# nyasyamorina/font-renderer

Measured on AMD Instinct MI355X. Metric: Mpixel/s AA glyph coverage, higher is better.
Workload: dtype f32

## Files before the change

### bindings/fr_raster.zig

```
const std = @import("std");

const Font = @import("../font/Font.zig");
const Glyph = @import("../font/Glyph.zig");
const Image = @import("Image.zig");
const Point = @import("geometry.zig").Point;

pub const fr_ctx = opaque {};
pub const fr_glyphset = opaque {};
pub const fr_plan = opaque {};
pub const fr_font = opaque {};

pub const Status = enum(c_int) { ok = 0, invalid = -1, hip = -2, nomem = -3, unsupported = -4 };
pub const Mode = enum(i32) { winding_i16 = 0, gray_debug = 1, mask_nonzero = 2, coverage_u8 = 3, sdf_u8 = 4 };
pub const SamplePhase = enum(i32) { corner = 0, center = 1 };
pub const FR_FONT_ALLOW_HINTED: u32 = 1;
pub const FR_FILL_CONSISTENT: u32 = 1;
pub const FR_TEXT_BGRA: u32 = 4;
pub const FR_TEXT_SRGB: u32 = 8;
pub const FR_TEXT_LOAD: u32 = 32;
pub const FR_TEXT_CACHE: u32 = 128;
pub const FR_TEXT_OVER: u32 = 256;

pub const RasterParams = extern struct {
    mode: i32,
    samples_per_axis: i32,
    sample_phase: i32,
    reserved: i32 = 0,
};

pub const Job = extern struct {
    glyph: u32,
    min_x: i32,
    max_y: i32,
    w: u32,
    h: u32,
    out_x: u32,
    out_y: u32,
    scale: f32,
};

pub const GlyphPlace = extern struct {
    glyph: u32,
    pen_x64: i32,
    pen_y: i32,
};

pub const GlyphPlaceEx = extern struct {
    glyph: u32,
    pen_x64: i32,
    pen_y64: i32,
    scale: f32,
    slant: f32,
};

pub const GlyphPlaceAffine = extern struct {
    glyph: u32,
    pen_x64: i32,
    pen_y64: i32,
    m: [4]f32,
};

pub const TextRun = extern struct {
    first: u32,
    count: u32,
    w: u32,
    h: u32,
    out_x: u32,
    out_y: u32,
    scale: f32,
};

pub extern "c" fn fr_abi_version() c_int;
pub extern "c" fn fr_last_error() [*:0]const u8;
pub extern "c" fn fr_build_id() [*:0]const u8;
pub extern "c" fn fr_ctx_create(device: c_int, hip_stream: ?*anyopaque, out: *?*fr_ctx) c_int;
pub extern "c" fn fr_ctx_destroy(ctx: ?*fr_ctx) void;
pub extern "c" fn fr_ctx_sync(ctx: *fr_ctx) c_int;
pub extern "c" fn fr_ctx_set_option(ctx: *fr_ctx, key: [*:0]const u8, value: i64) c_int;
pub extern "c" fn fr_glyphset_create(ctx: *fr_ctx, points_xy: [*]const i16, contour_start: [*]const u32, n_contours: u32, glyph_start: [*]const u32, n_glyphs: u32, out: *?*fr_glyphset) c_int;
pub extern "c" fn fr_glyphset_destroy(gs: ?*fr_glyphset) void;
pub extern "c" fn fr_glyphset_prepare(gs: *fr_glyphset) c_int;
pub extern "c" fn fr_glyphset_stats(gs: *const fr_glyphset, n_segments: ?*u64, n_records: ?*u64) c_int;
pub extern "c" fn fr_glyphset_set_boxes(gs: *fr_glyphset, boxes: [*]const i16) c_int;
pub extern "c" fn fr_plan_create(ctx: *fr_ctx, gs: *const fr_glyphset, jobs: [*]const Job, n_jobs: u32, params: *const RasterParams, out: *?*fr_plan) c_int;
pub extern "c" fn fr_plan_create_ex(ctx: *fr_ctx, gs: *const fr_glyphset, jobs: [*]const Job, n_jobs: u32, params: *const RasterParams, flags: u32, out: *?*fr_plan) c_int;
pub extern "c" fn fr_plan_destroy(plan: ?*fr_plan) void;
pub extern "c" fn fr_plan_render(plan: *fr_plan, out_dev: *anyopaque, out_stride: usize, out_rows: usize) c_int;
pub extern "c" fn fr_plan_render_timed(plan: *fr_plan, out_dev: *anyopaque, out_stride: usize, out_rows: usize, ms: *f32) c_int;
pub extern "c" fn fr_plan_pixels(plan: *const fr_plan) u64;
pub extern "c" fn fr_plan_stats(plan: *const fr_plan, n_jobs_cov4: ?*u32, n_jobs_general: ?*u32) c_int;
pub extern "c" fn fr_plan_describe(plan: *const fr_plan, buf: [*]u8, cap: usize) c_int;
pub extern "c" fn fr_text_plan_create(ctx: *fr_ctx, gs: *const fr_glyphset, places: [*]const GlyphPlace, n_places: u32, runs: [*]const TextRun, n_runs: u32, params: *const RasterParams, flags: u32, out: *?*fr_plan) c_int;
pub extern "c" fn fr_text_plan_create_rgba(ctx: *fr_ctx, gs: *const fr_glyphset, places: [*]const GlyphPlace, place_rgba: [*]const u8, n_places: u32, runs: [*]const TextRun, run_clear_rgba: [*]const u8, n_runs: u32, params: *const RasterParams, flags: u32, out: *?*fr_plan) c_int;
pub extern "c" fn fr_text_plan_create_ex(ctx: *fr_ctx, gs: *const fr_glyphset, places: [*]const GlyphPlaceEx, n_places: u32, runs: [*]const TextRun, n_runs: u32, params: *const RasterParams, flags: u32, out: *?*fr_plan) c_int;
pub extern "c" fn fr_text_plan_create_rgba_ex(ctx: *fr_ctx, gs: *const fr_glyphset, places: [*]const GlyphPlaceEx, place_rgba: [*]const u8, n_places: u32, runs: [*]const TextRun, run_clear_rgba: [*]const u8, n_runs: u32, params: *const RasterParams, flags: u32, out: *?*fr_plan) c_int;
pub extern "c" fn fr_text_plan_create_affine(ctx: *fr_ctx, gs: *const fr_glyphset, places: [*]const GlyphPlaceAffine, n_places: u32, runs: [*]const TextRun, n_runs: u32, params: *const RasterParams, flags: u32, out: *?*fr_plan) c_int;
pub extern "c" fn fr_text_plan_create_rgba_affine(ctx: *fr_ctx, gs: *const fr_glyphset, places: [*]const GlyphPlaceAffine, place_rgba: [*]const u8, n_places: u32, runs: [*]const TextRun, run_clear_rgba: [*]const u8, n_runs: u32, params: *const RasterParams, flags: u32, out: *?*fr_plan) c_int;
pub extern "c" fn fr_allgather_bands(ctx: *fr_ctx, nccl_comm: *anyopaque, atlas_dev: *anyopaque, band_bytes: usize) c_int;
pub extern "c" fn fr_gather_bands(ctx: *fr_ctx, nccl_comm: *anyopaque, atlas_dev: *anyopaque, band_bytes: usize, root: c_int) c_int;
pub extern "c" fn fr_render_batch(ctx: *fr_ctx, gs: *const fr_glyphset, jobs: [*]const Job, n_jobs: u32, params: *const RasterParams, out_host: *anyopaque, out_stride: usize, out_rows: usize) c_int;
pub extern "c" fn fr_render_batch_ex(ctx: *fr_ctx, gs: *const fr_glyphset, jobs: [*]const Job, n_jobs: u32, params: *const RasterParams, flags: u32, out_host: *anyopaque, out_stride: usize, out_rows: usize) c_int;
pub extern "c" fn fr_render_glyph_dims(box: *const [4]i16, units_per_em: u16, font_size: u16, min_corner: *[2]i16, max_corner: *[2]i16, width: *u16, height: *u16, scale: ?*f32) c_int;
pub extern "c" fn fr_render_glyph(ctx: *fr_ctx, points_xy: [*]const i16, contour_start: [*]const u32, n_contours: u32, box: *const [4]i16, units_per_em: u16, font_size: u16, mode: i32, out_host: *anyopaque) c_int;
pub extern "c" fn fr_render_glyph_ex(ctx: *fr_ctx, points_xy: [*]const i16, contour_start: [*]const u32, n_contours: u32, box: *const [4]i16, units_per_em: u16, font_size: u16, mode: i32, flags: u32, out_host: *anyopaque) c_int;
pub extern "c" fn fr_glyph_info_init(ctx: *fr_ctx, points_xy: [*]const i16, contour_start: [*]const u32, n_contours: u32, curve_type: [*]u8, include_p0: [*]u8) c_int;
pub extern "c" fn fr_winding_in_glyph(ctx: *fr_ctx, points_xy: [*]const i16, contour_start: [*]const u32, n_contours: u32, query_xy: [*]const i16, n_query: u32, out_winding: [*]i16) c_int;
pub extern "c" fn fr_winding_lattice(ctx: *fr_ctx, points_xy: [*]const i16, contour_start: [*]const u32, n_contours: u32, box: *const [4]i16, out_host: [*]i16) c_int;
pub extern "c" fn fr_glyph_debug_render(ctx: *fr_ctx, points_xy: [*]const i16, contour_start: [*]const u32, n_contours: u32, box: *const [4]i16, winding_scale: u8, rgb_host: [*]u8) c_int;
pub extern "c" fn fr_exact_lattice(ctx: *fr_ctx, points_xy: [*]const i16, contour_start: [*]const u32, n_contours: u32, k: u32, x0: i32, y0: i32, w: u32, h: u32, out_host: [*]i16) c_int;
pub extern "c" fn fr_exact_coverage(ctx: *fr_ctx, points_xy: [*]const i16, contour_start: [*]const u32, n_contours: u32, k: u32, x0: i32, y0: i32, w_px: u32, h_px: u32, n: u32, out_host: [*]u8) c_int;
pub extern "c" fn fr_atlas_layout(boxes: [*]const i16, n_glyphs: u32, first_glyph: u32, units_per_em: [*]const u16, n_upm: u32, font_size: u16, cell: u32, cols: u32, rows_per_page: u32, jobs_out: [*]Job, page_of_job: ?[*]u32, n_pages: ?*u32) c_int;
pub extern "c" fn fr_atlas_layout_glyph_dims(boxes: [*]const i16, n_glyphs: u32, first_glyph: u32, units_per_em: [*]const u16, n_upm: u32, font_size: u16, atlas_w: u32, @"align": u32, jobs_out: [*]Job, atlas_h: ?*u32) c_int;
pub extern "c" fn fr_font_open(ttf_bytes: *const anyopaque, len: usize, flags: u32, out: *?*fr_font) c_int;
pub extern "c" fn fr_font_close(font: ?*fr_font) void;
pub extern "c" fn fr_font_info(font: *const fr_font, units_per_em: ?*u16, num_glyphs: ?*u16, y0_baseline: ?*c_int) c_int;
pub extern "c" fn fr_font_char_to_glyph(font: *const fr_font, codepoint: u32, glyph_index: *u16) c_int;
pub extern "c" fn fr_font_glyph_advance(font: *const fr_font, glyph_index: u16, advance_width: *i16) c_int;
pub extern "c" fn fr_text_layout(font: *const fr_font, codepoints: [*]const u32, n: u32, font_size: u16, glyph_index_out: [*]u16, pen_x64_out: [*]i32, end_pen_x64: ?*i32) c_int;
pub extern "c" fn fr_font_glyph_measure(font: *fr_font, glyph_index: u16, n_contours: *u32, n_points: *u32, box: *[4]i16) c_int;
pub extern "c" fn fr_font_glyph_fill(font: *fr_font, glyph_index: u16, points_xy: [*]i16, contour_start: [*]u32) c_int;
pub extern "c" fn fr_qoi_bound(width: u32, height: u32) usize;
pub extern "c" fn fr_qoi_encode_rgb(rgb: [*]const u8, width: u32, height: u32, out: [*]u8, cap: usize, n_out: *usize) c_int;
pub extern "c" fn fr_qoi_encode_gray(gray: [*]const u8, width: u32, height: u32, stride: usize, out: [*]u8, cap: usize, n_out: *usize) c_int;
pub extern "c" fn fr_qoi_encode_rgba(rgba: [*]const u8, width: u32, height: u32, stride_px: usize, out: [*]u8, cap: usize, n_out: *usize) c_int;
pub extern "c" fn fr_srgb_decode(in: [*]const u8, n: usize, out: [*]u16) c_int;
pub extern "c" fn fr_srgb_encode(in: [*]const u16, n: usize, out: [*]u8) c_int;
pub extern "c" fn fr_rgba_unpremultiply(rgba: [*]u8, n_pixels: usize, srgb: c_int) c_int;
pub extern "c" fn fr_selftest_division(d_lo: u32, d_hi: u32, mismatches: *u64, bad_divisor: ?*u32, bad_x_bits: ?*u32) c_int;
pub extern "c" fn fr_selftest_sqrt(mismatches: *u64, bad_x_bits: ?*u32) c_int;

pub const Error = error{ RasterFailed, OutOfMemory };

var g_ctx: ?*fr_ctx = null;

fn context() Error!*fr_ctx {
    if (g_ctx == null) {
        if (fr_ctx_create(0, null, &g_ctx) != 0) return error.RasterFailed;
    }
    return g_ctx.?;
}

pub fn deinit() void {
    if (g_ctx) |c| fr_ctx_destroy(c);
    g_ctx = null;
}

fn flatten(glyph: Glyph, starts: []u32) [*]const i16 {
    starts[0] = 0;
    for (glyph.contours, 0..) |contour, i| starts[i + 1] = starts[i] + @as(u32, @intCast(contour.points.len));
    if (glyph.contours.len == 0) return @ptrCast(&[_]i16{ 0, 0 });
    return @ptrCast(glyph.contours[0].points.ptr);
}

fn boxOf(glyph: Glyph) [4]i16 {
    return .{ glyph.box.x_min, glyph.box.y_min, glyph.box.x_max, glyph.box.y_max };
}

pub fn renderGlyph(glyph: Glyph, font_info: Font.Information, font_size: u16) !Image.Gray {
    const helpers = @import("../helpers.zig");
    const ctx = try context();
    const box = boxOf(glyph);
    var mn: [2]i16 = undefined;
    var mx: [2]i16 = undefined;
    var w: u16 = 0;
    var h: u16 = 0;
    if (fr_render_glyph_dims(&box, font_info.units_per_em, font_size, &mn, &mx, &w, &h, null) != 0) return error.RasterFailed;

    var im: Image.Gray = .init(w, h);
    errdefer im.deinit();

    const starts = helpers.alloc(u32, glyph.contours.len + 1);
    defer helpers.allocator.free(starts);
    const pts = flatten(glyph, starts);
    const rc = fr_render_glyph(ctx, pts, starts.ptr, @intCast(glyph.contours.len), &box, font_info.units_per_em, font_size, @intFromEnum(Mode.gray_debug), im.data.ptr);
    if (rc != 0) return error.RasterFailed;
    return im;
}

pub fn renderGlyphWinding(glyph: Glyph, font_info: Font.Information, font_size: u16, scaler: u8, overflow_color: u8) !Image.Winding {
    const helpers = @import("../helpers.zig");
    const ctx = try context();
    const box = boxOf(glyph);
    var mn: [2]i16 = undefined;
    var mx: [2]i16 = undefined;
    var w: u16 = 0;
    var h: u16 = 0;
    if (fr_render_glyph_dims(&box, font_info.units_per_em, font_size, &mn, &mx, &w, &h, null) != 0) return error.RasterFailed;

    var im: Image.Winding = .init(w, h, scaler, overflow_color);
    errdefer im.deinit();

    const starts = helpers.alloc(u32, glyph.contours.len + 1);
    defer helpers.allocator.free(starts);
    const pts = flatten(glyph, starts);
    const rc = fr_render_glyph(ctx, pts, starts.ptr, @intCast(glyph.contours.len), &box, font_info.units_per_em, font_size, @intFromEnum(Mode.winding_i16), im.data.ptr);
    if (rc != 0) return error.RasterFailed;
    return im;
}

pub fn windingLattice(glyph: Glyph, out: []i16) !void {
    const helpers = @import("../helpers.zig");
    const ctx = try context();
    const box = boxOf(glyph);
    const starts = helpers.alloc(u32, glyph.contours.len + 1);
    defer helpers.allocator.free(starts);
    const pts = flatten(glyph, starts);
    if (fr_winding_lattice(ctx, pts, starts.ptr, @intCast(glyph.contours.len), &box, out.ptr) != 0) return error.RasterFailed;
}

pub fn glyphDebugRender(glyph: Glyph, winding_scale: u8) !Image.GlyphDebug {
    const helpers = @import("../helpers.zig");
    const ctx = try context();
    const box = boxOf(glyph);
    var im: Image.GlyphDebug = .init(glyph.box, winding_scale, 150, .{ 255, 255, 0 }, .{ 0, 255, 255 });
    errdefer im.rgb.deinit();
    const starts = helpers.alloc(u32, glyph.contours.len + 1);
    defer helpers.allocator.free(starts);
    const pts = flatten(glyph, starts);
    if (fr_glyph_debug_render(ctx, pts, starts.ptr, @intCast(glyph.contours.len), &box, winding_scale, @ptrCast(im.rgb.data.ptr)) != 0) return error.RasterFailed;
    return im;
}

pub fn renderAtlas(glyphs: []const Glyph, font_info: Font.Information, font_size: u16, cell: u32, cols: u32, samples_per_axis: i32) !Image.Gray {
    const helpers = @import("../helpers.zig");
    const ctx = try context();
    var n_points: usize = 0;
    var n_contours: usize = 0;
    for (glyphs) |g| {
        n_contours += g.contours.len;
        for (g.contours) |c| n_points += c.points.len;
    }
    const pts = helpers.alloc(i16, 2 * @max(n_points, 1));
    defer helpers.allocator.free(pts);
    const cstart = helpers.alloc(u32, n_contours + 1);
    defer helpers.allocator.free(cstart);
    const gstart = helpers.alloc(u32, glyphs.len + 1);
    defer helpers.allocator.free(gstart);
    const boxes = helpers.alloc(i16, 4 * @max(glyphs.len, 1));
    defer helpers.allocator.free(boxes);
    var p: usize = 0;
    var c_i: usize = 0;
    cstart[0] = 0;
    gstart[0] = 0;
    for (glyphs, 0..) |g, gi| {
        for (g.contours) |c| {
            for (c.points) |pt| {
                pts[2 * p] = pt.x;
                pts[2 * p + 1] = pt.y;
                p += 1;
            }
            c_i += 1;
            cstart[c_i] = @intCast(p);
        }
        gstart[gi + 1] = @intCast(c_i);
        const b = boxOf(g);
        @memcpy(boxes[4 * gi .. 4 * gi + 4], &b);
    }
    const jobs = helpers.alloc(Job, @max(glyphs.len, 1));
    defer helpers.allocator.free(jobs);
    const upm = [1]u16{font_info.units_per_em};
    if (fr_atlas_layout(boxes.ptr, @intCast(glyphs.len), 0, &upm, 1, font_size, cell, cols, 0, jobs.ptr, null, null) != 0) return error.RasterFailed;

    var gs: ?*fr_glyphset = null;
    if (fr_glyphset_create(ctx, pts.ptr, cstart.ptr, @intCast(n_contours), gstart.ptr, @intCast(glyphs.len), &gs) != 0) return error.RasterFailed;
    defer fr_glyphset_destroy(gs);

    const rows: u32 = @intCast((glyphs.len + cols - 1) / cols);
    var im: Image.Gray = .init(@intCast(cols * cell), @intCast(rows * cell));
    errdefer im.deinit();
    @memset(im.data, 0);
    const prm = RasterParams{ .mode = @intFromEnum(Mode.coverage_u8), .samples_per_axis = samples_per_axis, .sample_phase = @intFromEnum(SamplePhase.center) };
    if (fr_render_batch(ctx, gs.?, jobs.ptr, @intCast(glyphs.len), &prm, im.data.ptr, cols * cell, rows * cell) != 0) return error.RasterFailed;
    return im;
}
```

### font-renderer_amd/_lib.py

```python
from __future__ import annotations

import ctypes as C
import os

FR_WINDING_I16, FR_GRAY_DEBUG, FR_MASK_NONZERO, FR_COVERAGE_U8, FR_SDF_U8 = 0, 1, 2, 3, 4
FR_SAMPLE_CORNER, FR_SAMPLE_CENTER = 0, 1
FR_FILL_CONSISTENT = 1
FR_TEXT_SRGB, FR_TEXT_BGRA = 8, 4
FR_TEXT_LOAD = 32
FR_TEXT_CACHE = 128
FR_TEXT_OVER = 256

_HERE = os.path.dirname(os.path.abspath(__file__))


def lib_path() -> str:
    return os.environ.get("FR_RASTER_LIB") or os.path.join(_HERE, "libfr_raster.so")


class FrError(RuntimeError):
    def __init__(self, code: int, msg: str):
        super().__init__(f"fr_raster error {code}: {msg}")
        self.code = code


class Job(C.Structure):
    _fields_ = [("glyph", C.c_uint32), ("min_x", C.c_int32), ("max_y", C.c_int32),
                ("w", C.c_uint32), ("h", C.c_uint32), ("out_x", C.c_uint32), ("out_y", C.c_uint32),
                ("scale", C.c_float)]


class RasterParams(C.Structure):
    _fields_ = [("mode", C.c_int32), ("samples_per_axis", C.c_int32), ("sample_phase", C.c_int32),
                ("reserved", C.c_int32)]


class GlyphPlace(C.Structure):
    _fields_ = [("glyph", C.c_uint32), ("pen_x64", C.c_int32), ("pen_y", C.c_int32)]


class GlyphPlaceEx(C.Structure):
    _fields_ = [("glyph", C.c_uint32), ("pen_x64", C.c_int32), ("pen_y64", C.c_int32), ("scale", C.c_float),
                ("slant", C.c_float)]


class GlyphPlaceAffine(C.Structure):
    _fields_ = [("glyph", C.c_uint32), ("pen_x64", C.c_int32), ("pen_y64", C.c_int32), ("m", C.c_float * 4)]


class TextRun(C.Structure):
    _fields_ = [("first", C.c_uint32), ("count", C.c_uint32), ("w", C.c_uint32), ("h", C.c_uint32),
                ("out_x", C.c_uint32), ("out_y", C.c_uint32), ("scale", C.c_float)]


_P = C.c_void_p
_I16P, _U32P, _U8P = C.POINTER(C.c_int16), C.POINTER(C.c_uint32), C.POINTER(C.c_uint8)
SYMBOLS = [
    ("fr_abi_version", C.c_int, []),
    ("fr_last_error", C.c_char_p, []),
    ("fr_build_id", C.c_char_p, []),
    ("fr_ctx_create", C.c_int, [C.c_int, _P, C.POINTER(_P)]),
    ("fr_ctx_destroy", None, [_P]),
    ("fr_ctx_sync", C.c_int, [_P]),
    ("fr_ctx_set_option", C.c_int, [_P, C.c_char_p, C.c_int64]),
    ("fr_glyphset_create", C.c_int, [_P, _P, _P, C.c_uint32, _P, C.c_uint32, C.POINTER(_P)]),
    ("fr_glyphset_destroy", None, [_P]),
    ("fr_glyphset_prepare", C.c_int, [_P]),
    ("fr_glyphset_stats", C.c_int, [_P, C.POINTER(C.c_uint64), C.POINTER(C.c_uint64)]),
    ("fr_glyphset_set_boxes", C.c_int, [_P, _P]),
    ("fr_plan_create", C.c_int, [_P, _P, _P, C.c_uint32, C.POINTER(RasterParams), C.POINTER(_P)]),
    ("fr_plan_create_ex", C.c_int, [_P, _P, _P, C.c_uint32, C.POINTER(RasterParams), C.c_uint32, C.POINTER(_P)]),
    ("fr_plan_destroy", None, [_P]),
    ("fr_plan_render", C.c_int, [_P, _P, C.c_size_t, C.c_size_t]),
    ("fr_plan_render_timed", C.c_int, [_P, _P, C.c_size_t, C.c_size_t, C.POINTER(C.c_float)]),
    ("fr_plan_pixels", C.c_uint64, [_P]),
    ("fr_plan_stats", C.c_int, [_P, C.POINTER(C.c_uint32), C.POINTER(C.c_uint32)]),
    ("fr_plan_describe", C.c_int, [_P, C.c_char_p, C.c_size_t]),
    ("fr_text_plan_create", C.c_int, [_P, _P, _P, C.c_uint32, _P, C.c_uint32, C.POINTER(RasterParams), C.c_uint32,
                                      C.POINTER(_P)]),
    ("fr_text_plan_create_rgba", C.c_int, [_P, _P, _P, _P, C.c_uint32, _P, _P, C.c_uint32, C.POINTER(RasterParams),
                                           C.c_uint32, C.POINTER(_P)]),
    ("fr_text_plan_create_ex", C.c_int, [_P, _P, _P, C.c_uint32, _P, C.c_uint32, C.POINTER(RasterParams), C.c_uint32,
                                         C.POINTER(_P)]),
    ("fr_text_plan_create_rgba_ex", C.c_int, [_P, _P, _P, _P, C.c_uint32, _P, _P, C.c_uint32, C.POINTER(RasterParams),
                                              C.c_uint32, C.POINTER(_P)]),
    ("fr_text_plan_create_affine", C.c_int, [_P, _P, _P, C.c_uint32, _P, C.c_uint32, C.POINTER(RasterParams), C.c_uint32,
                                             C.POINTER(_P)]),
    ("fr_text_plan_create_rgba_affine", C.c_int, [_P, _P, _P, _P, C.c_uint32, _P, _P, C.c_uint32, C.POINTER(RasterParams),
                                                  C.c_uint32, C.POINTER(_P)]),
    ("fr_allgather_bands", C.c_int, [_P, _P, _P, C.c_size_t]),
    ("fr_gather_bands", C.c_int, [_P, _P, _P, C.c_size_t, C.c_int]),
    ("fr_render_batch", C.c_int, [_P, _P, _P, C.c_uint32, C.POINTER(RasterParams), _P, C.c_size_t, C.c_size_t]),
    ("fr_render_batch_ex", C.c_int, [_P, _P, _P, C.c_uint32, C.POINTER(RasterParams), C.c_uint32, _P, C.c_size_t, C.c_size_t]),
    ("fr_render_glyph_dims", C.c_int, [_P, C.c_uint16, C.c_uint16, _P, _P, C.POINTER(C.c_uint16),
                                       C.POINTER(C.c_uint16), C.POINTER(C.c_float)]),
    ("fr_render_glyph", C.c_int, [_P, _P, _P, C.c_uint32, _P, C.c_uint16, C.c_uint16, C.c_int32, _P]),
    ("fr_render_glyph_ex", C.c_int, [_P, _P, _P, C.c_uint32, _P, C.c_uint16, C.c_uint16, C.c_int32, C.c_uint32, _P]),
    ("fr_glyph_info_init", C.c_int, [_P, _P, _P, C.c_uint32, _P, _P]),
    ("fr_winding_in_glyph", C.c_int, [_P, _P, _P, C.c_uint32, _P, C.c_uint32, _P]),
    ("fr_winding_lattice", C.c_int, [_P, _P, _P, C.c_uint32, _P, _P]),
    ("fr_glyph_debug_render", C.c_int, [_P, _P, _P, C.c_uint32, _P, C.c_uint8, _P]),
    ("fr_atlas_layout", C.c_int, [_P, C.c_uint32, C.c_uint32, _P, C.c_uint32, C.c_uint16, C.c_uint32, C.c_uint32, C.c_uint32,
                                  _P, _P, C.POINTER(C.c_uint32)]),
    ("fr_atlas_layout_glyph_dims", C.c_int, [_P, C.c_uint32, C.c_uint32, _P, C.c_uint32, C.c_uint16, C.c_uint32, C.c_uint32, _P,
                                             C.POINTER(C.c_uint32)]),
    ("fr_exact_lattice", C.c_int, [_P, _P, _P, C.c_uint32, C.c_uint32, C.c_int32, C.c_int32, C.c_uint32, C.c_uint32, _P]),
    ("fr_exact_coverage", C.c_int, [_P, _P, _P, C.c_uint32, C.c_uint32, C.c_int32, C.c_int32, C.c_uint32, C.c_uint32, C.c_uint32, _P]),
    ("fr_font_open", C.c_int, [_P, C.c_size_t, C.c_uint32, C.POINTER(_P)]),
    ("fr_font_close", None, [_P]),
    ("fr_font_info", C.c_int, [_P, C.POINTER(C.c_uint16), C.POINTER(C.c_uint16), C.POINTER(C.c_int)]),
    ("fr_font_char_to_glyph", C.c_int, [_P, C.c_uint32, C.POINTER(C.c_uint16)]),
    ("fr_font_glyph_advance", C.c_int, [_P, C.c_uint16, C.POINTER(C.c_int16)]),
    ("fr_text_layout", C.c_int, [_P, _P, C.c_uint32, C.c_uint16, _P, _P, C.POINTER(C.c_int32)]),
    ("fr_font_glyph_measure", C.c_int, [_P, C.c_uint16, C.POINTER(C.c_uint32), C.POINTER(C.c_uint32), _P]),
    ("fr_font_glyph_fill", C.c_int, [_P, C.c_uint16, _P, _P]),
    ("fr_qoi_bound", C.c_size_t, [C.c_uint32, C.c_uint32]),
    ("fr_qoi_encode_rgb", C.c_int, [_P, C.c_uint32, C.c_uint32, _P, C.c_size_t, C.POINTER(C.c_size_t)]),
    ("fr_qoi_encode_gray", C.c_int, [_P, C.c_uint32, C.c_uint32, C.c_size_t, _P, C.c_size_t, C.POINTER(C.c_size_t)]),
    ("fr_qoi_encode_rgba", C.c_int, [_P, C.c_uint32, C.c_uint32, C.c_size_t, _P, C.c_size_t, C.POINTER(C.c_size_t)]),
    ("fr_srgb_decode", C.c_int, [_P, C.c_size_t, _P]),
    ("fr_srgb_encode", C.c_int, [_P, C.c_size_t, _P]),
    ("fr_rgba_unpremultiply", C.c_int, [_P, C.c_size_t, C.c_int]),
    ("fr_selftest_sqrt", C.c_int, [C.POINTER(C.c_uint64), C.POINTER(C.c_uint32)]),
    ("fr_selftest_division", C.c_int, [C.c_uint32, C.c_uint32, C.POINTER(C.c_uint64), C.POINTER(C.c_uint32), C.POINTER(C.c_uint32)]),
]

_lib = None


def _preload_hip_runtime() -> None:
    if os.environ.get("FR_HIP_RUNTIME", "") == "system":
        return
    import importlib.util
    import sys
    if "torch" in sys.modules:
        return
    try:
        spec = importlib.util.find_spec("torch")
    except (ImportError, ValueError):
        spec = None
    if spec and spec.submodule_search_locations:
        cand = os.path.join(list(spec.submodule_search_locations)[0], "lib", "libamdhip64.so")
        if os.path.exists(cand):
            C.CDLL(cand, mode=C.RTLD_GLOBAL)


def load_library() -> C.CDLL:
    global _lib
    if _lib is not None:
        return _lib
    path = lib_path()
    if not os.path.exists(path):
        raise FileNotFoundError(
            f"{path} not found: build the HIP library first (python -c 'import __graft_entry__ as g; g.build()'). "
            "There is no CPU fallback.")
    _preload_hip_runtime()
    lib = C.CDLL(path)
    for name, res, args in SYMBOLS:
        fn = getattr(lib, name)
        fn.restype = res
        fn.argtypes = args
    _lib = lib
    return lib


def check(rc: int) -> None:
    if rc != 0:
        raise FrError(rc, load_library().fr_last_error().decode("utf-8", "replace"))


def ptr(a):
    return a.ctypes.data_as(C.c_void_p)
```

### font-renderer_amd/csrc/fr_api.hip

```cpp
#include "../../include/fr_raster.h"
#include "fr_device.hpp"
#include "fr_srgb.hpp"
#include "fr_text.hpp"
#include "fr_raster_plan.hpp"
#include "fr_text_plan.hpp"

#include <cmath>
#include <cstdarg>
#include <cstdio>
#include <cstring>
#include <new>
#include <algorithm>
#include <dlfcn.h>
#include <type_traits>
#include <vector>

namespace fr {
void launch_prepare(const int16_t *, const uint32_t *, const uint32_t *, const uint32_t *, uint32_t, Rec *,
                    uint32_t *, hipStream_t, int fill = 0);
hipError_t launch_render(const RenderArgs &, const RasterLaunch &, hipStream_t);
uint32_t render_wg_waves();
hipError_t launch_cov4(const RenderArgs &, const RasterLaunch &, hipStream_t);
hipError_t launch_win1(const RenderArgs &, const RasterLaunch &, hipStream_t);
uint32_t cov4_wg_waves();
uint32_t cov4_max_segments();
hipError_t launch_sdf(const RenderArgs &, uint32_t, uint32_t, uint32_t max_seg, int cull, hipStream_t);
void launch_glyph_info(const int16_t *, const uint32_t *, const uint32_t *, uint32_t, int, uint8_t *,
                       uint8_t *, hipStream_t);
void launch_exact_winding(const int16_t *, const uint32_t *, const uint8_t *, const uint8_t *,
                          uint32_t, const int16_t *, uint64_t, uint32_t, int, int, int, int16_t *,
                          hipStream_t);
void launch_exact_cover(const int16_t *, uint32_t, uint32_t, uint32_t, uint8_t *, hipStream_t);
void launch_glyph_debug_color(const int16_t *, uint64_t, uint32_t, uint32_t, uint8_t *, hipStream_t);
}

static_assert(sizeof(fr_job) == sizeof(fr::Job), "fr_job layout");
static_assert(sizeof(fr_job) == 32, "fr_job is 32 bytes");

static thread_local char g_err[512] = "";

static int fail(int code, const char *fmt, ...)
{
    va_list ap;
    va_start(ap, fmt);
    vsnprintf(g_err, sizeof g_err, fmt, ap);
    va_end(ap);
    return code;
}
namespace fr {
int set_error(int code, const char *fmt, ...)
{
    va_list ap;
    va_start(ap, fmt);
    vsnprintf(g_err, sizeof g_err, fmt, ap);
    va_end(ap);
    return code;
}
}
#define HIP_TRY(expr)                                                                        \
    do {                                                                                     \
        hipError_t e_ = (expr);                                                              \
        if (e_ != hipSuccess)                                                                \
            return fail(e_ == hipErrorOutOfMemory ? FR_E_NOMEM : FR_E_HIP, "%s: %s", #expr,  \
                        hipGetErrorString(e_));                                              \
    } while (0)

struct fr_ctx {
    int device = 0;
    hipStream_t stream = nullptr;
    bool owns_stream = false;
    uint32_t kmax = 32;
    uint32_t strip_px = 256;
    uint32_t fuse_prepare = 1;
    uint32_t lds_pad = 0;
    uint32_t min_wgs = 2048;
    uint32_t cov4 = 1;
    uint32_t zero_copy = 0;
    uint32_t sdf_cull = 1;
    uint32_t overlap = 1;
    uint32_t graph = 0;
    uint32_t opt_epoch = 0;
    hipStream_t aux = nullptr;
    hipEvent_t ev_fork = nullptr, ev_join = nullptr;
    unsigned char *arena = nullptr;
    size_t arena_cap = 0;
    unsigned char *stage = nullptr;
    size_t stage_cap = 0;
};

struct fr_glyphset {
    fr_ctx *ctx = nullptr;
    uint32_t n_glyphs = 0, n_contours = 0, n_seg = 0, max_seg_per_glyph = 0;
    uint64_t n_points = 0;
    int16_t *d_pts = nullptr, *d_seg_pts = nullptr;
    uint32_t *d_seg_p0 = nullptr, *d_seg_prev = nullptr, *d_glyph_seg_start = nullptr, *d_rec_count = nullptr;
    fr::Rec *d_recs = nullptr;
    std::vector<uint32_t> h_glyph_seg_start;
    std::vector<uint32_t> h_root_bound;
    std::vector<uint32_t> h_ray_bound;
    std::vector<int16_t> h_box;
};

enum TextForm { TEXT_PLAIN, TEXT_EX, TEXT_AFFINE };
static constexpr TextForm text_form_of(const fr_glyph_place *) { return TEXT_PLAIN; }
static constexpr TextForm text_form_of(const fr_glyph_place_ex *) { return TEXT_EX; }
static constexpr TextForm text_form_of(const fr_glyph_place_affine *) { return TEXT_AFFINE; }

struct fr_plan {
    fr_ctx *ctx = nullptr;
    const fr_glyphset *gs = nullptr;
    fr::Job *d_jobs = nullptr;
    uint32_t *d_job_seg = nullptr;
    uint32_t *d_bits = nullptr;
    uint32_t *d_job_bits = nullptr;
    uint32_t *d_large = nullptr;
    fr::RasterPlan rp;
    fr_raster_params params{};
    uint32_t flags = 0;
    hipEvent_t ev0 = nullptr, ev1 = nullptr;
    hipGraphExec_t gexec = nullptr;
    void *g_out = nullptr;
    size_t g_stride = 0, g_rows = 0;
    uint32_t g_epoch = 0;
    bool text = false;
    bool rgba = false;
    bool srgb = false;
    bool load = false;
    int blend = 0;
    fr::TextTile *d_tiles = nullptr;
    fr::TextRun *d_runs = nullptr;
    TextForm text_form = TEXT_PLAIN;
    void *d_insts = nullptr;
    uint32_t *d_tlist = nullptr, *d_tglyphs = nullptr, *d_trec_count = nullptr;
    fr::Rec *d_trecs = nullptr;
    uint32_t n_tiles = 0, n_insts = 0, n_tglyphs = 0;
    bool cached = false;
    fr::TextMaskCell *d_mcells = nullptr;
    fr::TextMaskTile *d_mtiles = nullptr;
    uint16_t *d_masks = nullptr;
    uint32_t n_mcells = 0, n_mtiles = 0;
};

template <class T> static void dfree(T *&p) { if (p) { (void)hipFree(p); p = nullptr; } }

static fr::RasterOpts raster_opts(const fr_ctx *ctx)
{
    return fr::RasterOpts{ctx->strip_px, ctx->cov4, ctx->fuse_prepare, ctx->min_wgs, ctx->overlap, fr::render_wg_waves(), fr::cov4_wg_waves(), ctx->kmax};
}

static fr::RenderArgs render_args(const fr_plan *plan, void *out_dev, size_t out_stride)
{
    fr::RenderArgs a{};
    a.glyph_seg_start = plan->gs->d_glyph_seg_start;
    a.glyph_rec_count = plan->gs->d_rec_count;
    a.recs = plan->gs->d_recs;
    a.pts = plan->gs->d_pts;
    a.seg_p0 = plan->gs->d_seg_p0;
    a.seg_pts = plan->gs->d_seg_pts;
    a.fused = plan->ctx->fuse_prepare ? 1u : 0u;
    a.out = out_dev;
    a.out_stride = out_stride;
    a.kmax = plan->ctx->kmax;
    a.phase_center = plan->params.sample_phase == FR_SAMPLE_CENTER ? 1 : 0;
    a.lds_pad = plan->ctx->lds_pad;
    return a;
}

static hipError_t launch_entry(const fr_plan *plan, fr::RenderArgs a, const fr::RasterLaunch &e, hipStream_t st)
{
    const fr_glyphset *gs = plan->gs;
    a.jobs = plan->d_jobs + e.first;
    a.job_seg = plan->d_job_seg + 2u * (size_t)e.first;
    a.n_jobs = e.cnt; a.bands = e.bands; a.strips = e.strips; a.strip_w = e.strip_w; a.uniform = e.uniform ? 1u : 0u;
    a.bands_per_wg = e.bands_per_wg; a.band_groups = e.band_groups;
    switch (e.family) {
    case fr::RL_PREPARE:
        fr::launch_prepare(gs->d_pts, gs->d_seg_p0, gs->d_glyph_seg_start, e.cnt ? plan->d_large : nullptr,
                           e.cnt ? e.cnt : gs->n_glyphs, gs->d_recs, gs->d_rec_count, st, e.mode);
        return hipSuccess;
    case fr::RL_RENDER: return fr::launch_render(a, e, st);
    case fr::RL_COV4: return fr::launch_cov4(a, e, st);
    case fr::RL_WIN1:
        if (e.mode == 3) { a.out = plan->d_bits; a.job_bits = plan->d_job_bits + e.first; }
        return fr::launch_win1(a, e, st);
    default:
        a.bits = plan->d_bits; a.job_bits = plan->d_job_bits;
        return fr::launch_sdf(a, plan->rp.max_w, plan->rp.max_h, gs->max_seg_per_glyph, (int)plan->ctx->sdf_cull, st);
    }
}

template <class ARGS>
static hipError_t text_args_launch(const fr_plan *plan, void *out_dev, size_t out_stride, uint32_t n_tiles, char *name = nullptr,
                                   size_t name_cap = 0)
{
    ARGS a;
    a.tiles = plan->d_tiles; a.runs = plan->d_runs; a.list = plan->d_tlist;
    a.insts = static_cast<decltype(a.insts)>(plan->d_insts);
    a.recs = plan->d_trecs; a.rec_count = plan->d_trec_count;
    a.out = static_cast<uint8_t *>(out_dev);
    a.out_stride = out_stride;
    a.phase_center = plan->params.sample_phase == FR_SAMPLE_CENTER ? 1 : 0;
    return fr::launch_text(a, plan->params.samples_per_axis, (plan->flags & FR_FILL_CONSISTENT) ? 1 : 0, plan->rgba, plan->blend,
                           plan->srgb, plan->load, n_tiles, plan->ctx->stream, name, name_cap);
}

static hipError_t text_plan_launch(const fr_plan *plan, void *out_dev, size_t out_stride, uint32_t n_tiles, char *name = nullptr,
                                   size_t name_cap = 0)
{
    if (plan->cached) {
        fr::TextCachedArgs a;
        a.tiles = plan->d_tiles; a.runs = plan->d_runs; a.list = plan->d_tlist;
        a.insts = static_cast<const fr::TextCachedInst *>(plan->d_insts);
        a.recs = nullptr; a.rec_count = nullptr;
        a.out = static_cast<uint8_t *>(out_dev);
        a.out_stride = out_stride;
        a.phase_center = plan->params.sample_phase == FR_SAMPLE_CENTER ? 1 : 0;
        a.masks = plan->d_masks;
        return fr::launch_text_cached(a, plan->params.samples_per_axis, plan->rgba, plan->blend, plan->srgb, plan->load, n_tiles,
                                      plan->ctx->stream, name, name_cap);
    }
    switch (plan->text_form) {
    case TEXT_AFFINE: return text_args_launch<fr::TextAffineArgs>(plan, out_dev, out_stride, n_tiles, name, name_cap);
    case TEXT_EX: return text_args_launch<fr::TextPlaceArgs>(plan, out_dev, out_stride, n_tiles, name, name_cap);
    default: return text_args_launch<fr::TextArgs>(plan, out_dev, out_stride, n_tiles, name, name_cap);
    }
}

static hipError_t text_mask_launch(const fr_plan *plan, uint32_t n_tiles, char *name = nullptr, size_t name_cap = 0)
{
    fr::TextMaskArgs a;
    a.tiles = plan->d_mtiles; a.cells = plan->d_mcells;
    a.recs = plan->d_trecs; a.rec_count = plan->d_trec_count;
    a.masks = plan->d_masks;
    a.phase_center = plan->params.sample_phase == FR_SAMPLE_CENTER ? 1 : 0;
    return fr::launch_glyph_mask(a, plan->params.samples_per_axis, (plan->flags & FR_FILL_CONSISTENT) ? 1 : 0, n_tiles, plan->ctx->stream,
                                 name, name_cap);
}

extern "C" {

int fr_abi_version(void) { return FR_ABI_VERSION; }
const char *fr_last_error(void) { return g_err; }
#ifndef FR_BUILD_ID
#error "FR_BUILD_ID comes from the Makefile (a hash of the sources)"
#endif
const char *fr_build_id(void) { return FR_BUILD_ID; }

int fr_ctx_create(int device, void *hip_stream, fr_ctx **out)
{
    if (!out) return fail(FR_E_INVALID, "fr_ctx_create: out is NULL");
    *out = nullptr;
    int n = 0;
    hipError_t e = hipGetDeviceCount(&n);
    if (e != hipSuccess || n <= 0)
        return fail(FR_E_HIP, "fr_ctx_create: no HIP device (%s); this library has no CPU path",
                    e != hipSuccess ? hipGetErrorString(e) : "count = 0");
    if (device < 0 || device >= n) return fail(FR_E_INVALID, "fr_ctx_create: device %d of %d", device, n);
    if (fr::cov4_max_segments() != fr::COV4_MAX_SEGMENTS)
        return fail(FR_E_UNSUPPORTED, "fr_ctx_create: fast_class takes %u segments, cov4_kernel %u", fr::COV4_MAX_SEGMENTS, fr::cov4_max_segments());
    HIP_TRY(hipSetDevice(device));
    fr_ctx *c = new (std::nothrow) fr_ctx;
    if (!c) return fail(FR_E_NOMEM, "fr_ctx_create: host allocation");
    c->device = device;
    if (hip_stream) {
        c->stream = static_cast<hipStream_t>(hip_stream);
    } else {
        e = hipStreamCreateWithFlags(&c->stream, hipStreamNonBlocking);
        if (e != hipSuccess) { delete c; return fail(FR_E_HIP, "hipStreamCreate: %s", hipGetErrorString(e)); }
        c->owns_stream = true;
    }
    *out = c;
    return FR_OK;
}

void fr_ctx_destroy(fr_ctx *ctx)
{
    if (!ctx) return;
    (void)hipSetDevice(ctx->device);
    (void)hipStreamSynchronize(ctx->stream);
    if (ctx->arena) (void)hipFree(ctx->arena);
    if (ctx->stage) (void)hipHostFree(ctx->stage);
    if (ctx->aux) { (void)hipStreamSynchronize(ctx->aux); (void)hipStreamDestroy(ctx->aux); }
    if (ctx->ev_fork) (void)hipEventDestroy(ctx->ev_fork);
    if (ctx->ev_join) (void)hipEventDestroy(ctx->ev_join);
    if (ctx->owns_stream) (void)hipStreamDestroy(ctx->stream);
    delete ctx;
}

int fr_ctx_sync(fr_ctx *ctx)
{
    if (!ctx) return fail(FR_E_INVALID, "fr_ctx_sync: ctx is NULL");
    HIP_TRY(hipStreamSynchronize(ctx->stream));
    return FR_OK;
}

int fr_ctx_set_option(fr_ctx *ctx, const char *key, int64_t value)
{
    if (!ctx || !key) return fail(FR_E_INVALID, "fr_ctx_set_option: NULL argument");
    ++ctx->opt_epoch;
    if (!strcmp(key, "graph")) { ctx->graph = value ? 1u : 0u; return FR_OK; }
    if (!strcmp(key, "kmax")) {
        if (value < 1 || value > 128) return fail(FR_E_INVALID, "kmax must be in [1,128]");
        ctx->kmax = (uint32_t)value;
        return FR_OK;
    }
    if (!strcmp(key, "strip_px")) {
        if (value < 16 || value > 256 || (value % 16)) return fail(FR_E_INVALID, "strip_px must be a multiple of 16 in [16,256]");
        ctx->strip_px = (uint32_t)value;
        return FR_OK;
    }
    if (!strcmp(key, "fuse_prepare")) { ctx->fuse_prepare = value ? 1u : 0u; return FR_OK; }
    if (!strcmp(key, "lds_pad")) { ctx->lds_pad = (uint32_t)value; return FR_OK; }
    if (!strcmp(key, "cov4")) { ctx->cov4 = value ? 1u : 0u; return FR_OK; }
    if (!strcmp(key, "sdf_cull")) { ctx->sdf_cull = value ? 1u : 0u; return FR_OK; }
    if (!strcmp(key, "overlap")) {
        if (value < 0 || value > 2) return fail(FR_E_INVALID, "overlap must be 0 (never), 1 (plans of >= 32 Mpixel) or 2 (always)");
        ctx->overlap = (uint32_t)value;
        return FR_OK;
    }
    if (!strcmp(key, "zero_copy")) { ctx->zero_copy = value ? 1u : 0u; return FR_OK; }
    if (!strcmp(key, "min_wgs")) {
        if (value < 1 || value > (1 << 24)) return fail(FR_E_INVALID, "min_wgs out of range");
        ctx->min_wgs = (uint32_t)value;
        return FR_OK;
    }
    return fail(FR_E_INVALID, "fr_ctx_set_option: unknown key '%s'", key);
}

void fr_glyphset_destroy(fr_glyphset *gs)
{
    if (!gs) return;
    (void)hipSetDevice(gs->ctx->device);
    (void)hipStreamSynchronize(gs->ctx->stream);
    dfree(gs->d_pts); dfree(gs->d_seg_pts); dfree(gs->d_seg_p0); dfree(gs->d_seg_prev); dfree(gs->d_glyph_seg_start);
    dfree(gs->d_rec_count); dfree(gs->d_recs);
    delete gs;
}

int fr_glyphset_prepare(fr_glyphset *gs)
{
    if (!gs) return fail(FR_E_INVALID, "fr_glyphset_prepare: NULL");
    HIP_TRY(hipSetDevice(gs->ctx->device));
    fr::launch_prepare(gs->d_pts, gs->d_seg_p0, gs->d_glyph_seg_start, nullptr, gs->n_glyphs, gs->d_recs,
                       gs->d_rec_count, gs->ctx->stream);
    HIP_TRY(hipGetLastError());
    return FR_OK;
}

int fr_glyphset_create(fr_ctx *ctx, const int16_t *points_xy, const uint32_t *contour_start,
                       uint32_t n_contours, const uint32_t *glyph_start, uint32_t n_glyphs,
                       fr_glyphset **out)
{
    if (!ctx || !out) return fail(FR_E_INVALID, "fr_glyphset_create: NULL argument");
    *out = nullptr;
    if (n_glyphs && !glyph_start) return fail(FR_E_INVALID, "glyph_start is NULL");
    if (n_glyphs && (glyph_start[0] != 0 || glyph_start[n_glyphs] != n_contours))
        return fail(FR_E_INVALID, "glyph_start must run from 0 to n_contours");
    std::vector<uint32_t> seg_p0, seg_prev, cseg;
    uint64_t np = 0;
    int rc = fr::flatten_segments(contour_start, n_contours, &np, seg_p0, seg_prev, &cseg);
    if (rc) return rc;
    if (np && !points_xy) return fail(FR_E_INVALID, "points_xy is NULL");
    if (seg_p0.size() > 0x7fffffffull) return fail(FR_E_UNSUPPORTED, "too many segments");
    std::vector<uint32_t> gseg(n_glyphs + 1, 0u);
    for (uint32_t g = 0; g < n_glyphs; ++g) {
        if (glyph_start[g + 1] < glyph_start[g] || glyph_start[g + 1] > n_contours)
            return fail(FR_E_INVALID, "glyph_start not monotone at %u", g);
        gseg[g + 1] = cseg[glyph_start[g + 1]];
    }
    uint32_t max_seg = 0;
    for (uint32_t g = 0; g < n_glyphs; ++g) max_seg = std::max(max_seg, gseg[g + 1] - gseg[g]);
    std::vector<uint32_t> root_bound(n_glyphs, 0u), ray_bound(n_glyphs, 0u);
    {
        std::vector<std::pair<int32_t, int32_t>> ev;
        for (uint32_t g = 0; g < n_glyphs; ++g) {
            root_bound[g] = fr::glyph_root_bound(points_xy, seg_p0.data(), gseg[g], gseg[g + 1]);
            ray_bound[g] = fr::glyph_ray_bound(points_xy, seg_p0.data(), gseg[g], gseg[g + 1], ev);
        }
    }
    HIP_TRY(hipSetDevice(ctx->device));
    fr_glyphset *gs = new (std::nothrow) fr_glyphset;
    if (!gs) return fail(FR_E_NOMEM, "fr_glyphset_create: host allocation");
    gs->ctx = ctx; gs->n_glyphs = n_glyphs; gs->n_contours = n_contours;
    gs->n_seg = (uint32_t)seg_p0.size(); gs->n_points = np; gs->max_seg_per_glyph = max_seg;
    const size_t nseg1 = gs->n_seg ? gs->n_seg : 1, np1 = np ? np : 1;
#define GS_TRY(expr)                                                                          \
    do {                                                                                      \
        hipError_t e_ = (expr);                                                               \
        if (e_ != hipSuccess) {                                                               \
            fr_glyphset_destroy(gs);                                                          \
            return fail(e_ == hipErrorOutOfMemory ? FR_E_NOMEM : FR_E_HIP, "%s: %s", #expr,   \
                        hipGetErrorString(e_));                                               \
        }                                                                                     \
    } while (0)
    GS_TRY(hipMalloc(&gs->d_pts, np1 * 2 * sizeof(int16_t) + 16));
    GS_TRY(hipMalloc(&gs->d_seg_pts, nseg1 * 12 + 16));
    GS_TRY(hipMalloc(&gs->d_seg_p0, nseg1 * 4));
    GS_TRY(hipMalloc(&gs->d_seg_prev, nseg1 * 4));
    GS_TRY(hipMalloc(&gs->d_glyph_seg_start, ((size_t)n_glyphs + 1) * 4));
    GS_TRY(hipMalloc(&gs->d_rec_count, ((size_t)n_glyphs + 1) * 4));
    GS_TRY(hipMalloc(&gs->d_recs, 2 * nseg1 * sizeof(fr::Rec)));
    hipStream_t st = ctx->stream;
    if (np) GS_TRY(hipMemcpyAsync(gs->d_pts, points_xy, np * 2 * sizeof(int16_t), hipMemcpyHostToDevice, st));
    std::vector<int16_t> seg_pts((size_t)gs->n_seg * 6);
    for (size_t sgi = 0; sgi < gs->n_seg; ++sgi) memcpy(&seg_pts[6 * sgi], points_xy + 2u * (size_t)seg_p0[sgi], 12);
    if (gs->n_seg) {
        GS_TRY(hipMemcpyAsync(gs->d_seg_pts, seg_pts.data(), (size_t)gs->n_seg * 12, hipMemcpyHostToDevice, st));
        GS_TRY(hipMemcpyAsync(gs->d_seg_p0, seg_p0.data(), (size_t)gs->n_seg * 4, hipMemcpyHostToDevice, st));
        GS_TRY(hipMemcpyAsync(gs->d_seg_prev, seg_prev.data(), (size_t)gs->n_seg * 4, hipMemcpyHostToDevice, st));
    }
    GS_TRY(hipMemcpyAsync(gs->d_glyph_seg_start, gseg.data(), ((size_t)n_glyphs + 1) * 4, hipMemcpyHostToDevice, st));
    gs->h_glyph_seg_start = gseg;
    gs->h_root_bound = root_bound;
    gs->h_ray_bound = ray_bound;
    GS_TRY(hipMemsetAsync(gs->d_rec_count, 0, ((size_t)n_glyphs + 1) * 4, st));
    fr::launch_prepare(gs->d_pts, gs->d_seg_p0, gs->d_glyph_seg_start, nullptr, n_glyphs, gs->d_recs,
                       gs->d_rec_count, st);
    GS_TRY(hipGetLastError());
    GS_TRY(hipStreamSynchronize(st));
#undef GS_TRY
    *out = gs;
    return FR_OK;
}

int fr_glyphset_stats(const fr_glyphset *gs, uint64_t *n_segments, uint64_t *n_records)
{
    if (!gs) return fail(FR_E_INVALID, "fr_glyphset_stats: NULL");
    HIP_TRY(hipSetDevice(gs->ctx->device));
    if (n_segments) *n_segments = gs->n_seg;
    if (n_records) {
        std::vector<uint32_t> cnt(gs->n_glyphs + 1);
        HIP_TRY(hipStreamSynchronize(gs->ctx->stream));
        HIP_TRY(hipMemcpy(cnt.data(), gs->d_rec_count, ((size_t)gs->n_glyphs) * 4, hipMemcpyDeviceToHost));
        uint64_t t = 0;
        for (uint32_t g = 0; g < gs->n_glyphs; ++g) t += cnt[g];
        *n_records = t;
    }
    return FR_OK;
}

static int check_params(const fr_raster_params *p)
{
    if (!p) return fail(FR_E_INVALID, "params is NULL");
    if (p->mode < FR_WINDING_I16 || p->mode > FR_SDF_U8) return fail(FR_E_INVALID, "unknown mode %d", p->mode);
    const int n = p->samples_per_axis;
    if (p->mode == FR_COVERAGE_U8) {
        if (n != 1 && n != 2 && n != 4) return fail(FR_E_UNSUPPORTED, "samples_per_axis %d not in {1,2,4}", n);
    } else if (n != 1) {
        return fail(FR_E_INVALID, "samples_per_axis must be 1 for mode %d", p->mode);
    }
    if (p->sample_phase != FR_SAMPLE_CORNER && p->sample_phase != FR_SAMPLE_CENTER)
        return fail(FR_E_INVALID, "unknown sample_phase %d", p->sample_phase);
    return FR_OK;
}

void fr_plan_destroy(fr_plan *plan)
{
    if (!plan) return;
    (void)hipSetDevice(plan->ctx->device);
    (void)hipStreamSynchronize(plan->ctx->stream);
    dfree(plan->d_jobs); dfree(plan->d_job_seg); dfree(plan->d_large); dfree(plan->d_bits); dfree(plan->d_job_bits);
    dfree(plan->d_tiles); dfree(plan->d_runs); dfree(plan->d_insts); dfree(plan->d_tlist); dfree(plan->d_tglyphs);
    dfree(plan->d_trec_count); dfree(plan->d_trecs);
    dfree(plan->d_mcells); dfree(plan->d_mtiles); dfree(plan->d_masks);
    if (plan->ev0) (void)hipEventDestroy(plan->ev0);
    if (plan->ev1) (void)hipEventDestroy(plan->ev1);
    if (plan->gexec) (void)hipGraphExecDestroy(plan->gexec);
    delete plan;
}

static int check_flags(uint32_t flags, uint32_t also = 0u)
{
    const uint32_t known = (uint32_t)FR_FILL_CONSISTENT | also;
    if (flags & ~known) return fail(FR_E_INVALID, "unknown flag bits 0x%x", flags & ~known);
    return FR_OK;
}

}

static int raster_plan_upload(fr_plan *p, const fr::RasterPlanIn &in, fr::RasterTables t)
{
    fr::RasterPlan &rp = p->rp;
    hipStream_t st = p->ctx->stream;
    hipError_t e = hipSetDevice(p->ctx->device);
    auto upload = [&](auto *&dst, const void *src, size_t bytes) {
        if (e != hipSuccess || !bytes) return;
        e = hipMalloc(&dst, bytes);
        if (e == hipSuccess) e = hipMemcpyAsync(dst, src, bytes, hipMemcpyHostToDevice, st);
    };
    upload(p->d_jobs, t.sorted_jobs, (size_t)rp.n_jobs * sizeof(fr::Job));
    std::vector<uint32_t> jseg((size_t)rp.n_jobs * 2), large(rp.n_jobs - rp.n_fast), jbits(in.params.mode == FR_SDF_U8 ? rp.n_jobs : 0u);
    t.jseg = jseg.data(); t.large = large.data(); t.jbits = jbits.data();
    fr::raster_plan_tables(in, t, rp);
    upload(p->d_large, t.large, (size_t)rp.n_large * 4);
    upload(p->d_job_seg, t.jseg, (size_t)rp.n_jobs * 8);
    if (rp.bit_plane) {
        if (rp.bit_words >= 0xffffffffull) e = hipErrorInvalidValue;
        if (e == hipSuccess) e = hipMalloc(&p->d_bits, (size_t)(rp.bit_words ? rp.bit_words : 1) * 4);
        upload(p->d_job_bits, t.jbits, (size_t)rp.n_jobs * 4);
    }
    if (e == hipSuccess) e = hipStreamSynchronize(st);
    if (e == hipSuccess) e = hipEventCreate(&p->ev0);
    if (e == hipSuccess) e = hipEventCreate(&p->ev1);
    if (e != hipSuccess) return fail(e == hipErrorOutOfMemory ? FR_E_NOMEM : FR_E_HIP, "fr_plan_create: %s", hipGetErrorString(e));
    return FR_OK;
}

extern "C" {

int fr_plan_create(fr_ctx *ctx, const fr_glyphset *gs, const fr_job *jobs, uint32_t n_jobs,
                   const fr_raster_params *params, fr_plan **out)
{
    return fr_plan_create_ex(ctx, gs, jobs, n_jobs, params, 0u, out);
}

int fr_plan_create_ex(fr_ctx *ctx, const fr_glyphset *gs, const fr_job *jobs, uint32_t n_jobs,
                      const fr_raster_params *params, uint32_t flags, fr_plan **out)
{
    if (!ctx || !gs || !out) return fail(FR_E_INVALID, "fr_plan_create: NULL argument");
    *out = nullptr;
    if (const int frc = check_flags(flags)) return frc;
    if (gs->ctx != ctx) return fail(FR_E_INVALID, "glyph set belongs to another context");
    int rc = check_params(params);
    if (rc) return rc;
    if (n_jobs && !jobs) return fail(FR_E_INVALID, "jobs is NULL");
    for (uint32_t j = 0; j < n_jobs; ++j) {
        const fr_job &jb = jobs[j];
        if (jb.glyph >= gs->n_glyphs) return fail(FR_E_INVALID, "job %u: glyph %u of %u", j, jb.glyph, gs->n_glyphs);
        if (!(jb.scale > 0.0f) || !std::isfinite(jb.scale)) return fail(FR_E_INVALID, "job %u: scale must be finite and > 0", j);
        if (jb.scale < 9.5367431640625e-07f || jb.scale > 1048576.0f)
            return fail(FR_E_UNSUPPORTED, "job %u: scale outside [2^-20, 2^20]", j);
        if (jb.w > 65535u || jb.h > 65535u) return fail(FR_E_UNSUPPORTED, "job %u: cell larger than 65535", j);
        if (jb.min_x < -(1 << 22) || (int64_t)jb.min_x + jb.w > (1 << 22) || jb.max_y > (1 << 22) ||
            (int64_t)jb.max_y - jb.h < -(1 << 22))
            return fail(FR_E_UNSUPPORTED, "job %u: pixel coordinates beyond +-2^22", j);
    }
    fr_plan *p = new (std::nothrow) fr_plan;
    if (!p) return fail(FR_E_NOMEM, "fr_plan_create: host allocation");
    p->ctx = ctx; p->gs = gs; p->params = *params; p->flags = flags;
    std::vector<uint8_t> cls(n_jobs);
    std::vector<uint32_t> order(n_jobs);
    std::vector<fr_job> sorted_jobs(n_jobs);
    const fr::RasterTables t = {cls.data(), order.data(), sorted_jobs.data(), nullptr, nullptr, nullptr};
    fr::RasterPlanIn in{};
    in.jobs = jobs; in.n_jobs = n_jobs; in.params = *params;
    in.glyph_seg_start = gs->h_glyph_seg_start.data(); in.root_bound = gs->h_root_bound.data(); in.ray_bound = gs->h_ray_bound.data();
    in.sdf_fast = true; in.merge = true; in.uniform = true;
    fr::raster_plan_build(in, raster_opts(ctx), t, p->rp);
    if (p->rp.too_many) {
        delete p;
        return fail(FR_E_UNSUPPORTED, "batch needs more than 2^31 workgroups; split it");
    }
    if (const int urc = raster_plan_upload(p, in, t)) {
        fr_plan_destroy(p);
        return urc;
    }
    *out = p;
    return FR_OK;
}

int fr_glyphset_set_boxes(fr_glyphset *gs, const int16_t *boxes)
{
    if (!gs || (gs->n_glyphs && !boxes)) return fail(FR_E_INVALID, "fr_glyphset_set_boxes: NULL argument");
    for (uint32_t g = 0; g < gs->n_glyphs; ++g)
        if (boxes[4 * (size_t)g] > boxes[4 * (size_t)g + 2] || boxes[4 * (size_t)g + 1] > boxes[4 * (size_t)g + 3])
            return fail(FR_E_INVALID, "glyph %u: box min above max", g);
    gs->h_box.assign(boxes, boxes + 4 * (size_t)gs->n_glyphs);
    return FR_OK;
}

}

template <class PLACE>
static int text_plan_upload(const char *fn, fr_plan *p, const fr::TextPlanTables<PLACE> &t, const fr::TextCacheTables *cache)
{
    fr_ctx *ctx = p->ctx;
    const fr_glyphset *gs = p->gs;
    p->text_form = text_form_of((const PLACE *)nullptr);
    p->blend = t.blend;
    p->rp.pixels = t.pixels; p->rp.need_cols = t.need_cols; p->rp.need_rows = t.need_rows;
    p->n_tiles = (uint32_t)t.tiles.size(); p->n_insts = (uint32_t)t.insts.size(); p->n_tglyphs = (uint32_t)t.glyphs.size();
    hipStream_t st = ctx->stream;
    hipError_t e = hipSetDevice(ctx->device);
    auto upload = [&](auto *&dst, const auto &v) {
        using T = typename std::remove_reference<decltype(v)>::type::value_type;
        if (e != hipSuccess || v.empty()) return;
        e = hipMalloc(&dst, v.size() * sizeof(T));
        if (e == hipSuccess) e = hipMemcpyAsync(dst, v.data(), v.size() * sizeof(T), hipMemcpyHostToDevice, st);
    };
    upload(p->d_tiles, t.tiles);
    upload(p->d_runs, t.runs);
    if (cache) {
        p->cached = true;
        p->n_mcells = (uint32_t)cache->cells.size(); p->n_mtiles = (uint32_t)cache->tiles.size();
        upload(p->d_insts, cache->insts);
        upload(p->d_mcells, cache->cells);
        upload(p->d_mtiles, cache->tiles);
        if (e == hipSuccess) e = hipMalloc(&p->d_masks, (size_t)cache->elems * sizeof(uint16_t));
    } else {
        upload(p->d_insts, t.insts);
    }
    upload(p->d_tlist, t.list);
    upload(p->d_tglyphs, t.glyphs);
    if (e == hipSuccess && p->n_tglyphs) e = hipMalloc(&p->d_trecs, 2 * (size_t)gs->n_seg * sizeof(fr::Rec));
    if (e == hipSuccess && p->n_tglyphs) e = hipMalloc(&p->d_trec_count, ((size_t)gs->n_glyphs + 1) * 4);
    if (e == hipSuccess && p->n_tglyphs) e = hipMemsetAsync(p->d_trec_count, 0, ((size_t)gs->n_glyphs + 1) * 4, st);
    if (e == hipSuccess) e = hipStreamSynchronize(st);
    if (e == hipSuccess) e = hipEventCreate(&p->ev0);
    if (e == hipSuccess) e = hipEventCreate(&p->ev1);
    if (e != hipSuccess) return fail(e == hipErrorOutOfMemory ? FR_E_NOMEM : FR_E_HIP, "%s: %s", fn, hipGetErrorString(e));
    return FR_OK;
}

template <class PLACE>
static int text_plan_create(const char *fn, fr_ctx *ctx, const fr_glyphset *gs, const PLACE *places, const uint8_t *place_rgba,
                            uint32_t n_places, const fr_text_run *runs, const uint8_t *run_clear_rgba, uint32_t n_runs,
                            const fr_raster_params *params, uint32_t flags, bool rgba, fr_plan **out)
{
    if (!ctx || !gs || !out) return fail(FR_E_INVALID, "%s: NULL argument", fn);
    *out = nullptr;
    constexpr bool can_cache = !std::is_same<PLACE, fr_glyph_place_affine>::value;
    if (const int frc = check_flags(flags, (rgba ? FR_TEXT_SRGB | FR_TEXT_BGRA | FR_TEXT_LOAD | FR_TEXT_OVER : 0u) | (can_cache ? FR_TEXT_CACHE : 0u))) return frc;
    if (gs->ctx != ctx) return fail(FR_E_INVALID, "glyph set belongs to another context");
    if (!params) return fail(FR_E_INVALID, "params is NULL");
    if (params->mode < FR_WINDING_I16 || params->mode > FR_SDF_U8) return fail(FR_E_INVALID, "unknown mode %d", params->mode);
    if (params->sample_phase != FR_SAMPLE_CORNER && params->sample_phase != FR_SAMPLE_CENTER)
        return fail(FR_E_INVALID, "unknown sample_phase %d", params->sample_phase);
    const int n = params->samples_per_axis;
    if (rgba) {
        if (params->mode != FR_COVERAGE_U8)
            return fail(FR_E_UNSUPPORTED, "RGBA text runs: mode %d (only FR_COVERAGE_U8)", params->mode);
        if (n != 1 && n != 2 && n != 4) return fail(FR_E_UNSUPPORTED, "RGBA text runs: samples_per_axis %d", n);
    } else {
        if (params->mode != FR_COVERAGE_U8 && params->mode != FR_MASK_NONZERO)
            return fail(FR_E_UNSUPPORTED, "text runs: mode %d has no meaning for overlapping instances", params->mode);
        if (params->mode == FR_COVERAGE_U8 ? (n != 1 && n != 2 && n != 4) : n != 1)
            return fail(FR_E_UNSUPPORTED, "text runs: samples_per_axis %d with mode %d", n, params->mode);
    }
    fr::TextPlanIn in{};
    in.runs = runs; in.n_runs = n_runs; in.n_places = n_places;
    in.place_rgba = place_rgba; in.run_clear_rgba = run_clear_rgba;
    in.rgba = rgba; in.flags = flags;
    in.boxes = gs->h_box.empty() ? nullptr : gs->h_box.data();
    in.glyph_seg_start = gs->h_glyph_seg_start.data(); in.n_glyphs = gs->n_glyphs;
    fr::TextPlanTables<PLACE> t;
    if (const int rc = fr::text_plan_tables(in, places, t)) return rc;
    fr::TextCacheTables cache;
    if constexpr (can_cache) {
        if (flags & FR_TEXT_CACHE)
            if (const int rc = fr::text_cache_tables(in, places, t, cache)) return rc;
    }

    fr_plan *p = new (std::nothrow) fr_plan;
    if (!p) return fail(FR_E_NOMEM, "%s: host allocation", fn);
    p->ctx = ctx; p->gs = gs; p->params = *params; p->flags = flags; p->text = true;
    p->rgba = rgba;
    p->srgb = (flags & FR_TEXT_SRGB) != 0;
    p->load = (flags & FR_TEXT_LOAD) != 0;
    if (const int rc = text_plan_upload(fn, p, t, cache.cells.empty() ? nullptr : &cache)) {
        fr_plan_destroy(p);
        return rc;
    }
    *out = p;
    return FR_OK;
}

extern "C" {

int fr_text_plan_create(fr_ctx *ctx, const fr_glyphset *gs, const fr_glyph_place *places, uint32_t n_places,
                        const fr_text_run *runs, uint32_t n_runs, const fr_raster_params *params, uint32_t flags,
                        fr_plan **out)
{
    return text_plan_create("fr_text_plan_create", ctx, gs, places, nullptr, n_places, runs, nullptr, n_runs, params, flags, false, out);
}
int fr_text_plan_create_rgba(fr_ctx *ctx, const fr_glyphset *gs, const fr_glyph_place *places, const uint8_t *place_rgba,
                             uint32_t n_places, const fr_text_run *runs, const uint8_t *run_clear_rgba, uint32_t n_runs,
                             const fr_raster_params *params, uint32_t flags, fr_plan **out)
{
    return text_plan_create("fr_text_plan_create_rgba", ctx, gs, places, place_rgba, n_places, runs, run_clear_rgba, n_runs, params, flags, true, out);
}
int fr_text_plan_create_ex(fr_ctx *ctx, const fr_glyphset *gs, const fr_glyph_place_ex *places, uint32_t n_places,
                           const fr_text_run *runs, uint32_t n_runs, const fr_raster_params *params, uint32_t flags,
                           fr_plan **out)
{
    return text_plan_create("fr_text_plan_create_ex", ctx, gs, places, nullptr, n_places, runs, nullptr, n_runs, params, flags, false, out);
}
int fr_text_plan_create_rgba_ex(fr_ctx *ctx, const fr_glyphset *gs, const fr_glyph_place_ex *places, const uint8_t *place_rgba,
                                uint32_t n_places, const fr_text_run *runs, const uint8_t *run_clear_rgba, uint32_t n_runs,
                                const fr_raster_params *params, uint32_t flags, fr_plan **out)
{
    return text_plan_create("fr_text_plan_create_rgba_ex", ctx, gs, places, place_rgba, n_places, runs, run_clear_rgba, n_runs, params, flags, true, out);
}
int fr_text_plan_create_affine(fr_ctx *ctx, const fr_glyphset *gs, const fr_glyph_place_affine *places, uint32_t n_places,
                               const fr_text_run *runs, uint32_t n_runs, const fr_raster_params *params, uint32_t flags,
                               fr_plan **out)
{
    return text_plan_create("fr_text_plan_create_affine", ctx, gs, places, nullptr, n_places, runs, nullptr, n_runs, params, flags, false, out);
}
int fr_text_plan_create_rgba_affine(fr_ctx *ctx, const fr_glyphset *gs, const fr_glyph_place_affine *places,
                                    const uint8_t *place_rgba, uint32_t n_places, const fr_text_run *runs,
                                    const uint8_t *run_clear_rgba, uint32_t n_runs, const fr_raster_params *params,
                                    uint32_t flags, fr_plan **out)
{
    return text_plan_create("fr_text_plan_create_rgba_affine", ctx, gs, places, place_rgba, n_places, runs, run_clear_rgba, n_runs, params, flags, true, out);
}

int fr_srgb_decode(const uint8_t *in, size_t n, uint16_t *out)
{
    if (n && (!in || !out)) return fail(FR_E_INVALID, "fr_srgb_decode: NULL argument");
    for (size_t i = 0; i < n; ++i) out[i] = fr::SRGB_D[in[i]];
    return FR_OK;
}

int fr_srgb_encode(const uint16_t *in, size_t n, uint8_t *out)
{
    if (n && (!in || !out)) return fail(FR_E_INVALID, "fr_srgb_encode: NULL argument");
    for (size_t i = 0; i < n; ++i) {
        const uint32_t L = in[i], k = fr::SRGB_K[L >> 4];
        out[i] = (uint8_t)((k & 0xffu) + ((L & 15u) >= (k >> 8) ? 1u : 0u));
    }
    return FR_OK;
}

int fr_rgba_unpremultiply(uint8_t *rgba, size_t n_pixels, int srgb)
{
    if (n_pixels && !rgba) return fail(FR_E_INVALID, "fr_rgba_unpremultiply: NULL argument");
    for (size_t i = 0; i < n_pixels; ++i) {
        uint8_t *p = rgba + 4 * i;
        const uint32_t a = p[3];
        if (a == 0u) { p[0] = p[1] = p[2] = 0; continue; }
        for (int c = 0; c < 3; ++c) {
            if (srgb) {
                const uint32_t L = std::min<uint32_t>(65535u, (255u * fr::SRGB_D[p[c]] + a / 2u) / a), k = fr::SRGB_K[L >> 4];
                p[c] = (uint8_t)((k & 0xffu) + ((L & 15u) >= (k >> 8) ? 1u : 0u));
            } else {
                p[c] = (uint8_t)std::min<uint32_t>(255u, (255u * p[c] + a / 2u) / a);
            }
        }
    }
    return FR_OK;
}

uint64_t fr_plan_pixels(const fr_plan *plan) { return plan ? plan->rp.pixels : 0; }

int fr_plan_stats(const fr_plan *plan, uint32_t *n_jobs_cov4, uint32_t *n_jobs_general)
{
    if (!plan) return fail(FR_E_INVALID, "fr_plan_stats: NULL");
    if (plan->text) {
        if (n_jobs_cov4) *n_jobs_cov4 = 0;
        if (n_jobs_general) *n_jobs_general = plan->n_insts;
        return FR_OK;
    }
    if (n_jobs_cov4) *n_jobs_cov4 = plan->rp.n_fast;
    if (n_jobs_general) *n_jobs_general = plan->rp.n_jobs - plan->rp.n_fast;
    return FR_OK;
}

int fr_plan_describe(const fr_plan *plan, char *buf, size_t cap)
{
    if (!plan || !buf || cap == 0) return fail(FR_E_INVALID, "fr_plan_describe: NULL argument");
    buf[0] = 0;
    size_t at = 0;
    auto add = [&](const char *name, uint32_t cnt) {
        const int k = snprintf(buf + at, cap - at, "%s%s x%u", at ? "; " : "", name, cnt);
        if (k > 0) at = std::min(cap - 1, at + (size_t)k);
    };
    char name[96];
    const int fill = (plan->flags & FR_FILL_CONSISTENT) ? 1 : 0;
    if (plan->text) {
        if (plan->n_tglyphs) add(fill ? "fr::prepare_fill_kernel" : "fr::prepare_kernel", plan->n_tglyphs);
        name[0] = 0;
        if (plan->cached) {
            (void)text_mask_launch(plan, 0u, name, sizeof name);
            add(name, plan->n_mcells);
        }
        (void)text_plan_launch(plan, nullptr, 0, 0u, name, sizeof name);
        if (plan->n_tiles) add(name, plan->n_insts);
        return FR_OK;
    }
    fr::RasterLaunchList L;
    fr::raster_launches(plan->rp, plan->params, plan->flags, raster_opts(plan->ctx), plan->gs->max_seg_per_glyph, L);
    for (const bool fast : {true, false})
        for (uint32_t i = 0; i < L.n; ++i) {
            const fr::RasterLaunch &e = L.l[i];
            if (e.family == fr::RL_PREPARE || (e.family == fr::RL_COV4 || e.family == fr::RL_WIN1) != fast) continue;
            fr::raster_launch_name(e, name, sizeof name);
            add(name, e.cnt);
        }
    return FR_OK;
}

static int ensure_aux(fr_ctx *ctx)
{
    if (!ctx->aux) {
        HIP_TRY(hipStreamCreateWithFlags(&ctx->aux, hipStreamNonBlocking));
        HIP_TRY(hipEventCreateWithFlags(&ctx->ev_fork, hipEventDisableTiming));
        HIP_TRY(hipEventCreateWithFlags(&ctx->ev_join, hipEventDisableTiming));
    }
    return FR_OK;
}

static int plan_check(fr_plan *plan, void *out_dev, size_t out_stride, size_t out_rows)
{
    if (!plan) return fail(FR_E_INVALID, "plan is NULL");
    if (plan->rp.n_jobs == 0 && plan->n_tiles == 0 && !(plan->load && plan->rp.pixels)) return FR_OK;
    if (!out_dev) return fail(FR_E_INVALID, "out is NULL");
    if (plan->rp.need_cols > out_stride || plan->rp.need_rows > out_rows)
        return fail(FR_E_INVALID, "jobs need %llu x %llu elements, output is %zu x %zu",
                    (unsigned long long)plan->rp.need_cols, (unsigned long long)plan->rp.need_rows, out_stride, out_rows);
    if (out_stride > ((size_t)1 << 26))
        return fail(FR_E_INVALID, "row pitch of %zu elements: at most 2^26", out_stride);
    if (plan->rgba && ((uintptr_t)out_dev & 3u)) return fail(FR_E_INVALID, "RGBA output %p is not 4-byte aligned", out_dev);
    return FR_OK;
}

static int text_launch(fr_plan *plan, void *out_dev, size_t out_stride)
{
    if (plan->n_tiles == 0) return FR_OK;
    HIP_TRY(hipSetDevice(plan->ctx->device));
    const int fill = (plan->flags & FR_FILL_CONSISTENT) ? 1 : 0;
    hipStream_t st = plan->ctx->stream;
    if (plan->n_tglyphs) {
        fr::launch_prepare(plan->gs->d_pts, plan->gs->d_seg_p0, plan->gs->d_glyph_seg_start, plan->d_tglyphs, plan->n_tglyphs,
                           plan->d_trecs, plan->d_trec_count, st, fill);
        HIP_TRY(hipGetLastError());
    }
    if (plan->cached) HIP_TRY(text_mask_launch(plan, plan->n_mtiles));
    HIP_TRY(text_plan_launch(plan, out_dev, out_stride, plan->n_tiles));
    return FR_OK;
}

static int plan_launch_direct(fr_plan *plan, void *out_dev, size_t out_stride, size_t out_rows)
{
    if (const int rc = plan_check(plan, out_dev, out_stride, out_rows)) return rc;
    if (plan->text) return text_launch(plan, out_dev, out_stride);
    if (plan->rp.n_jobs == 0) return FR_OK;
    HIP_TRY(hipSetDevice(plan->ctx->device));
    fr_ctx *const ctx = plan->ctx;
    fr::RasterLaunchList L;
    fr::raster_launches(plan->rp, plan->params, plan->flags, raster_opts(ctx), plan->gs->max_seg_per_glyph, L);
    const fr::RenderArgs a = render_args(plan, out_dev, out_stride);
    if (L.forked) {
        if (const int rc = ensure_aux(ctx)) return rc;
        HIP_TRY(hipEventRecord(ctx->ev_fork, ctx->stream));
        HIP_TRY(hipStreamWaitEvent(ctx->aux, ctx->ev_fork, 0));
    }
    auto run = [&](uint32_t i0, uint32_t i1, bool forked) -> int {
        for (uint32_t i = i0; i < i1; ++i)
            HIP_TRY(launch_entry(plan, a, L.l[i], (forked && !L.l[i].largest) ? ctx->aux : ctx->stream));
        return FR_OK;
    };
    const int rc_parts = run(0, L.join_at, L.forked);
    if (L.forked) {
        HIP_TRY(hipEventRecord(ctx->ev_join, ctx->aux));
        HIP_TRY(hipStreamWaitEvent(ctx->stream, ctx->ev_join, 0));
    }
    if (rc_parts) return rc_parts;
    return run(L.join_at, L.n, false);
}

static int plan_launch(fr_plan *plan, void *out_dev, size_t out_stride, size_t out_rows)
{
    if (const int rc = plan_check(plan, out_dev, out_stride, out_rows)) return rc;
    if (plan->rp.n_jobs == 0 && plan->n_tiles == 0) return FR_OK;
    fr_ctx *const ctx = plan->ctx;
    if (!ctx->graph) return plan_launch_direct(plan, out_dev, out_stride, out_rows);
    HIP_TRY(hipSetDevice(ctx->device));
    if (plan->gexec && (plan->g_out != out_dev || plan->g_stride != out_stride || plan->g_rows != out_rows || plan->g_epoch != ctx->opt_epoch)) {
        (void)hipGraphExecDestroy(plan->gexec);
        plan->gexec = nullptr;
    }
    if (!plan->gexec) {
        if (const int rc = ensure_aux(ctx)) return rc;
        HIP_TRY(hipStreamBeginCapture(ctx->stream, hipStreamCaptureModeRelaxed));
        const int rc = plan_launch_direct(plan, out_dev, out_stride, out_rows);
        hipGraph_t g = nullptr;
        const hipError_t ce = hipStreamEndCapture(ctx->stream, &g);
        if (rc) { if (g) (void)hipGraphDestroy(g); return rc; }
        HIP_TRY(ce);
        const hipError_t ie = hipGraphInstantiate(&plan->gexec, g, nullptr, nullptr, 0);
        (void)hipGraphDestroy(g);
        if (ie != hipSuccess) plan->gexec = nullptr;
        HIP_TRY(ie);
        plan->g_out = out_dev; plan->g_stride = out_stride; plan->g_rows = out_rows; plan->g_epoch = ctx->opt_epoch;
    }
    HIP_TRY(hipGraphLaunch(plan->gexec, ctx->stream));
    return FR_OK;
}

namespace {
using nccl_allgather_fn = int (*)(const void *, void *, size_t, int , void * , hipStream_t);
using nccl_rank_fn = int (*)(void *, int *);
void *rccl_symbol(const char *name)
{
    if (void *p = dlsym(RTLD_DEFAULT, name)) return p;
    for (const char *lib : {"librccl.so", "librccl.so.1"})
        if (void *h = dlopen(lib, RTLD_NOW | RTLD_NOLOAD))
            if (void *p = dlsym(h, name)) return p;
    return nullptr;
}
}

int fr_allgather_bands(fr_ctx *ctx, void *nccl_comm, void *atlas_dev, size_t band_bytes)
{
    if (!ctx || !nccl_comm || !atlas_dev) return fail(FR_E_INVALID, "fr_allgather_bands: NULL argument");
    if (band_bytes == 0) return FR_OK;
    static const auto all_gather = reinterpret_cast<nccl_allgather_fn>(rccl_symbol("ncclAllGather"));
    static const auto user_rank = reinterpret_cast<nccl_rank_fn>(rccl_symbol("ncclCommUserRank"));
    if (!all_gather || !user_rank)
        return fail(FR_E_UNSUPPORTED, "fr_allgather_bands: no RCCL in this process (the host creates the communicator with it)");
    HIP_TRY(hipSetDevice(ctx->device));
    int rank = -1;
    if (user_rank(nccl_comm, &rank) != 0 || rank < 0) return fail(FR_E_INVALID, "fr_allgather_bands: ncclCommUserRank failed");
    const unsigned char *mine = static_cast<const unsigned char *>(atlas_dev) + (size_t)rank * band_bytes;
    const int rc = all_gather(mine, atlas_dev, band_bytes, 0 , nccl_comm, ctx->stream);
    if (rc != 0) return fail(FR_E_HIP, "fr_allgather_bands: ncclAllGather returned %d", rc);
    return FR_OK;
}

int fr_gather_bands(fr_ctx *ctx, void *nccl_comm, void *atlas_dev, size_t band_bytes, int root)
{
    if (root < 0) return fr_allgather_bands(ctx, nccl_comm, atlas_dev, band_bytes);
    if (!ctx || !nccl_comm || !atlas_dev) return fail(FR_E_INVALID, "fr_gather_bands: NULL argument");
    if (band_bytes == 0) return FR_OK;
    using p2p_fn = int (*)(void *, size_t, int, int, void *, hipStream_t);
    using group_fn = int (*)();
    using count_fn = int (*)(void *, int *);
    static const auto nsend = reinterpret_cast<p2p_fn>(rccl_symbol("ncclSend"));
    static const auto nrecv = reinterpret_cast<p2p_fn>(rccl_symbol("ncclRecv"));
    static const auto gstart = reinterpret_cast<group_fn>(rccl_symbol("ncclGroupStart"));
    static const auto gend = reinterpret_cast<group_fn>(rccl_symbol("ncclGroupEnd"));
    static const auto user_rank = reinterpret_cast<nccl_rank_fn>(rccl_symbol("ncclCommUserRank"));
    static const auto comm_count = reinterpret_cast<count_fn>(rccl_symbol("ncclCommCount"));
    if (!nsend || !nrecv || !gstart || !gend || !user_rank || !comm_count)
        return fail(FR_E_UNSUPPORTED, "fr_gather_bands: no RCCL in this process (the host creates the communicator with it)");
    HIP_TRY(hipSetDevice(ctx->device));
    int rank = -1, world = 0;
    if (user_rank(nccl_comm, &rank) != 0 || comm_count(nccl_comm, &world) != 0 || rank < 0 || world <= 0)
        return fail(FR_E_INVALID, "fr_gather_bands: ncclCommUserRank / ncclCommCount failed");
    if (root >= world) return fail(FR_E_INVALID, "fr_gather_bands: root %d of %d ranks", root, world);
    unsigned char *base = static_cast<unsigned char *>(atlas_dev);
    int rc = gstart();
    if (rc == 0) {
        if (rank == root) {
            for (int r = 0; r < world && rc == 0; ++r)
                if (r != root) rc = nrecv(base + (size_t)r * band_bytes, band_bytes, 0 , r, nccl_comm, ctx->stream);
        } else {
            rc = nsend(base + (size_t)rank * band_bytes, band_bytes, 0, root, nccl_comm, ctx->stream);
        }
        const int rc2 = gend();
        if (rc == 0) rc = rc2;
    }
    if (rc != 0) return fail(FR_E_HIP, "fr_gather_bands: RCCL returned %d", rc);
    return FR_OK;
}

int fr_plan_render(fr_plan *plan, void *out_dev, size_t out_stride, size_t out_rows)
{
    return plan_launch(plan, out_dev, out_stride, out_rows);
}

int fr_plan_render_timed(fr_plan *plan, void *out_dev, size_t out_stride, size_t out_rows, float *ms)
{
    if (!plan || !ms) return fail(FR_E_INVALID, "fr_plan_render_timed: NULL argument");
    HIP_TRY(hipSetDevice(plan->ctx->device));
    HIP_TRY(hipEventRecord(plan->ev0, plan->ctx->stream));
    int rc = plan_launch(plan, out_dev, out_stride, out_rows);
    if (rc) return rc;
    HIP_TRY(hipEventRecord(plan->ev1, plan->ctx->stream));
    HIP_TRY(hipEventSynchronize(plan->ev1));
    HIP_TRY(hipEventElapsedTime(ms, plan->ev0, plan->ev1));
    return FR_OK;
}

int fr_render_batch(fr_ctx *ctx, const fr_glyphset *gs, const fr_job *jobs, uint32_t n_jobs,
                    const fr_raster_params *params, void *out_host, size_t out_stride, size_t out_rows)
{
    return fr_render_batch_ex(ctx, gs, jobs, n_jobs, params, 0u, out_host, out_stride, out_rows);
}

int fr_render_batch_ex(fr_ctx *ctx, const fr_glyphset *gs, const fr_job *jobs, uint32_t n_jobs,
                       const fr_raster_params *params, uint32_t flags, void *out_host, size_t out_stride, size_t out_rows)
{
    fr_plan *plan = nullptr;
    int rc = fr_plan_create_ex(ctx, gs, jobs, n_jobs, params, flags, &plan);
    if (rc) return rc;
    if (n_jobs == 0) { fr_plan_destroy(plan); return FR_OK; }
    if (!out_host) { fr_plan_destroy(plan); return fail(FR_E_INVALID, "out_host is NULL"); }
    const size_t esz = params->mode == FR_WINDING_I16 ? 2 : 1;
    const size_t bytes = out_stride * out_rows * esz;
    void *d_out = nullptr;
    hipError_t e = hipMalloc(&d_out, bytes ? bytes : 16);
    if (e == hipSuccess) e = hipMemcpyAsync(d_out, out_host, bytes, hipMemcpyHostToDevice, ctx->stream);
    if (e == hipSuccess) {
        rc = plan_launch(plan, d_out, out_stride, out_rows);
        if (rc == FR_OK) {
            e = hipMemcpyAsync(out_host, d_out, bytes, hipMemcpyDeviceToHost, ctx->stream);
            if (e == hipSuccess) e = hipStreamSynchronize(ctx->stream);
        }
    }
    if (d_out) { (void)hipStreamSynchronize(ctx->stream); (void)hipFree(d_out); }
    fr_plan_destroy(plan);
    if (rc) return rc;
    if (e != hipSuccess) return fail(e == hipErrorOutOfMemory ? FR_E_NOMEM : FR_E_HIP, "fr_render_batch: %s", hipGetErrorString(e));
    return FR_OK;
}

int fr_render_glyph_dims(const int16_t box[4], uint16_t units_per_em, uint16_t font_size,
                         int16_t min_corner[2], int16_t max_corner[2], uint16_t *width,
                         uint16_t *height, float *scale_out)
{
    if (!box || !min_corner || !max_corner || !width || !height) return fail(FR_E_INVALID, "fr_render_glyph_dims: NULL argument");
    if (units_per_em == 0 || font_size == 0) return fail(FR_E_INVALID, "units_per_em and font_size must be > 0");
    const float scale = (float)font_size / (float)units_per_em;
    const float b[4] = {(float)box[0] * scale, (float)box[1] * scale, (float)box[2] * scale, (float)box[3] * scale};
    const float lo0 = std::floor(b[0]), lo1 = std::floor(b[1]), hi0 = std::ceil(b[2]), hi1 = std::ceil(b[3]);
    if (lo0 < -32768.f || lo1 < -32768.f || hi0 > 32767.f || hi1 > 32767.f)
        return fail(FR_E_UNSUPPORTED, "scaled box leaves i16 (the reference's @intFromFloat would trap)");
    min_corner[0] = (int16_t)lo0; min_corner[1] = (int16_t)lo1;
    max_corner[0] = (int16_t)hi0; max_corner[1] = (int16_t)hi1;
    const int w = (int)max_corner[0] - min_corner[0] + 1, h = (int)max_corner[1] - min_corner[1] + 1;
    if (w < 1 || h < 1 || w > 32767 || h > 32767) return fail(FR_E_UNSUPPORTED, "image size leaves i16");
    *width = (uint16_t)w; *height = (uint16_t)h;
    if (scale_out) *scale_out = scale;
    return FR_OK;
}

int fr_render_glyph(fr_ctx *ctx, const int16_t *points_xy, const uint32_t *contour_start,
                    uint32_t n_contours, const int16_t box[4], uint16_t units_per_em,
                    uint16_t font_size, int32_t mode, void *out_host)
{
    return fr_render_glyph_ex(ctx, points_xy, contour_start, n_contours, box, units_per_em, font_size, mode, 0u, out_host);
}

int fr_render_glyph_ex(fr_ctx *ctx, const int16_t *points_xy, const uint32_t *contour_start,
                       uint32_t n_contours, const int16_t box[4], uint16_t units_per_em,
                       uint16_t font_size, int32_t mode, uint32_t flags, void *out_host)
{
    if (!ctx) return fail(FR_E_INVALID, "ctx is NULL");
    if (const int frc = check_flags(flags)) return frc;
    int16_t mn[2], mx[2];
    uint16_t w, h;
    float scale;
    int rc = fr_render_glyph_dims(box, units_per_em, font_size, mn, mx, &w, &h, &scale);
    if (rc) return rc;
    fr_raster_params prm{};
    prm.mode = mode; prm.samples_per_axis = 1; prm.sample_phase = FR_SAMPLE_CORNER;
    rc = check_params(&prm);
    if (rc) return rc;
    if (!out_host) return fail(FR_E_INVALID, "out_host is NULL");
    const uint32_t zero_start[1] = {0};
    std::vector<uint32_t> seg_p0, seg_prev;
    uint64_t np = 0;
    rc = fr::flatten_segments(n_contours ? contour_start : zero_start, n_contours, &np, seg_p0, seg_prev, nullptr);
    if (rc) return rc;
    if (np && !points_xy) return fail(FR_E_INVALID, "points_xy is NULL");
    const uint32_t ns = (uint32_t)seg_p0.size();
    if (scale < 9.5367431640625e-07f || scale > 1048576.0f) return fail(FR_E_UNSUPPORTED, "scale outside [2^-20, 2^20]");
    fr_job jb{};
    jb.glyph = 0; jb.min_x = mn[0]; jb.max_y = mx[1]; jb.w = w; jb.h = h; jb.out_x = 0; jb.out_y = 0; jb.scale = scale;
    auto al = [](size_t v) { return (v + 15u) & ~(size_t)15; };
    const size_t esz = mode == FR_WINDING_I16 ? 2 : 1;
    const size_t o_pts = 0, o_p0 = al(o_pts + np * 4 + 16), o_spts = al(o_p0 + (size_t)ns * 4 + 4);
    const size_t o_gseg = al(o_spts + (size_t)ns * 12 + 16), o_job = al(o_gseg + 8), o_jseg = al(o_job + sizeof(fr_job));
    const size_t o_large = al(o_jseg + 8), up = al(o_large + 4);
    const size_t o_cnt = up, o_recs = al(o_cnt + 8), o_out = al(o_recs + (size_t)(ns ? ns : 1) * 2 * sizeof(fr::Rec));
    const size_t total = al(o_out + (size_t)w * h * esz);
    HIP_TRY(hipSetDevice(ctx->device));
    const size_t img_bytes = (size_t)w * h * esz;
    const bool zero_copy = ns <= 128u && mode != FR_SDF_U8 && total <= ((size_t)1 << 20) && ctx->zero_copy;
    if (!zero_copy && total > ctx->arena_cap) {
        HIP_TRY(hipStreamSynchronize(ctx->stream));
        if (ctx->arena) { (void)hipFree(ctx->arena); ctx->arena = nullptr; ctx->arena_cap = 0; }
        const size_t cap = std::max<size_t>(total + total / 2, 1u << 20);
        HIP_TRY(hipMalloc(&ctx->arena, cap));
        ctx->arena_cap = cap;
    }
    const size_t stage_need = zero_copy ? total : up + img_bytes;
    if (stage_need > ctx->stage_cap) {
        HIP_TRY(hipStreamSynchronize(ctx->stream));
        if (ctx->stage) { (void)hipHostFree(ctx->stage); ctx->stage = nullptr; ctx->stage_cap = 0; }
        const size_t cap = std::max<size_t>(stage_need * 2, 1u << 16);
        HIP_TRY(hipHostMalloc(reinterpret_cast<void **>(&ctx->stage), cap, hipHostMallocDefault));
        ctx->stage_cap = cap;
    }
    unsigned char *st = ctx->stage;
    memset(st, 0, up);
    if (np) memcpy(st + o_pts, points_xy, np * 4);
    if (ns) memcpy(st + o_p0, seg_p0.data(), (size_t)ns * 4);
    for (uint32_t sgi = 0; sgi < ns; ++sgi) memcpy(st + o_spts + 12u * (size_t)sgi, points_xy + 2u * (size_t)seg_p0[sgi], 12);
    const uint32_t gseg[2] = {0, ns}, jseg[2] = {0, ns}, large0[1] = {0};
    memcpy(st + o_gseg, gseg, 8); memcpy(st + o_job, &jb, sizeof jb); memcpy(st + o_jseg, jseg, 8); memcpy(st + o_large, large0, 4);
    unsigned char *A0 = zero_copy ? st : ctx->arena;
    if (!zero_copy) HIP_TRY(hipMemcpyAsync(A0, st, up, hipMemcpyHostToDevice, ctx->stream));
    fr_glyphset gs;
    gs.ctx = ctx; gs.n_glyphs = 1; gs.n_contours = n_contours; gs.n_seg = ns; gs.max_seg_per_glyph = ns; gs.n_points = np;
    gs.d_pts = reinterpret_cast<int16_t *>(A0 + o_pts); gs.d_seg_pts = reinterpret_cast<int16_t *>(A0 + o_spts);
    gs.d_seg_p0 = reinterpret_cast<uint32_t *>(A0 + o_p0); gs.d_glyph_seg_start = reinterpret_cast<uint32_t *>(A0 + o_gseg);
    gs.d_rec_count = reinterpret_cast<uint32_t *>(A0 + o_cnt); gs.d_recs = reinterpret_cast<fr::Rec *>(A0 + o_recs);
    fr_plan pl;
    pl.ctx = ctx; pl.gs = &gs; pl.params = prm; pl.flags = flags;
    pl.d_jobs = reinterpret_cast<fr::Job *>(A0 + o_job); pl.d_job_seg = reinterpret_cast<uint32_t *>(A0 + o_jseg);
    pl.d_large = reinterpret_cast<uint32_t *>(A0 + o_large);
    {
        std::vector<std::pair<int32_t, int32_t>> ev;
        const uint32_t root = fr::glyph_root_bound(points_xy, seg_p0.data(), 0, ns), ray = fr::glyph_ray_bound(points_xy, seg_p0.data(), 0, ns, ev);
        const fr::RasterPlanIn in = fr::single_glyph_in(&jb, gseg, &root, &ray, prm);
        uint8_t cls1;
        uint32_t order1, jseg1[2], large1, jbits1;
        fr_job sorted1;
        const fr::RasterTables t1 = {&cls1, &order1, &sorted1, jseg1, &large1, &jbits1};
        fr::raster_plan_build(in, raster_opts(ctx), t1, pl.rp);
        fr::raster_plan_tables(in, t1, pl.rp);
    }
    int lrc = FR_OK;
    if (mode == FR_SDF_U8 || pl.rp.n_large) {
        hipError_t e = hipMemsetAsync(gs.d_rec_count, 0, 8, ctx->stream);
        if (e != hipSuccess) lrc = fail(FR_E_HIP, "hipMemsetAsync: %s", hipGetErrorString(e));
    }
    if (lrc == FR_OK) lrc = plan_launch_direct(&pl, A0 + o_out, w, h);
    hipError_t e = hipSuccess;
    if (lrc == FR_OK && !zero_copy) e = hipMemcpyAsync(st + up, A0 + o_out, img_bytes, hipMemcpyDeviceToHost, ctx->stream);
    hipError_t e2 = hipStreamSynchronize(ctx->stream);
    if (lrc == FR_OK && e == hipSuccess && e2 == hipSuccess) memcpy(out_host, zero_copy ? st + o_out : st + up, img_bytes);
    gs.d_pts = gs.d_seg_pts = nullptr; gs.d_seg_p0 = gs.d_glyph_seg_start = gs.d_rec_count = nullptr; gs.d_recs = nullptr;
    pl.d_jobs = nullptr; pl.d_job_seg = nullptr; pl.d_large = nullptr;
    if (lrc) return lrc;
    if (e == hipSuccess) e = e2;
    if (e != hipSuccess) return fail(FR_E_HIP, "fr_render_glyph: %s", hipGetErrorString(e));
    return FR_OK;
}

struct ExactDev {
    int16_t *pts = nullptr;
    uint32_t *seg_p0 = nullptr, *seg_prev = nullptr;
    uint8_t *ctype = nullptr, *inc = nullptr;
    uint32_t n_seg = 0;
    int K = 1;
    ~ExactDev() { dfree(pts); dfree(seg_p0); dfree(seg_prev); dfree(ctype); dfree(inc); }
};

static int exact_setup(fr_ctx *ctx, const int16_t *points_xy, const uint32_t *contour_start,
                       uint32_t n_contours, ExactDev &d, int K = 1)
{
    if (!ctx) return fail(FR_E_INVALID, "ctx is NULL");
    std::vector<uint32_t> seg_p0, seg_prev;
    uint64_t np = 0;
    int rc = fr::flatten_segments(contour_start, n_contours, &np, seg_p0, seg_prev, nullptr);
    if (rc) return rc;
    if (np && !points_xy) return fail(FR_E_INVALID, "points_xy is NULL");
    d.n_seg = (uint32_t)seg_p0.size();
    const size_t ns1 = d.n_seg ? d.n_seg : 1, np1 = np ? np : 1;
    HIP_TRY(hipSetDevice(ctx->device));
    HIP_TRY(hipMalloc(&d.pts, np1 * 4 + 16));
    HIP_TRY(hipMalloc(&d.seg_p0, ns1 * 4));
    HIP_TRY(hipMalloc(&d.seg_prev, ns1 * 4));
    HIP_TRY(hipMalloc(&d.ctype, ns1));
    HIP_TRY(hipMalloc(&d.inc, ns1));
    if (np) HIP_TRY(hipMemcpyAsync(d.pts, points_xy, np * 4, hipMemcpyHostToDevice, ctx->stream));
    if (d.n_seg) {
        HIP_TRY(hipMemcpyAsync(d.seg_p0, seg_p0.data(), (size_t)d.n_seg * 4, hipMemcpyHostToDevice, ctx->stream));
        HIP_TRY(hipMemcpyAsync(d.seg_prev, seg_prev.data(), (size_t)d.n_seg * 4, hipMemcpyHostToDevice, ctx->stream));
    }
    d.K = K;
    fr::launch_glyph_info(d.pts, d.seg_p0, d.seg_prev, d.n_seg, K, d.ctype, d.inc, ctx->stream);
    HIP_TRY(hipGetLastError());
    HIP_TRY(hipStreamSynchronize(ctx->stream));
    return FR_OK;
}

int fr_glyph_info_init(fr_ctx *ctx, const int16_t *points_xy, const uint32_t *contour_start,
                       uint32_t n_contours, uint8_t *curve_type, uint8_t *include_p0)
{
    ExactDev d;
    int rc = exact_setup(ctx, points_xy, contour_start, n_contours, d);
    if (rc) return rc;
    if (d.n_seg) {
        if (!curve_type || !include_p0) return fail(FR_E_INVALID, "output is NULL");
        HIP_TRY(hipMemcpy(curve_type, d.ctype, d.n_seg, hipMemcpyDeviceToHost));
        HIP_TRY(hipMemcpy(include_p0, d.inc, d.n_seg, hipMemcpyDeviceToHost));
    }
    return FR_OK;
}

static int exact_run(fr_ctx *ctx, ExactDev &d, const int16_t *query_xy, uint64_t n_query,
                     uint32_t lat_w, int lat_x0, int lat_y0, void *out_host,
                     uint32_t cover_w = 0, uint32_t cover_h = 0, uint32_t cover_n = 0)
{
    if (n_query == 0) return FR_OK;
    if (!out_host) return fail(FR_E_INVALID, "output is NULL");
    if (n_query > 0xffffffffull * 256ull) return fail(FR_E_UNSUPPORTED, "too many query points");
    int16_t *d_q = nullptr, *d_out = nullptr;
    hipError_t e = hipMalloc(&d_out, n_query * 2);
    if (e == hipSuccess && query_xy) e = hipMalloc(&d_q, n_query * 4);
    if (e == hipSuccess && query_xy) e = hipMemcpyAsync(d_q, query_xy, n_query * 4, hipMemcpyHostToDevice, ctx->stream);
    if (e == hipSuccess) {
        fr::launch_exact_winding(d.pts, d.seg_p0, d.ctype, d.inc, d.n_seg, d_q, n_query, lat_w, lat_x0, lat_y0, d.K, d_out, ctx->stream);
        e = hipGetLastError();
    }
    uint8_t *d_cov = nullptr;
    if (cover_n) {
        const size_t npx = (size_t)cover_w * cover_h;
        if (e == hipSuccess) e = hipMalloc(&d_cov, npx ? npx : 1);
        if (e == hipSuccess) {
            fr::launch_exact_cover(d_out, cover_w, cover_h, cover_n, d_cov, ctx->stream);
            e = hipGetLastError();
        }
        if (e == hipSuccess) e = hipMemcpyAsync(out_host, d_cov, npx, hipMemcpyDeviceToHost, ctx->stream);
    } else if (e == hipSuccess) {
        e = hipMemcpyAsync(out_host, d_out, n_query * 2, hipMemcpyDeviceToHost, ctx->stream);
    }
    hipError_t e2 = hipStreamSynchronize(ctx->stream);
    if (e == hipSuccess) e = e2;
    dfree(d_q); dfree(d_out); dfree(d_cov);
    if (e != hipSuccess) return fail(e == hipErrorOutOfMemory ? FR_E_NOMEM : FR_E_HIP, "exact winding: %s", hipGetErrorString(e));
    return FR_OK;
}

int fr_winding_in_glyph(fr_ctx *ctx, const int16_t *points_xy, const uint32_t *contour_start,
                        uint32_t n_contours, const int16_t *query_xy, uint32_t n_query,
                        int16_t *out_winding)
{
    if (n_query && !query_xy) return fail(FR_E_INVALID, "query_xy is NULL");
    ExactDev d;
    int rc = exact_setup(ctx, points_xy, contour_start, n_contours, d);
    if (rc) return rc;
    return exact_run(ctx, d, query_xy, n_query, 1, 0, 0, out_winding);
}

int fr_winding_lattice(fr_ctx *ctx, const int16_t *points_xy, const uint32_t *contour_start,
                       uint32_t n_contours, const int16_t box[4], int16_t *out_host)
{
    if (!box) return fail(FR_E_INVALID, "box is NULL");
    const int W = (int)box[2] - box[0] + 3, H = (int)box[3] - box[1] + 3;
    if (W < 1 || H < 1) return fail(FR_E_INVALID, "empty box");
    ExactDev d;
    int rc = exact_setup(ctx, points_xy, contour_start, n_contours, d);
    if (rc) return rc;
    return exact_run(ctx, d, nullptr, (uint64_t)W * H, (uint32_t)W, box[0] - 1, box[3] + 1, out_host);
}

static int check_k(uint32_t K, int32_t x0, int32_t y0, uint64_t w, uint64_t h)
{
    if (K < 1 || K > 8) return fail(FR_E_UNSUPPORTED, "K must be in [1, 8] (128-bit predicate range)");
    if (w > (1u << 20) || h > (1u << 20)) return fail(FR_E_UNSUPPORTED, "lattice larger than 2^20 per axis");
    const int64_t lim = (int64_t)1 << 20;
    if (x0 < -lim || x0 + (int64_t)w > lim || y0 > lim || y0 - (int64_t)h < -lim)
        return fail(FR_E_UNSUPPORTED, "lattice beyond +-2^20 scaled units");
    return FR_OK;
}

int fr_exact_lattice(fr_ctx *ctx, const int16_t *points_xy, const uint32_t *contour_start,
                     uint32_t n_contours, uint32_t K, int32_t x0, int32_t y0, uint32_t w, uint32_t h,
                     int16_t *out_host)
{
    int rc = check_k(K, x0, y0, w, h);
    if (rc) return rc;
    ExactDev d;
    rc = exact_setup(ctx, points_xy, contour_start, n_contours, d, (int)K);
    if (rc) return rc;
    return exact_run(ctx, d, nullptr, (uint64_t)w * h, w, x0, y0, out_host);
}

int fr_exact_coverage(fr_ctx *ctx, const int16_t *points_xy, const uint32_t *contour_start,
                      uint32_t n_contours, uint32_t K, int32_t x0, int32_t y0, uint32_t w_px, uint32_t h_px,
                      uint32_t n, uint8_t *out_host)
{
    if (n < 1 || n > 8) return fail(FR_E_INVALID, "samples per axis must be in [1, 8]");
    int rc = check_k(K, x0, y0, (uint64_t)w_px * n, (uint64_t)h_px * n);
    if (rc) return rc;
    ExactDev d;
    rc = exact_setup(ctx, points_xy, contour_start, n_contours, d, (int)K);
    if (rc) return rc;
    return exact_run(ctx, d, nullptr, (uint64_t)w_px * n * h_px * n, w_px * n, x0, y0, out_host, w_px, h_px, n);
}


int fr_glyph_debug_render(fr_ctx *ctx, const int16_t *points_xy, const uint32_t *contour_start,
                          uint32_t n_contours, const int16_t box[4], uint8_t winding_scale, uint8_t *rgb_host)
{
    if (!box) return fail(FR_E_INVALID, "box is NULL");
    if (!rgb_host) return fail(FR_E_INVALID, "rgb_host is NULL");
    const int W = (int)box[2] - box[0] + 3, H = (int)box[3] - box[1] + 3;
    if (W < 1 || H < 1) return fail(FR_E_INVALID, "empty box");
    ExactDev d;
    int rc = exact_setup(ctx, points_xy, contour_start, n_contours, d);
    if (rc) return rc;
    const uint64_t nq = (uint64_t)W * H;
    int16_t *d_lat = nullptr;
    uint8_t *d_rgb = nullptr;
    hipError_t e = hipMalloc(&d_lat, nq * 2);
    if (e == hipSuccess) e = hipMalloc(&d_rgb, nq * 3);
    if (e == hipSuccess) {
        fr::launch_exact_winding(d.pts, d.seg_p0, d.ctype, d.inc, d.n_seg, nullptr, nq, (uint32_t)W, box[0] - 1, box[3] + 1, 1, d_lat, ctx->stream);
        fr::launch_glyph_debug_color(d_lat, nq, winding_scale, 150u, d_rgb, ctx->stream);
        e = hipGetLastError();
    }
    if (e == hipSuccess) e = hipMemcpyAsync(rgb_host, d_rgb, nq * 3, hipMemcpyDeviceToHost, ctx->stream);
    hipError_t e2 = hipStreamSynchronize(ctx->stream);
    if (e == hipSuccess) e = e2;
    dfree(d_lat); dfree(d_rgb);
    if (e != hipSuccess) return fail(e == hipErrorOutOfMemory ? FR_E_NOMEM : FR_E_HIP, "fr_glyph_debug_render: %s", hipGetErrorString(e));
    for (uint32_t c = 0; c < n_contours; ++c) {
        const int16_t *cp = points_xy + 2u * (size_t)contour_start[c];
        const uint32_t curves = (contour_start[c + 1] - contour_start[c]) / 2u;
        for (uint32_t k = 0; k < curves; ++k) {
            for (int which = 0; which < 2; ++which) {
                const int16_t *pt = cp + 2u * (2u * k + (uint32_t)which);
                const int64_t wq = (int64_t)pt[0] - box[0] + 1, hq = (int64_t)box[3] - pt[1] + 1;
                if (wq < 0 || hq < 0 || wq >= W || hq >= H)
                    return fail(FR_E_INVALID, "glyph point outside its box (the reference would write out of bounds)");
                uint8_t *px = rgb_host + 3u * ((size_t)hq * W + (size_t)wq);
                if (which == 0) { px[0] = 255; px[1] = 255; px[2] = 0; }
                else { px[0] = 0; px[1] = 255; px[2] = 255; }
            }
        }
    }
    return FR_OK;
}

int fr_atlas_layout(const int16_t *boxes, uint32_t n_glyphs, uint32_t first_glyph,
                    const uint16_t *units_per_em, uint32_t n_upm, uint16_t font_size,
                    uint32_t cell, uint32_t cols, uint32_t rows_per_page,
                    fr_job *jobs_out, uint32_t *page_of_job, uint32_t *n_pages)
{
    if (n_glyphs && (!boxes || !jobs_out)) return fail(FR_E_INVALID, "fr_atlas_layout: NULL argument");
    if (!units_per_em || (n_upm != 1 && n_upm != n_glyphs)) return fail(FR_E_INVALID, "units_per_em: one value or one per glyph");
    if (cell == 0 || cols == 0 || font_size == 0) return fail(FR_E_INVALID, "cell, cols and font_size must be > 0");
    if ((uint64_t)cell * cols > 0xffffffffull) return fail(FR_E_UNSUPPORTED, "atlas wider than 2^32 pixels");
    const uint64_t per_page = rows_per_page ? (uint64_t)rows_per_page * cols : 0;
    for (uint32_t i = 0; i < n_glyphs; ++i) {
        const uint16_t upm = units_per_em[n_upm == 1 ? 0 : i];
        if (upm == 0) return fail(FR_E_INVALID, "units_per_em must be > 0");
        const float scale = (float)font_size / (float)upm;
        const float fx = std::floor((float)boxes[4 * (size_t)i + 0] * scale);
        const float fy = std::ceil((float)boxes[4 * (size_t)i + 3] * scale);
        const uint64_t slot = per_page ? i % per_page : i;
        const uint64_t row = slot / cols;
        if (row * cell > 0xffffffffull) return fail(FR_E_UNSUPPORTED, "atlas taller than 2^32 pixels: use pages");
        fr_job &jb = jobs_out[i];
        jb.glyph = first_glyph + i;
        jb.min_x = (int32_t)fx; jb.max_y = (int32_t)fy;
        jb.w = cell; jb.h = cell;
        jb.out_x = (uint32_t)(slot % cols) * cell;
        jb.out_y = (uint32_t)row * cell;
        jb.scale = scale;
        if (page_of_job) page_of_job[i] = per_page ? (uint32_t)(i / per_page) : 0u;
    }
    if (n_pages) *n_pages = per_page ? (uint32_t)((n_glyphs + per_page - 1) / per_page) : (n_glyphs ? 1u : 0u);
    return FR_OK;
}

int fr_atlas_layout_glyph_dims(const int16_t *boxes, uint32_t n_glyphs, uint32_t first_glyph,
                               const uint16_t *units_per_em, uint32_t n_upm, uint16_t font_size,
                               uint32_t atlas_w, uint32_t align, fr_job *jobs_out, uint32_t *atlas_h)
{
    if (n_glyphs && (!boxes || !jobs_out)) return fail(FR_E_INVALID, "fr_atlas_layout_glyph_dims: NULL argument");
    if (!units_per_em || (n_upm != 1 && n_upm != n_glyphs)) return fail(FR_E_INVALID, "units_per_em: one value or one per glyph");
    if (atlas_w == 0 || font_size == 0) return fail(FR_E_INVALID, "atlas_w and font_size must be > 0");
    if (align == 0) align = 1;
    uint64_t x = 0, y = 0, shelf_h = 0;
    for (uint32_t i = 0; i < n_glyphs; ++i) {
        int16_t mn[2], mx[2];
        uint16_t w, h;
        float scale;
        const int rc = fr_render_glyph_dims(boxes + 4 * (size_t)i, units_per_em[n_upm == 1 ? 0 : i], font_size, mn, mx, &w, &h, &scale);
        if (rc) return rc;
        if (w > atlas_w) return fail(FR_E_INVALID, "glyph %u is %u pixels wide, the atlas %u", i, (unsigned)w, atlas_w);
        x = (x + align - 1) / align * align;
        if (x + w > atlas_w) { x = 0; y += shelf_h; shelf_h = 0; }
        if (y + h > 0xffffffffull) return fail(FR_E_UNSUPPORTED, "atlas taller than 2^32 pixels");
        fr_job &jb = jobs_out[i];
        jb.glyph = first_glyph + i;
        jb.min_x = mn[0]; jb.max_y = mx[1];
        jb.w = w; jb.h = h;
        jb.out_x = (uint32_t)x; jb.out_y = (uint32_t)y;
        jb.scale = scale;
        x += w;
        shelf_h = std::max<uint64_t>(shelf_h, h);
    }
    if (atlas_h) *atlas_h = (uint32_t)std::min<uint64_t>(y + shelf_h, 0xffffffffull);
    return FR_OK;
}

}
```

### font-renderer_amd/csrc/fr_c4.hpp

```cpp
#pragma once
#include "fr_records.hpp"
#include "fr_wave.hpp"

namespace fr {

#ifndef FR_C4_WAVES
#define FR_C4_WAVES 4
#endif
#ifndef FR_C4_OCC
#define FR_C4_OCC 4
#endif
#ifndef FR_C4_PCAP
#define FR_C4_PCAP 448
#endif
#ifndef FR_C4_OCC_SMALL
#define FR_C4_OCC_SMALL 6
#endif
#ifndef FR_DYN_BANDS
#define FR_DYN_BANDS 1
#endif
#ifndef FR_W1_OCC_SMALL
#define FR_W1_OCC_SMALL 6
#endif
enum { C4_WAVES = FR_C4_WAVES, C4_PCAP = FR_C4_PCAP };
constexpr uint32_t c4_lstride(int cap) { return (uint32_t)cap + 4u; }
constexpr int c4_occ(int cap, int wlog, int rpl) { return rpl >= 16 ? 2 : (rpl >= 8 ? 3 : ((cap <= 16 && rpl == 2) ? FR_C4_OCC_SMALL : FR_C4_OCC)); }
constexpr int w1_occ(int rpl, int wlog) { return rpl >= 16 ? 2 : ((rpl == 2) ? FR_W1_OCC_SMALL : FR_C4_OCC); }
template <uint32_t LSTRIDE>
__device__ __forceinline__ uint4 c4_ld16(const uint16_t *p)
{
    if ((LSTRIDE * 2) % 16 == 0) return *reinterpret_cast<const uint4 *>(p);
    const uint2 a = reinterpret_cast<const uint2 *>(p)[0], b = reinterpret_cast<const uint2 *>(p)[1];
    return make_uint4(a.x, a.y, b.x, b.y);
}
template <uint32_t LSTRIDE>
__device__ __forceinline__ void c4_st16(uint16_t *p, uint4 v)
{
    if ((LSTRIDE * 2) % 16 == 0) { *reinterpret_cast<uint4 *>(p) = v; return; }
    reinterpret_cast<uint2 *>(p)[0] = make_uint2(v.x, v.y);
    reinterpret_cast<uint2 *>(p)[1] = make_uint2(v.z, v.w);
}

struct __attribute__((aligned(8))) Rec40 {
    float a;
    float b;
    float c1, c2;
    float ax, bx, p0x;
    float rden;
    float sgn;
    uint32_t fr;
};

__device__ __forceinline__ uint32_t c4_sel(unsigned long long m, uint32_t if_set, uint32_t if_clear)
{
    uint32_t r;
    asm("v_cndmask_b32_e64 %0, %1, %2, %3" : "=v"(r) : "v"(if_clear), "v"(if_set), "s"(m));
    return r;
}
__device__ __forceinline__ float c4_self(unsigned long long m, float if_set, float if_clear)
{
    return __builtin_bit_cast(float, c4_sel(m, __builtin_bit_cast(uint32_t, if_set), __builtin_bit_cast(uint32_t, if_clear)));
}
__device__ __forceinline__ void c4_store16(void *dst, uint4 v)
{
    typedef uint32_t u32x4 __attribute__((ext_vector_type(4)));
    typedef u32x4 u32x4_u __attribute__((aligned(4)));
    u32x4 w = {v.x, v.y, v.z, v.w};
    __builtin_nontemporal_store(w, reinterpret_cast<u32x4_u *>(dst));
}

template <int FILL = 0>
__device__ __forceinline__ Rec40 c4_make_rec40(const Rec &r, uint32_t ra, uint32_t re)
{
    Rec40 m;
    const bool lin = (int32_t)r.flags < 0;
    m.a = lin ? r.c1 : r.a;
    m.b = r.b; m.c1 = lin ? 0.0f : r.c1; m.c2 = r.c2;
    m.ax = r.ax; m.bx = r.bx; m.p0x = r.p0x; m.rden = r.rden;
    m.sgn = r.sqsign ? -1.0f : 1.0f;
    const uint32_t cb = (lin || FILL) ? (r.flags & 2u) : 2u, zb = (lin || FILL) ? cb : 0u;
    m.fr = ra | (re << 12) | (cb << 24) | (zb << 26) | (lin ? 0x80000000u : 0u);
    return m;
}

template <int N, uint32_t NCOL, uint32_t STEP>
__device__ __forceinline__ void c4_fill_cx(float *s_cxp, uint32_t tid, int32_t min_xs, int phase, const ScaleDiv &sdiv)
{
    auto num = [&](uint32_t j) { return (float)(min_xs + (int32_t)(j / (uint32_t)N)) + sub_off((int)(j % (uint32_t)N), N, phase); };
    if (sdiv.pow2) {
        for (uint32_t j = tid; j < NCOL; j += STEP) s_cxp[1u + j] = num(j) * sdiv.inv;
    } else {
        for (uint32_t j = tid; j < NCOL; j += STEP) s_cxp[1u + j] = num(j) / sdiv.scale;
    }
}

template <uint32_t RCAP, int N, uint32_t NCOL, int FILL>
__device__ __forceinline__ uint32_t c4_setup_small(const RenderArgs &A, const Job &job, uint32_t seg0, uint32_t nseg, uint32_t x0s,
                                                   int phase, float *s_cxp, Rec40 *s_rec, uint32_t *s_wcnt, uint32_t *s_tmp, const float *cyt = nullptr)
{
    const uint32_t tid = threadIdx.x, lane = tid & 63u, wave = tid >> 6;
    const uint32_t Hs = job.h * (uint32_t)N;
    const ScaleDiv sdiv = scale_div(job.scale);
    RowGeom geo;
    geo.max_y = job.max_y; geo.set_scale(sdiv); geo.rows = Hs; geo.n = N; geo.phase = phase; geo.cyt = cyt;
    const bool have = lane < 2u * nseg;
    Rec r;
    RowGuess g;
    Piece pc;
    g.empty = true; g.ra = 1u; g.re = 0u;
    uint32_t cls = 3u;
    if (have) {
        record_prep<FILL>(A.seg_pts + 6u * (size_t)(seg0 + (lane >> 1)), lane & 1u, geo, r, g, &pc);
        if (!g.empty) {
            const uint32_t row = (wave == 0u) ? g.ra - 1u : (wave == 1u) ? g.ra : (wave == 2u) ? g.re - 1u : g.re;
            if (row < Hs && (wave != 2u || g.re > g.ra)) cls = (uint32_t)row_class<FILL>(r, pc, geo.cy(row));
        }
    }
    s_tmp[tid] = cls;
    const int32_t min_xs = job.min_x + (int32_t)x0s;
    c4_fill_cx<N, NCOL, 256u>(s_cxp, tid, min_xs, phase, sdiv);
    if (tid == 2) s_cxp[0] = -__builtin_inff();
    if (tid == 3) s_cxp[1u + NCOL] = __builtin_inff();
    __syncthreads();
    if (wave == 0u) {
        Rec40 mine;
        mine.fr = 0u;
        bool live = false;
        if (have) {
            uint32_t ra = g.ra, re = g.re;
            if (!g.empty) {
                const uint32_t c0 = s_tmp[lane], c1 = s_tmp[64u + lane], c2 = s_tmp[128u + lane], c3 = s_tmp[192u + lane];
                const bool ok = (c0 >= 2u) && (c1 <= 1u || c1 == 3u) && re >= ra && (c2 >= 1u) && (c3 == 0u || c3 == 3u);
                if (!ok) record_settle<FILL>(r, geo, ra, re, &pc);
            }
            live = ra < re;
            mine = c4_make_rec40<FILL>(r, ra, re);
        }
        const bool linr = live && (int32_t)mine.fr < 0;
        const unsigned long long lm = __ballot(live && !linr), ll = __ballot(linr), below = (1ull << lane) - 1ull;
        const uint32_t n_quad = (uint32_t)__popcll(lm);
        uint32_t pos = RCAP;
        if ((lm >> lane) & 1ull) pos = (uint32_t)__popcll(lm & below);
        if ((ll >> lane) & 1ull) pos = n_quad + (uint32_t)__popcll(ll & below);
        if (pos < RCAP) s_rec[pos] = mine;
        if (lane == 0u) s_wcnt[0] = min(n_quad + (uint32_t)__popcll(ll), RCAP);
    }
    __syncthreads();
    return s_wcnt[0];
}

template <uint32_t RCAP, int N, uint32_t NCOL, int FILL>
__device__ __forceinline__ uint32_t c4_setup_mid(const RenderArgs &A, const Job &job, uint32_t seg0, uint32_t nseg, uint32_t x0s,
                                                 int phase, float *s_cxp, Rec40 *s_rec, uint32_t *s_wcnt, uint32_t *s_tmp, const float *cyt = nullptr)
{
    const uint32_t tid = threadIdx.x, lane = tid & 63u, wave = tid >> 6;
    const uint32_t c = tid & 127u, h = tid >> 7;
    const uint32_t Hs = job.h * (uint32_t)N;
    const ScaleDiv sdiv = scale_div(job.scale);
    RowGeom geo;
    geo.max_y = job.max_y; geo.set_scale(sdiv); geo.rows = Hs; geo.n = N; geo.phase = phase; geo.cyt = cyt;
    const bool have = c < 2u * nseg;
    Rec r;
    RowGuess g;
    Piece pc;
    g.empty = true; g.ra = 1u; g.re = 0u;
    uint32_t cls0 = 3u, cls1 = 3u;
    if (have) {
        record_prep<FILL>(A.seg_pts + 6u * (size_t)(seg0 + (c >> 1)), c & 1u, geo, r, g, &pc);
        if (!g.empty) {
            const uint32_t end = h ? g.re : g.ra;
            if (end - 1u < Hs && (h == 0u || g.re > g.ra)) cls0 = (uint32_t)row_class<FILL>(r, pc, geo.cy(end - 1u));
            if (end < Hs) cls1 = (uint32_t)row_class<FILL>(r, pc, geo.cy(end));
        }
    }
    s_tmp[tid] = cls0 | (cls1 << 8);
    const int32_t min_xs = job.min_x + (int32_t)x0s;
    c4_fill_cx<N, NCOL, 256u>(s_cxp, tid, min_xs, phase, sdiv);
    if (tid == 2) s_cxp[0] = -__builtin_inff();
    if (tid == 3) s_cxp[1u + NCOL] = __builtin_inff();
    __syncthreads();
    Rec40 mine;
    mine.fr = 0u;
    bool live = false;
    if (h == 0u && have) {
        uint32_t ra = g.ra, re = g.re;
        if (!g.empty) {
            const uint32_t up = s_tmp[c], dn = s_tmp[128u + c];
            const uint32_t c0 = up & 0xffu, c1 = up >> 8, c2 = dn & 0xffu, c3 = dn >> 8;
            const bool ok = (c0 >= 2u) && (c1 <= 1u || c1 == 3u) && re >= ra && (c2 >= 1u) && (c3 == 0u || c3 == 3u);
            if (!ok) record_settle<FILL>(r, geo, ra, re, &pc);
        }
        live = ra < re;
        mine = c4_make_rec40<FILL>(r, ra, re);
    }
    const bool linr = live && (int32_t)mine.fr < 0;
    const unsigned long long lm = __ballot(live && !linr), ll = __ballot(linr), below = (1ull << lane) - 1ull;
    if (lane == 0u && wave < 2u) { s_wcnt[wave] = (uint32_t)__popcll(lm); s_wcnt[2u + wave] = (uint32_t)__popcll(ll); }
    __syncthreads();
    const uint32_t q0 = s_wcnt[0], q1 = s_wcnt[1], l0 = s_wcnt[2], l1 = s_wcnt[3];
    const uint32_t n_quad = q0 + q1;
    uint32_t pos = RCAP;
    if ((lm >> lane) & 1ull) pos = (wave ? q0 : 0u) + (uint32_t)__popcll(lm & below);
    if ((ll >> lane) & 1ull) pos = n_quad + (wave ? l0 : 0u) + (uint32_t)__popcll(ll & below);
    if (wave < 2u && pos < RCAP) s_rec[pos] = mine;
    __syncthreads();
    return min(n_quad + l0 + l1, RCAP);
}

template <uint32_t NW, uint32_t RCAP, int N, uint32_t NCOL, int FILL = 0>
__device__ __forceinline__ uint32_t c4_setup(const RenderArgs &A, const Job &job, uint32_t seg0, uint32_t nseg, uint32_t x0s,
                                             int phase, float *s_cxp, Rec40 *s_rec, uint32_t *s_wcnt, uint32_t *s_tmp, const float *cyt = nullptr)
{
    if (NW == 4u && 2u * nseg <= 64u)
        return c4_setup_small<RCAP, N, NCOL, FILL>(A, job, seg0, nseg, x0s, phase, s_cxp, s_rec, s_wcnt, s_tmp, cyt);
    if (NW == 4u && 2u * nseg <= 128u)
        return c4_setup_mid<RCAP, N, NCOL, FILL>(A, job, seg0, nseg, x0s, phase, s_cxp, s_rec, s_wcnt, s_tmp, cyt);
    const uint32_t tid = threadIdx.x, lane = tid & 63u, wave = tid >> 6;
    const uint32_t Hs = job.h * (uint32_t)N;
    const ScaleDiv sdiv = scale_div(job.scale);
    constexpr uint32_t CPT = (RCAP >= 1024u ? 1536u : (RCAP >= 512u ? 768u : 512u)) / (64u * NW);
    s_wcnt = s_tmp;
    Rec40 mine[CPT];
    unsigned long long lm[CPT], ll[CPT];
#pragma unroll
    for (uint32_t it = 0; it < CPT; ++it) {
        const uint32_t c = tid + it * 64u * NW;
        bool live = false;
        lm[it] = 0ull; ll[it] = 0ull;
        mine[it].fr = 0u;
        if (it > 0 && it * 64u * NW >= 2u * nseg) continue;
        if (c < 2u * nseg) {
            Rec r;
            RowGeom geo;
            geo.max_y = job.max_y; geo.set_scale(sdiv); geo.rows = Hs; geo.n = N; geo.phase = phase; geo.cyt = cyt;
            build_record_rows<FILL>(A.seg_pts + 6u * (size_t)(seg0 + (c >> 1)), c & 1u, geo, r);
            const uint32_t ra = __builtin_bit_cast(uint32_t, r.lo), re = __builtin_bit_cast(uint32_t, r.hi);
            live = ra < re;
            mine[it] = c4_make_rec40<FILL>(r, ra, re);
        }
        const bool linr = live && (int32_t)mine[it].fr < 0;
        lm[it] = __ballot(live && !linr);
        ll[it] = __ballot(linr);
        if (lane == 0) { s_wcnt[it * NW + wave] = (uint32_t)__popcll(lm[it]); s_wcnt[CPT * NW + it * NW + wave] = (uint32_t)__popcll(ll[it]); }
    }
    const int32_t min_xs = job.min_x + (int32_t)x0s;
    c4_fill_cx<N, NCOL, 64u * NW>(s_cxp, tid, min_xs, phase, sdiv);
    if (tid == 2) s_cxp[0] = -__builtin_inff();
    if (tid == 3) s_cxp[1u + NCOL] = __builtin_inff();
    __syncthreads();
    uint32_t rec_cnt = 0;
    {
        uint32_t base_q[CPT], base_l[CPT], n_quad = 0;
#pragma unroll
        for (uint32_t it = 0; it < CPT; ++it) base_q[it] = base_l[it] = 0;
#pragma unroll
        for (uint32_t q = 0; q < CPT * NW; ++q) {
            if (q >= NW && q / NW * 64u * NW >= 2u * nseg) continue;
            const uint32_t cq = s_wcnt[q], cl = s_wcnt[CPT * NW + q];
#pragma unroll
            for (uint32_t it = 0; it < CPT; ++it) {
                base_q[it] += (q < it * NW + wave) ? cq : 0u;
                base_l[it] += (q < it * NW + wave) ? cl : 0u;
            }
            n_quad += cq;
            rec_cnt += cq + cl;
        }
#pragma unroll
        for (uint32_t it = 0; it < CPT; ++it) {
            const unsigned long long below = (1ull << lane) - 1ull;
            uint32_t pos = RCAP;
            if ((lm[it] >> lane) & 1ull) pos = base_q[it] + (uint32_t)__popcll(lm[it] & below);
            if ((ll[it] >> lane) & 1ull) pos = n_quad + base_l[it] + (uint32_t)__popcll(ll[it] & below);
            if (pos < RCAP) s_rec[pos] = mine[it];
        }
    }
    rec_cnt = min(rec_cnt, RCAP);
    __syncthreads();
    return rec_cnt;
}

}
```

### font-renderer_amd/csrc/fr_device.hpp

```cpp
#pragma once
#include <hip/hip_runtime.h>
#include <stdint.h>
#include <type_traits>

#pragma clang fp contract(off)

namespace fr {

struct __attribute__((aligned(16))) Rec {
    float lo, hi, a, b, c1, c2, ax, bx, p0x;
    uint32_t flags;
    float rden;
    uint32_t sqsign;
};

__device__ __forceinline__ float div_by_int(float x, float d, float rd)
{
    const float q = x * rd;
    const float r = __builtin_fmaf(-q, d, x);
    return __builtin_fmaf(r, rd, q);
}
__device__ __forceinline__ float sqrt_rn(float x)
{
    const float s = __builtin_amdgcn_sqrtf(x);
    const float sm = __builtin_bit_cast(float, __builtin_bit_cast(int, s) - 1);
    const float sp = __builtin_bit_cast(float, __builtin_bit_cast(int, s) + 1);
    const float rm = __builtin_fmaf(-sm, s, x);
    const float rp = __builtin_fmaf(-sp, s, x);
    float r = (rm <= 0.0f) ? sm : s;
    r = (rp > 0.0f) ? sp : r;
    return r;
}
template <int VARIANT>
__device__ __forceinline__ float sqrt_fast(float x)
{
    const float s = __builtin_amdgcn_sqrtf(x);
    const float g = VARIANT == 0 ? __builtin_amdgcn_rcpf(s) : __builtin_amdgcn_rsqf(x);
    const float h = __builtin_fminf(0.5f * g, 1.0e+30f);
    const float r = __builtin_fmaf(-s, s, x);
    return __builtin_fmaf(r, h, s);
}
struct ScaleDiv {
    float scale = 1.0f, inv = 1.0f;
    bool pow2 = false;
    __device__ __forceinline__ float operator()(float x) const
    {
        if (pow2) return x * inv;
        return x / scale;
    }
};
__device__ __forceinline__ ScaleDiv scale_div(float scale)
{
    ScaleDiv d;
    const uint32_t b = (uint32_t)__builtin_amdgcn_readfirstlane(__builtin_bit_cast(int, scale));
    const uint32_t e = (b >> 23) & 0xffu;
    d.scale = scale;
    d.pow2 = (b & 0x007fffffu) == 0u && e - 107u <= 40u;
    d.inv = __builtin_bit_cast(float, (b & 0x80000000u) | ((254u - e) << 23));
    return d;
}
enum : uint32_t {
    REC_LINEAR = 0x80000000u,
    REC_NEG_ROOT = 2u,
    REC_LIN_MINUS = 4u,
    REC_LIN_PLUS = 2u
};

struct Job {
    uint32_t glyph;
    int32_t min_x, max_y;
    uint32_t w, h;
    uint32_t out_x, out_y;
    float scale;
};

struct RenderArgs {
    const Job *jobs;
    const uint32_t *glyph_seg_start;
    const uint32_t *job_seg;
    const uint32_t *glyph_rec_count;
    const Rec *recs;
    const int16_t *pts;
    const uint32_t *seg_p0;
    const int16_t *seg_pts;
    const uint32_t *job_bits;
    const uint32_t *bits;
    uint32_t fused;
    uint32_t uniform;
    void *out;
    uint64_t out_stride;
    uint32_t n_jobs, bands, strips, strip_w, kmax;
    uint32_t bands_per_wg, band_groups;
    int32_t phase_center;
    uint32_t lds_pad;
    uint32_t nwin_log, lds_region, lds_rec_bytes, lds_wave_bytes, lds_tail;
};

template <typename K>
inline hipError_t launch_kernel(K *kern, dim3 grid, dim3 block, size_t lds, hipStream_t stream, const RenderArgs &a)
{
    if (lds > 48 * 1024) {
        const hipError_t e = hipFuncSetAttribute(reinterpret_cast<const void *>(kern), hipFuncAttributeMaxDynamicSharedMemorySize, (int)lds);
        if (e != hipSuccess) return e;
    }
    hipLaunchKernelGGL(kern, grid, block, lds, stream, a);
    return hipGetLastError();
}

template <int... V> struct Among {};
template <class F> inline hipError_t pick(const int *, F &&f) { return f(); }
template <class F, int... V, class... L>
inline hipError_t pick(const int *x, F &&f, Among<V...>, L... rest)
{
    hipError_t r = hipErrorInvalidValue;
    (void)((*x == V && (r = pick(x + 1, [&](auto... c) { return f(std::integral_constant<int, V>{}, c...); }, rest...), true)) || ...);
    return r;
}

__host__ __device__ inline uint32_t f2key(float f)
{
    uint32_t b;
    __builtin_memcpy(&b, &f, 4);
    return (b & 0x80000000u) ? ~b : (b | 0x80000000u);
}
__host__ __device__ inline float key2f(uint32_t k)
{
    uint32_t b = (k & 0x80000000u) ? (k & 0x7fffffffu) : ~k;
    float f;
    __builtin_memcpy(&f, &b, 4);
    return f;
}

__device__ __forceinline__ float rec_t_quad(const Rec &r, float cy)
{
    float delta = cy * r.a + r.c1 - r.c2;
    float sq = __builtin_sqrtf(delta);
    float num = (r.flags & REC_NEG_ROOT) ? (r.b - sq) : (r.b + sq);
    return num / r.a;
}
__device__ __forceinline__ float rec_t_lin(const Rec &r, float cy)
{
    return (cy - r.b) / r.c1;
}
template <int FILL = 0>
__device__ __forceinline__ bool rec_cross(const Rec &r, float cy, float &xx, int &sgn)
{
    float t;
    bool ok;
    if constexpr (FILL != 0) {
        if (r.flags & REC_LINEAR) {
            t = rec_t_lin(r, cy);
        } else {
            const float delta = __builtin_fmaxf(cy * r.a + r.c1 - r.c2, 0.0f);
            const float sq = __builtin_sqrtf(delta);
            t = ((r.flags & REC_NEG_ROOT) ? (r.b - sq) : (r.b + sq)) / r.a;
        }
        sgn = (r.flags & 2u) ? 1 : -1;
        xx = (r.ax * t + r.bx) * t + r.p0x;
        return true;
    }
    if (r.flags & REC_LINEAR) {
        t = rec_t_lin(r, cy);
        ok = !(t < 0.0f || t >= 1.0f);
        sgn = (r.flags & REC_LIN_MINUS) ? -1 : 1;
    } else {
        const float delta = cy * r.a + r.c1 - r.c2;
        t = rec_t_quad(r, cy);
        ok = !(delta < 0.0f) && !(t < 0.0f || t >= 1.0f);
        float dy = r.a * t + (-r.b);
        sgn = (dy > 0.0f) ? -1 : 1;
    }
    xx = (r.ax * t + r.bx) * t + r.p0x;
    return ok;
}

template <int FILL = 0>
__device__ inline int brute_winding(const Rec *__restrict__ recs, uint32_t n, float cx, float cy)
{
    int w = 0;
    for (uint32_t c = 0; c < n; ++c) {
        const Rec r = recs[c];
        if (cy >= r.lo && cy <= r.hi) {
            float xx; int sgn;
            if (rec_cross<FILL>(r, cy, xx, sgn) && !(xx < cx)) w += sgn;
        }
    }
    return w;
}

__device__ __forceinline__ float sub_off(int k, int n, int phase_center)
{
    return ((float)k + (phase_center ? 0.5f : 0.0f)) / (float)n;
}

}
```

### font-renderer_amd/csrc/fr_prepare.hip

```cpp
#include "fr_records.hpp"

namespace fr {

template <int FILL>
__device__ __forceinline__ void prepare_body(const int16_t *__restrict__ pts,
                                                     const uint32_t *__restrict__ seg_p0,
                                                     const uint32_t *__restrict__ glyph_seg_start,
                                                     const uint32_t *__restrict__ glyph_list,
                                                     uint32_t n_glyphs,
                                                     Rec *__restrict__ out_recs,
                                                     uint32_t *__restrict__ glyph_rec_count)
{
    if (blockIdx.x >= n_glyphs) return;
    const uint32_t g = glyph_list ? glyph_list[blockIdx.x] : blockIdx.x;
    const uint32_t s0 = glyph_seg_start[g], s1 = glyph_seg_start[g + 1];
    const uint32_t n_cand = 2u * (s1 - s0);
    const uint32_t lane = threadIdx.x;
    const size_t out_base = 2u * (size_t)s0;
    uint32_t n_out = 0;
    for (uint32_t base = 0; base < n_cand; base += 64u) {
        const uint32_t c = base + lane;
        bool valid = false;
        Rec r;
        if (c < n_cand) valid = FILL ? build_record_fill(pts + 2u * (size_t)seg_p0[s0 + (c >> 1)], c & 1u, r) : build_record(pts + 2u * (size_t)seg_p0[s0 + (c >> 1)], c & 1u, r);
        const unsigned long long m = __ballot(valid);
        if (valid) {
            const uint32_t pos = n_out + (uint32_t)__popcll(m & ((1ull << lane) - 1ull));
            out_recs[out_base + pos] = r;
        }
        n_out += (uint32_t)__popcll(m);
    }
    if (lane == 0) glyph_rec_count[g] = n_out;
}
__global__ __launch_bounds__(64) void prepare_kernel(const int16_t *__restrict__ pts,
                                                     const uint32_t *__restrict__ seg_p0,
                                                     const uint32_t *__restrict__ glyph_seg_start,
                                                     const uint32_t *__restrict__ glyph_list,
                                                     uint32_t n_glyphs,
                                                     Rec *__restrict__ out_recs,
                                                     uint32_t *__restrict__ glyph_rec_count)
{
    prepare_body<0>(pts, seg_p0, glyph_seg_start, glyph_list, n_glyphs, out_recs, glyph_rec_count);
}
__global__ __launch_bounds__(64) void prepare_fill_kernel(const int16_t *__restrict__ pts,
                                                     const uint32_t *__restrict__ seg_p0,
                                                     const uint32_t *__restrict__ glyph_seg_start,
                                                     const uint32_t *__restrict__ glyph_list,
                                                     uint32_t n_glyphs,
                                                     Rec *__restrict__ out_recs,
                                                     uint32_t *__restrict__ glyph_rec_count)
{
    prepare_body<1>(pts, seg_p0, glyph_seg_start, glyph_list, n_glyphs, out_recs, glyph_rec_count);
}

void launch_prepare(const int16_t *pts, const uint32_t *seg_p0, const uint32_t *glyph_seg_start,
                    const uint32_t *glyph_list, uint32_t n_glyphs, Rec *out_recs, uint32_t *glyph_rec_count,
                    hipStream_t stream, int fill)
{
    if (n_glyphs == 0) return;
    hipLaunchKernelGGL(fill ? prepare_fill_kernel : prepare_kernel, dim3(n_glyphs), dim3(64), 0, stream, pts, seg_p0,
                       glyph_seg_start, glyph_list, n_glyphs, out_recs, glyph_rec_count);
}

}
```

### font-renderer_amd/csrc/fr_records.hpp

```cpp
#pragma once
#include "fr_device.hpp"

namespace fr {

__device__ __forceinline__ int classify(const Rec &r, float cy)
{
    if (r.flags & REC_LINEAR) {
        float t = rec_t_lin(r, cy);
        bool up = r.c1 > 0.0f;
        if (t < 0.0f) return up ? 0 : 2;
        if (t >= 1.0f) return up ? 2 : 0;
        return 1;
    }
    float delta = cy * r.a + r.c1 - r.c2;
    if (delta < 0.0f) return (r.a > 0.0f) ? 0 : 2;
    float t = rec_t_quad(r, cy);
    bool neg = (r.flags & REC_NEG_ROOT) != 0;
    if (t < 0.0f) return neg ? 2 : 0;
    if (t >= 1.0f) return neg ? 0 : 2;
    return 1;
}

__device__ __noinline__ uint32_t first_at_least(float ra, float rb, float rc1, float rc2, uint32_t rflags, int T, uint32_t L, uint32_t H)
{
    Rec r;
    r.a = ra; r.b = rb; r.c1 = rc1; r.c2 = rc2; r.flags = rflags;
    uint32_t step = 1u;
    while (step < (1u << 30) && H - L > 2u * step) {
        const uint32_t pl = L + step - 1u;
        if (classify(r, key2f(pl)) >= T) { H = pl; break; }
        L = pl + 1u;
        const uint32_t ph = H - step;
        if (classify(r, key2f(ph)) < T) { L = ph + 1u; break; }
        H = ph;
        step <<= 1;
    }
    while (L < H) {
        const uint32_t mid = L + ((H - L) >> 1);
        if (classify(r, key2f(mid)) >= T) H = mid; else L = mid + 1u;
    }
    return L;
}

__device__ inline bool accept_bracket(const Rec &r, float p0y, float p2y, float &lo, float &hi)
{
    const uint32_t kmin = f2key(-3.402823466e+38f), kmax = f2key(3.402823466e+38f);
    uint32_t LB = kmin, HB = kmax + 1u;
    bool seen1 = false;
    auto probe = [&](float c) {
        if (!(c >= -3.402823466e+38f && c <= 3.402823466e+38f)) return;
        const uint32_t k = f2key(c);
        const int cl = classify(r, c);
        if (cl == 0) { if (k + 1u > LB) LB = k + 1u; }
        else if (cl == 2) { if (k < HB) HB = k; }
        else seen1 = true;
    };
    float w = 0.0f;
    float vert = 0.0f;
    const bool quad = !(r.flags & REC_LINEAR);
    if (quad) {
        vert = p0y - (r.b * r.b) / r.a;
        const float big = fmaxf(fmaxf(fabsf(r.c1), fabsf(r.c2)), 1.0f);
        w = (big * 1.1920929e-07f) / fabsf(r.a);
    }
    auto probe3 = [&](float c) {
        const float d = fmaxf(4.0f * w, fabsf(c) * 4.76837158e-07f);
        probe(c - d);
        probe(c);
        probe(c + d);
    };
    probe3(p0y);
    probe3(p2y);
    if (quad) probe3(vert);
    if (LB >= HB) return false;
    if (LB == kmin) LB = first_at_least(r.a, r.b, r.c1, r.c2, r.flags, 1, kmin, HB);
    if (HB == kmax + 1u) HB = first_at_least(r.a, r.b, r.c1, r.c2, r.flags, 2, LB, kmax + 1u);
    if (LB >= HB) return false;
    (void)seen1;
    lo = key2f(LB);
    hi = key2f(HB - 1u);
    return true;
}


__device__ inline bool build_record(const int16_t *p, uint32_t root, Rec &r)
{
    const float p0x = (float)p[0], p0y = (float)p[1];
    const float p1x = (float)p[2], p1y = (float)p[3];
    const float p2x = (float)p[4], p2y = (float)p[5];
    const float a = p0y - 2 * p1y + p2y;
    r.ax = p0x - 2 * p1x + p2x;
    r.bx = 2 * (p1x - p0x);
    r.p0x = p0x;
    r.sqsign = root ? 0x80000000u : 0u;
    if (a == 0.0f) {
        if (root != 0u || p2y == p0y) return false;
        r.a = 0.0f; r.b = p0y; r.c1 = p2y - p0y; r.c2 = 0.0f;
        r.rden = 1.0f / r.c1;
        r.flags = REC_LINEAR | ((p0y < p2y) ? REC_LIN_MINUS : REC_LIN_PLUS);
    } else {
        r.a = a; r.b = p0y - p1y; r.c1 = p1y * p1y; r.c2 = p0y * p2y;
        r.rden = 1.0f / a;
        r.flags = root ? REC_NEG_ROOT : 0u;
    }
    float lo, hi;
    if (!accept_bracket(r, p0y, p2y, lo, hi)) return false;
    r.lo = lo; r.hi = hi;
    return true;
}

struct RowGeom {
    int32_t max_y;
    float scale;
    uint32_t rows;
    int n, phase;
    const float *cyt = nullptr;
    float inv = 1.0f;
    bool pow2 = false;
    __device__ __forceinline__ void set_scale(const ScaleDiv &d) { scale = d.scale; inv = d.inv; pow2 = d.pow2; }
    __device__ __forceinline__ float cy(uint32_t r) const
    {
        if (cyt) return cyt[r];
        const float num = (float)(max_y - (int32_t)(r / (uint32_t)n)) - sub_off((int)(r % (uint32_t)n), n, phase);
        if (pow2) return num * inv;
        return num / scale;
    }
    __device__ __forceinline__ float row_of(float c) const
    {
        return ((float)max_y - c * scale) * (float)n - (phase ? 0.5f : 0.0f);
    }
};

__device__ __forceinline__ int classify_row(const Rec &r, float cy)
{
    const bool lin = (r.flags & REC_LINEAR) != 0;
    const float delta = cy * r.a + r.c1 - r.c2;
    const float sq = sqrt_rn(delta);
    const float num = lin ? (cy - r.b) : ((r.flags & REC_NEG_ROOT) ? (r.b - sq) : (r.b + sq));
    const float t = div_by_int(num, lin ? r.c1 : r.a, r.rden);
    const bool falls = lin ? !(r.c1 > 0.0f) : ((r.flags & REC_NEG_ROOT) != 0);
    int cl = 1;
    if (t >= 1.0f) cl = falls ? 0 : 2;
    if (t < 0.0f) cl = falls ? 2 : 0;
    if (!lin && delta < 0.0f) cl = (r.a > 0.0f) ? 0 : 2;
    return cl;
}

struct Piece {
    float ylo, yhi;
    float a;
    double cv;
    uint32_t vend;
};
__device__ __forceinline__ bool fill_at_or_above_vertex(const Piece &pc, float cy)
{
    const double d = __builtin_fma((double)pc.a, (double)cy, pc.cv);
    return pc.a > 0.0f ? d >= 0.0 : d <= 0.0;
}
__device__ __forceinline__ int classify_fill(const Piece &pc, float cy)
{
    const bool above = (pc.vend == 2u) ? fill_at_or_above_vertex(pc, cy) : (cy >= pc.yhi);
    const bool below = (pc.vend == 1u) ? !fill_at_or_above_vertex(pc, cy) : (cy < pc.ylo);
    return above ? 2 : (below ? 0 : 1);
}
template <int FILL>
__device__ __forceinline__ int row_class(const Rec &r, const Piece &pc, float cy)
{
    if constexpr (FILL != 0) return classify_fill(pc, cy);
    else return classify_row(r, cy);
}

struct RowGuess {
    uint32_t ra, re;
    bool empty;
};

template <int FILL = 0>
__device__ __forceinline__ void record_prep(const int16_t *p, uint32_t root, const RowGeom &G, Rec &r, RowGuess &g, Piece *pc = nullptr)
{
    const float p0x = (float)p[0], p0y = (float)p[1];
    const float p1x = (float)p[2], p1y = (float)p[3];
    const float p2x = (float)p[4], p2y = (float)p[5];
    const float a = p0y - 2 * p1y + p2y;
    r.ax = p0x - 2 * p1x + p2x;
    r.bx = 2 * (p1x - p0x);
    r.p0x = p0x;
    r.sqsign = root ? 0x80000000u : 0u;
    const bool lin = a == 0.0f;
    const float b = p0y - p1y;
    bool empty;
    float c_start = p0y, c_stop = p2y;
    bool stop_incl = false;
    if (lin) {
        empty = (root != 0u) || (p2y == p0y);
        r.a = 0.0f; r.b = p0y; r.c1 = p2y - p0y; r.c2 = 0.0f;
        r.rden = 1.0f / r.c1;
        r.flags = REC_LINEAR | ((p0y < p2y) ? REC_LIN_MINUS : REC_LIN_PLUS);
    } else {
        r.a = a; r.b = b; r.c1 = p1y * p1y; r.c2 = p0y * p2y;
        r.rden = 1.0f / a;
        r.flags = root ? REC_NEG_ROOT : 0u;
        const bool far_side = (root == 0u) == (a > 0.0f);
        const bool tv_le0 = (b * a) <= 0.0f, tv_lt0 = (b * a) < 0.0f;
        const bool tv_ge1 = (a > 0.0f) ? (b >= a) : (b <= a);
        const float yv = p0y - (b * b) * r.rden;
        if (far_side) {
            empty = tv_ge1;
            if (!tv_le0) c_start = yv;
        } else {
            empty = tv_lt0;
            if (!tv_ge1) { c_stop = yv; stop_incl = true; }
        }
        if constexpr (FILL != 0) {
            const bool has_v = far_side ? !tv_le0 : !tv_ge1;
            if (!far_side && b == 0.0f) empty = true;
            const float other = far_side ? p2y : p0y;
            pc->a = a;
            pc->cv = (double)b * (double)b - (double)a * (double)p0y;
            pc->vend = has_v ? (a > 0.0f ? 1u : 2u) : 0u;
            pc->ylo = has_v ? (a > 0.0f ? yv : other) : fminf(p0y, p2y);
            pc->yhi = has_v ? (a > 0.0f ? other : yv) : fmaxf(p0y, p2y);
            if (!has_v && p0y == p2y) empty = true;
            c_start = pc->yhi; c_stop = pc->ylo;
            stop_incl = true;
        }
    }
    if constexpr (FILL != 0) {
        if (lin) {
            pc->a = 1.0f; pc->cv = 0.0; pc->vend = 0u;
            pc->ylo = fminf(p0y, p2y); pc->yhi = fmaxf(p0y, p2y);
            c_start = pc->yhi; c_stop = pc->ylo;
            stop_incl = true;
        }
    }
    g.empty = empty;
    g.ra = 1u; g.re = 0u;
    if (!empty) {
        const float top = (float)G.rows;
        const bool start_hi = c_start >= c_stop;
        const float xh = G.row_of(start_hi ? c_start : c_stop), xl = G.row_of(start_hi ? c_stop : c_start);
        const bool hi_incl = (FILL != 0) ? false : (start_hi ? true : stop_incl), lo_incl = start_hi ? stop_incl : true;
        const float fa = hi_incl ? __builtin_ceilf(xh) : __builtin_floorf(xh) + 1.0f;
        const float fe = lo_incl ? __builtin_floorf(xl) + 1.0f : __builtin_ceilf(xl);
        g.ra = (uint32_t)fminf(fmaxf(fa, 0.0f), top);
        g.re = (uint32_t)fminf(fmaxf(fe, 0.0f), top);
    }
}

template <int FILL = 0>
__device__ __forceinline__ void record_settle(const Rec &r, const RowGeom &G, uint32_t &ra, uint32_t &re, const Piece *pc = nullptr)
{
    auto classify_row = [&](const Rec &rr, float cy) {
        if constexpr (FILL != 0) return classify_fill(*pc, cy);
        else return fr::classify_row(rr, cy);
    };
#pragma clang loop unroll(disable) vectorize(disable) interleave(disable)
    while (ra > 0u && classify_row(r, G.cy(ra - 1u)) <= 1) --ra;
#pragma clang loop unroll(disable) vectorize(disable) interleave(disable)
    while (ra < G.rows && classify_row(r, G.cy(ra)) == 2) ++ra;
    if (re < ra) re = ra;
#pragma clang loop unroll(disable) vectorize(disable) interleave(disable)
    while (re > ra && classify_row(r, G.cy(re - 1u)) == 0) --re;
#pragma clang loop unroll(disable) vectorize(disable) interleave(disable)
    while (re < G.rows && classify_row(r, G.cy(re)) >= 1) ++re;
}

template <int FILL = 0>
__device__ __forceinline__ void build_record_rows(const int16_t *p, uint32_t root, const RowGeom &G, Rec &r)
{
    RowGuess g;
    Piece pc;
    record_prep<FILL>(p, root, G, r, g, &pc);
    uint32_t ra = g.ra, re = g.re;
    if (!g.empty) record_settle<FILL>(r, G, ra, re, &pc);
    r.lo = __builtin_bit_cast(float, ra);
    r.hi = __builtin_bit_cast(float, re);
}


__device__ inline bool build_record_fill(const int16_t *p, uint32_t root, Rec &r)
{
    RowGeom G;
    G.max_y = 0; G.scale = 1.0f; G.rows = 0u; G.n = 1; G.phase = 0;
    RowGuess g;
    Piece pc;
    record_prep<1>(p, root, G, r, g, &pc);
    if (g.empty) return false;
    const uint32_t kmin = f2key(-3.402823466e+38f), kmax = f2key(3.402823466e+38f);
    auto first_at_least = [&](int T) {
        uint32_t L = kmin, H = kmax + 1u;
        while (L < H) {
            const uint32_t mid = L + ((H - L) >> 1);
            if (classify_fill(pc, key2f(mid)) >= T) H = mid; else L = mid + 1u;
        }
        return L;
    };
    const uint32_t LB = first_at_least(1), HB = first_at_least(2);
    if (LB >= HB) return false;
    r.lo = key2f(LB);
    r.hi = key2f(HB - 1u);
    return true;
}
}
```

### font-renderer_amd/csrc/fr_selftest.hip

```cpp
#include "../../include/fr_raster.h"
#include "fr_device.hpp"

namespace fr {

__global__ __launch_bounds__(256) void selftest_div_kernel(uint32_t d_lo, uint32_t n_d,
                                                           unsigned long long *mismatches,
                                                           uint32_t *first_bad)
{
    const uint32_t d_idx = blockIdx.x / 32u, part = blockIdx.x % 32u;
    if (d_idx >= n_d) return;
    const float d = (float)(d_lo + d_idx);
    const float rd = 1.0f / d, rdn = 1.0f / (-d);
    uint32_t bad = 0, bad_x = 0;
    for (uint32_t m = part * 256u + threadIdx.x; m < (1u << 23); m += 32u * 256u) {
        const float x = __uint_as_float(0x3f800000u | m);
        const float xs = __uint_as_float(0x2f800000u | m);
        const float xl = __uint_as_float(0x4f800000u | m);
        const bool ok = (__float_as_uint(div_by_int(x, d, rd)) == __float_as_uint(x / d)) &&
                        (__float_as_uint(div_by_int(x, -d, rdn)) == __float_as_uint(x / -d)) &&
                        (__float_as_uint(div_by_int(-xs, d, rd)) == __float_as_uint(-xs / d)) &&
                        (__float_as_uint(div_by_int(xl, d, rd)) == __float_as_uint(xl / d));
        if (!ok) { ++bad; bad_x = 0x3f800000u | m; }
    }
    if (bad) {
        atomicAdd(mismatches, (unsigned long long)bad);
        atomicMax(&first_bad[0], d_lo + d_idx);
        first_bad[1] = bad_x;
    }
}

__global__ __launch_bounds__(256) void selftest_sqrt_kernel(uint32_t e_lo, unsigned long long *mismatches, uint32_t *first_bad)
{
    const uint32_t e = e_lo + blockIdx.x / 32u, part = blockIdx.x % 32u;
    uint32_t bad = 0, bad_x = 0;
    for (uint32_t m = part * 256u + threadIdx.x; m < (1u << 23); m += 32u * 256u) {
        const uint32_t bits = (e << 23) | m;
        const float x = __uint_as_float(bits);
        if (__float_as_uint(sqrt_rn(x)) != __float_as_uint(__builtin_sqrtf(x))) { ++bad; bad_x = bits; }
    }
    if (bad) {
        atomicAdd(mismatches, (unsigned long long)bad);
        first_bad[0] = bad_x;
    }
}

template <int VARIANT>
__global__ __launch_bounds__(256) void selftest_sqrt_fast_kernel(uint32_t e_lo, unsigned long long *mismatches, uint32_t *first_bad)
{
    const uint32_t e = e_lo + blockIdx.x / 32u, part = blockIdx.x % 32u;
    uint32_t bad = 0, bad_x = 0;
    for (uint32_t m = part * 256u + threadIdx.x; m < (1u << 23); m += 32u * 256u) {
        const uint32_t bits = (e << 23) | m;
        const float x = __uint_as_float(bits);
        if (__float_as_uint(sqrt_fast<VARIANT>(x)) != __float_as_uint(__builtin_sqrtf(x))) { ++bad; bad_x = bits; }
    }
    if (blockIdx.x == 0u && threadIdx.x == 0u) {
        float z = 0.0f, n = -2.0f;
        asm volatile("" : "+v"(z), "+v"(n));
        if (__float_as_uint(sqrt_fast<VARIANT>(z)) != 0u) { ++bad; bad_x = 0u; }
        const float sn = sqrt_fast<VARIANT>(n);
        if (sn == sn) { ++bad; bad_x = __float_as_uint(n); }
    }
    if (bad) {
        atomicAdd(mismatches, (unsigned long long)bad);
        first_bad[0] = bad_x;
    }
}

}

extern "C" int fr_selftest_sqrt_fast(int variant, uint64_t *mismatches, uint32_t *bad_x_bits)
{
    if (!mismatches || variant < 0 || variant > 1) return FR_E_INVALID;
    unsigned long long *d_m = nullptr;
    uint32_t *d_b = nullptr;
    if (hipMalloc(&d_m, 8) != hipSuccess || hipMalloc(&d_b, 8) != hipSuccess) return FR_E_HIP;
    (void)hipMemset(d_m, 0, 8);
    (void)hipMemset(d_b, 0, 8);
    const uint32_t e_lo = 97u, e_hi = 192u;
    const dim3 grid((e_hi - e_lo + 1u) * 32u), block(256);
    if (variant == 0) hipLaunchKernelGGL(fr::selftest_sqrt_fast_kernel<0>, grid, block, 0, 0, e_lo, d_m, d_b);
    else hipLaunchKernelGGL(fr::selftest_sqrt_fast_kernel<1>, grid, block, 0, 0, e_lo, d_m, d_b);
    unsigned long long m = 0;
    uint32_t b = 0;
    hipError_t e = hipMemcpy(&m, d_m, 8, hipMemcpyDeviceToHost);
    if (e == hipSuccess) e = hipMemcpy(&b, d_b, 4, hipMemcpyDeviceToHost);
    (void)hipFree(d_m);
    (void)hipFree(d_b);
    if (e != hipSuccess) return FR_E_HIP;
    *mismatches = m;
    if (bad_x_bits) *bad_x_bits = b;
    return FR_OK;
}

extern "C" int fr_selftest_sqrt(uint64_t *mismatches, uint32_t *bad_x_bits)
{
    if (!mismatches) return FR_E_INVALID;
    unsigned long long *d_m = nullptr;
    uint32_t *d_b = nullptr;
    if (hipMalloc(&d_m, 8) != hipSuccess || hipMalloc(&d_b, 8) != hipSuccess) return FR_E_HIP;
    (void)hipMemset(d_m, 0, 8);
    (void)hipMemset(d_b, 0, 8);
    const uint32_t e_lo = 97u, e_hi = 192u;
    hipLaunchKernelGGL(fr::selftest_sqrt_kernel, dim3((e_hi - e_lo + 1u) * 32u), dim3(256), 0, 0, e_lo, d_m, d_b);
    unsigned long long m = 0;
    uint32_t b = 0;
    hipError_t e = hipMemcpy(&m, d_m, 8, hipMemcpyDeviceToHost);
    if (e == hipSuccess) e = hipMemcpy(&b, d_b, 4, hipMemcpyDeviceToHost);
    (void)hipFree(d_m);
    (void)hipFree(d_b);
    if (e != hipSuccess) return FR_E_HIP;
    *mismatches = m;
    if (bad_x_bits) *bad_x_bits = b;
    return FR_OK;
}

extern "C" int fr_selftest_division(uint32_t d_lo, uint32_t d_hi, uint64_t *mismatches,
                                    uint32_t *bad_divisor, uint32_t *bad_x_bits)
{
    if (!mismatches || d_lo < 1 || d_hi < d_lo || d_hi > (1u << 17)) return FR_E_INVALID;
    unsigned long long *d_m = nullptr;
    uint32_t *d_b = nullptr;
    if (hipMalloc(&d_m, 8) != hipSuccess || hipMalloc(&d_b, 8) != hipSuccess) return FR_E_HIP;
    (void)hipMemset(d_m, 0, 8);
    (void)hipMemset(d_b, 0, 8);
    const uint32_t n_d = d_hi - d_lo + 1;
    for (uint32_t off = 0; off < n_d; off += 4096u) {
        const uint32_t n = n_d - off < 4096u ? n_d - off : 4096u;
        hipLaunchKernelGGL(fr::selftest_div_kernel, dim3(n * 32u), dim3(256), 0, 0, d_lo + off, n, d_m, d_b);
    }
    unsigned long long m = 0;
    uint32_t b[2] = {0, 0};
    hipError_t e = hipMemcpy(&m, d_m, 8, hipMemcpyDeviceToHost);
    if (e == hipSuccess) e = hipMemcpy(b, d_b, 8, hipMemcpyDeviceToHost);
    (void)hipFree(d_m);
    (void)hipFree(d_b);
    if (e != hipSuccess) return FR_E_HIP;
    *mismatches = m;
    if (bad_divisor) *bad_divisor = b[0];
    if (bad_x_bits) *bad_x_bits = b[1];
    return FR_OK;
}
```

### font-renderer_amd/render_glyph.py

```python
from __future__ import annotations

import ctypes as C
from typing import Optional, Sequence

import numpy as np

from . import _lib as L
from .glyph import FontInformation, Glyph, GlyphSet
from .image import RGB, Gray, Winding


def _flat(glyph: Glyph):
    gs = GlyphSet([glyph])
    return gs.points_xy, gs.contour_start, len(gs.contour_start) - 1


class Context:

    def __init__(self, device: int = 0, stream: Optional[int] = None):
        self._lib = L.load_library()
        h = C.c_void_p()
        L.check(self._lib.fr_ctx_create(device, C.c_void_p(stream) if stream else None, C.byref(h)))
        self._h = h
        self.device = device

    def set_option(self, key: str, value: int) -> None:
        L.check(self._lib.fr_ctx_set_option(self._h, key.encode(), value))

    def sync(self) -> None:
        L.check(self._lib.fr_ctx_sync(self._h))

    def close(self) -> None:
        if getattr(self, "_h", None):
            self._lib.fr_ctx_destroy(self._h)
            self._h = None

    def __enter__(self):
        return self

    def __exit__(self, *a):
        self.close()

    def __del__(self):
        try:
            self.close()
        except Exception:
            pass


_default_ctx: Optional[Context] = None


def default_context() -> Context:
    global _default_ctx
    if _default_ctx is None:
        _default_ctx = Context(0)
    return _default_ctx


class DeviceGlyphSet:

    def __init__(self, ctx: Context, gs: GlyphSet):
        self.ctx, self.host = ctx, gs
        h = C.c_void_p()
        L.check(ctx._lib.fr_glyphset_create(ctx._h, L.ptr(gs.points_xy), L.ptr(gs.contour_start), gs.n_contours,
                                            L.ptr(gs.glyph_start), len(gs), C.byref(h)))
        self._h = h
        boxes = np.ascontiguousarray(gs.boxes, np.int16)
        L.check(ctx._lib.fr_glyphset_set_boxes(self._h, L.ptr(boxes)))

    def prepare(self) -> None:
        L.check(self.ctx._lib.fr_glyphset_prepare(self._h))

    def stats(self):
        a, b = C.c_uint64(), C.c_uint64()
        L.check(self.ctx._lib.fr_glyphset_stats(self._h, C.byref(a), C.byref(b)))
        return {"segments": a.value, "records": b.value}

    def close(self) -> None:
        if getattr(self, "_h", None):
            self.ctx._lib.fr_glyphset_destroy(self._h)
            self._h = None

    def __del__(self):
        try:
            self.close()
        except Exception:
            pass


def make_jobs(rows: Sequence) -> np.ndarray:
    dt = np.dtype([("glyph", "<u4"), ("min_x", "<i4"), ("max_y", "<i4"), ("w", "<u4"), ("h", "<u4"),
                   ("out_x", "<u4"), ("out_y", "<u4"), ("scale", "<f4")])
    a = np.zeros(len(rows), dt)
    for i, r in enumerate(rows):
        a[i] = tuple(r)
    return a


class Plan:

    def __init__(self, dgs: DeviceGlyphSet, jobs: np.ndarray, mode: int, samples_per_axis: int = 1,
                 sample_phase: int = L.FR_SAMPLE_CORNER, flags: int = 0):
        assert jobs.dtype.itemsize == 32
        self.ctx, self.dgs, self.mode = dgs.ctx, dgs, mode
        self.params = L.RasterParams(mode, samples_per_axis, sample_phase, 0)
        jobs = np.ascontiguousarray(jobs)
        h = C.c_void_p()
        L.check(self.ctx._lib.fr_plan_create_ex(self.ctx._h, dgs._h, L.ptr(jobs), len(jobs), C.byref(self.params), flags,
                                                C.byref(h)))
        self._h = h
        self.n_jobs = len(jobs)

    @property
    def pixels(self) -> int:
        return int(self.ctx._lib.fr_plan_pixels(self._h))

    def stats(self) -> dict:
        a, b = C.c_uint32(), C.c_uint32()
        L.check(self.ctx._lib.fr_plan_stats(self._h, C.byref(a), C.byref(b)))
        return {"jobs_cov4": a.value, "jobs_general": b.value}

    def describe(self) -> str:
        buf = C.create_string_buffer(1024)
        L.check(self.ctx._lib.fr_plan_describe(self._h, buf, len(buf)))
        return buf.value.decode()

    def render(self, out_dev_ptr: int, out_stride: int, out_rows: int) -> None:
        L.check(self.ctx._lib.fr_plan_render(self._h, C.c_void_p(out_dev_ptr), out_stride, out_rows))

    def render_timed(self, out_dev_ptr: int, out_stride: int, out_rows: int) -> float:
        ms = C.c_float()
        L.check(self.ctx._lib.fr_plan_render_timed(self._h, C.c_void_p(out_dev_ptr), out_stride, out_rows, C.byref(ms)))
        return ms.value

    def close(self) -> None:
        if getattr(self, "_h", None):
            self.ctx._lib.fr_plan_destroy(self._h)
            self._h = None

    def __del__(self):
        try:
            self.close()
        except Exception:
            pass


PLACE_DTYPE = np.dtype([("glyph", "<u4"), ("pen_x64", "<i4"), ("pen_y", "<i4")])
PLACE_EX_DTYPE = np.dtype([("glyph", "<u4"), ("pen_x64", "<i4"), ("pen_y64", "<i4"), ("scale", "<f4"), ("slant", "<f4")])
PLACE_AFFINE_DTYPE = np.dtype([("glyph", "<u4"), ("pen_x64", "<i4"), ("pen_y64", "<i4"), ("m", "<f4", (4,))])
RUN_DTYPE = np.dtype([("first", "<u4"), ("count", "<u4"), ("w", "<u4"), ("h", "<u4"), ("out_x", "<u4"), ("out_y", "<u4"),
                      ("scale", "<f4")])


def make_places(rows: Sequence) -> np.ndarray:
    return np.array([tuple(r) for r in rows], PLACE_DTYPE)


def make_places_ex(rows: Sequence) -> np.ndarray:
    return np.array([tuple(r) for r in rows], PLACE_EX_DTYPE)


def make_places_affine(rows: Sequence) -> np.ndarray:
    out = np.zeros(len(rows), PLACE_AFFINE_DTYPE)
    for k, r in enumerate(rows):
        out[k] = (r[0], r[1], r[2], tuple(r[3:7]))
    return out


def _places(places) -> tuple:
    dt = getattr(places, "dtype", None)
    if dt == PLACE_AFFINE_DTYPE:
        return np.ascontiguousarray(places, PLACE_AFFINE_DTYPE), "_affine"
    ex = dt == PLACE_EX_DTYPE
    return np.ascontiguousarray(places, PLACE_EX_DTYPE if ex else PLACE_DTYPE), "_ex" if ex else ""


def make_runs(rows: Sequence) -> np.ndarray:
    return np.array([tuple(r) for r in rows], RUN_DTYPE)


class TextPlan(Plan):

    def __init__(self, dgs: DeviceGlyphSet, places: np.ndarray, runs: np.ndarray, mode: int = L.FR_COVERAGE_U8,
                 samples_per_axis: int = 4, sample_phase: int = L.FR_SAMPLE_CENTER, flags: int = 0):
        places, ex = _places(places)
        runs = np.ascontiguousarray(runs, RUN_DTYPE)
        self.ctx, self.dgs, self.mode = dgs.ctx, dgs, mode
        self.params = L.RasterParams(mode, samples_per_axis, sample_phase, 0)
        h = C.c_void_p()
        create = getattr(self.ctx._lib, "fr_text_plan_create" + ex)
        L.check(create(self.ctx._h, dgs._h, L.ptr(places), len(places), L.ptr(runs), len(runs), C.byref(self.params), flags, C.byref(h)))
        self._h = h
        self.n_places, self.n_runs = len(places), len(runs)


def _colors(rows, n: int, what: str) -> np.ndarray:
    c = np.ascontiguousarray(np.asarray(rows, np.uint8).reshape(-1, 4)) if n else np.zeros((0, 4), np.uint8)
    if c.shape != (n, 4):
        raise ValueError(f"{what}: expected {n} RGBA colours, got shape {np.shape(rows)}")
    return c


class TextPlanRGBA(Plan):

    def __init__(self, dgs: DeviceGlyphSet, places: np.ndarray, place_rgba, runs: np.ndarray, run_clear_rgba,
                 samples_per_axis: int = 4, sample_phase: int = L.FR_SAMPLE_CENTER, flags: int = 0):
        places, ex = _places(places)
        runs = np.ascontiguousarray(runs, RUN_DTYPE)
        pc = _colors(place_rgba, len(places), "place_rgba")
        rc = None if run_clear_rgba is None else _colors(run_clear_rgba, len(runs), "run_clear_rgba")
        self.ctx, self.dgs, self.mode = dgs.ctx, dgs, L.FR_COVERAGE_U8
        self.params = L.RasterParams(L.FR_COVERAGE_U8, samples_per_axis, sample_phase, 0)
        h = C.c_void_p()
        create = getattr(self.ctx._lib, "fr_text_plan_create_rgba" + ex)
        L.check(create(self.ctx._h, dgs._h, L.ptr(places), L.ptr(pc), len(places), L.ptr(runs), None if rc is None else L.ptr(rc),
                       len(runs), C.byref(self.params), flags, C.byref(h)))
        self._h = h
        self.n_places, self.n_runs = len(places), len(runs)


def render_batch(dgs: DeviceGlyphSet, jobs: np.ndarray, mode: int, out: np.ndarray, samples_per_axis: int = 1,
                 sample_phase: int = L.FR_SAMPLE_CORNER, flags: int = 0) -> np.ndarray:
    want = np.int16 if mode == L.FR_WINDING_I16 else np.uint8
    assert out.dtype == want and out.ndim == 2 and out.flags.c_contiguous
    prm = L.RasterParams(mode, samples_per_axis, sample_phase, 0)
    jobs = np.ascontiguousarray(jobs)
    L.check(dgs.ctx._lib.fr_render_batch_ex(dgs.ctx._h, dgs._h, L.ptr(jobs), len(jobs), C.byref(prm), flags, L.ptr(out),
                                            out.shape[1], out.shape[0]))
    return out


def render_glyph_dims(box, units_per_em: int, font_size: int):
    lib = L.load_library()
    b = np.asarray(box, np.int16)
    mn, mx = np.zeros(2, np.int16), np.zeros(2, np.int16)
    w, h, s = C.c_uint16(), C.c_uint16(), C.c_float()
    L.check(lib.fr_render_glyph_dims(L.ptr(b), units_per_em, font_size, L.ptr(mn), L.ptr(mx), C.byref(w), C.byref(h), C.byref(s)))
    return (int(mn[0]), int(mn[1])), (int(mx[0]), int(mx[1])), w.value, h.value, s.value


def srgb_to_linear16(values) -> np.ndarray:
    a = np.ascontiguousarray(values, np.uint8)
    out = np.empty(a.shape, np.uint16)
    L.check(L.load_library().fr_srgb_decode(L.ptr(a), a.size, L.ptr(out)))
    return out


def linear16_to_srgb(values) -> np.ndarray:
    a = np.asarray(values)
    if a.size and (a.min() < 0 or a.max() > 65535):
        raise ValueError("linear16_to_srgb: values outside [0, 65535]")
    a = np.ascontiguousarray(a, np.uint16)
    out = np.empty(a.shape, np.uint8)
    L.check(L.load_library().fr_srgb_encode(L.ptr(a), a.size, L.ptr(out)))
    return out


def renderGlyph(glyph: Glyph, font_info: FontInformation, font_size: int, *, ctx: Optional[Context] = None,
                mode: int = L.FR_GRAY_DEBUG, flags: int = 0) -> Gray:
    ctx = ctx or default_context()
    _, _, w, h, _ = render_glyph_dims(glyph.box.as_array(), font_info.units_per_em, font_size)
    im = Gray.init(w, h)
    pts, cstart, nc = _flat(glyph)
    box = glyph.box.as_array()
    L.check(ctx._lib.fr_render_glyph_ex(ctx._h, L.ptr(pts), L.ptr(cstart), nc, L.ptr(box), font_info.units_per_em,
                                        font_size, mode, flags, L.ptr(im.data)))
    return im


def renderGlyphWinding(glyph: Glyph, font_info: FontInformation, font_size: int, *, ctx: Optional[Context] = None,
                       scaler: int = 50, overflow_color: int = 150, flags: int = 0) -> Winding:
    ctx = ctx or default_context()
    _, _, w, h, _ = render_glyph_dims(glyph.box.as_array(), font_info.units_per_em, font_size)
    im = Winding.init(w, h, scaler, overflow_color)
    pts, cstart, nc = _flat(glyph)
    box = glyph.box.as_array()
    L.check(ctx._lib.fr_render_glyph_ex(ctx._h, L.ptr(pts), L.ptr(cstart), nc, L.ptr(box), font_info.units_per_em,
                                        font_size, L.FR_WINDING_I16, flags, L.ptr(im.data)))
    return im


class GlyphInfo:
    CURVE_TYPES = ("x_axis", "balance", "up_stright", "up_normal", "up_u", "up_inv_u",
                   "down_stright", "down_normal", "down_inv_u", "down_u")

    def __init__(self, curve_type: np.ndarray, include_p0: np.ndarray, curves_per_contour: Sequence[int]):
        self.curve_type, self.include_p0 = curve_type, include_p0
        self.contours, o = [], 0
        for n in curves_per_contour:
            self.contours.append(list(zip(curve_type[o:o + n].tolist(), include_p0[o:o + n].astype(bool).tolist())))
            o += n

    @staticmethod
    def init(glyph: Glyph, *, ctx: Optional[Context] = None) -> "GlyphInfo":
        ctx = ctx or default_context()
        pts, cstart, nc = _flat(glyph)
        n = glyph.curve_count
        ct, ip = np.zeros(max(n, 1), np.uint8), np.zeros(max(n, 1), np.uint8)
        L.check(ctx._lib.fr_glyph_info_init(ctx._h, L.ptr(pts), L.ptr(cstart), nc, L.ptr(ct), L.ptr(ip)))
        return GlyphInfo(ct[:n], ip[:n], [c.curve_count for c in glyph.contours])

    def deinit(self) -> None:
        self.contours = []


def windingInGlyph(glyph: Glyph, glyph_info: Optional[GlyphInfo], point, *, ctx: Optional[Context] = None):
    ctx = ctx or default_context()
    q = np.ascontiguousarray(point, np.int16).reshape(-1, 2)
    pts, cstart, nc = _flat(glyph)
    out = np.zeros(len(q), np.int16)
    L.check(ctx._lib.fr_winding_in_glyph(ctx._h, L.ptr(pts), L.ptr(cstart), nc, L.ptr(q), len(q), L.ptr(out)))
    return int(out[0]) if np.ndim(point) == 1 else out


def winding_lattice(glyph: Glyph, *, ctx: Optional[Context] = None) -> np.ndarray:
    ctx = ctx or default_context()
    pts, cstart, nc = _flat(glyph)
    box = glyph.box.as_array()
    W, H = int(box[2]) - int(box[0]) + 3, int(box[3]) - int(box[1]) + 3
    out = np.zeros((H, W), np.int16)
    L.check(ctx._lib.fr_winding_lattice(ctx._h, L.ptr(pts), L.ptr(cstart), nc, L.ptr(box), L.ptr(out)))
    return out


def exact_lattice(glyph: Glyph, K: int, x0: int, y0: int, w: int, h: int, *, ctx: Optional[Context] = None) -> np.ndarray:
    ctx = ctx or default_context()
    pts, cstart, nc = _flat(glyph)
    out = np.zeros((h, w), np.int16)
    L.check(ctx._lib.fr_exact_lattice(ctx._h, L.ptr(pts), L.ptr(cstart), nc, K, x0, y0, w, h, L.ptr(out)))
    return out


def exact_coverage(glyph: Glyph, K: int, x0: int, y0: int, w_px: int, h_px: int, n: int, *,
                   ctx: Optional[Context] = None) -> np.ndarray:
    ctx = ctx or default_context()
    pts, cstart, nc = _flat(glyph)
    out = np.zeros((h_px, w_px), np.uint8)
    L.check(ctx._lib.fr_exact_coverage(ctx._h, L.ptr(pts), L.ptr(cstart), nc, K, x0, y0, w_px, h_px, n, L.ptr(out)))
    return out


def glyph_debug_render(glyph: Glyph, winding_scale: int, *, ctx: Optional[Context] = None) -> RGB:
    ctx = ctx or default_context()
    pts, cs, nc = _flat(glyph)
    box = glyph.box.as_array()
    W, H = int(box[2]) - int(box[0]) + 3, int(box[3]) - int(box[1]) + 3
    out = np.zeros((H * W, 3), np.uint8)
    L.check(ctx._lib.fr_glyph_debug_render(ctx._h, L.ptr(pts), L.ptr(cs), nc, L.ptr(box), winding_scale, L.ptr(out)))
    return RGB(W, H, out)


def build_id() -> str:
    return L.load_library().fr_build_id().decode()
```

### include/fr_raster.h

```cpp
#ifndef FR_RASTER_H
#define FR_RASTER_H

#include <stddef.h>
#include <stdint.h>

#ifdef __cplusplus
extern "C" {
#endif

#define FR_ABI_VERSION 1

typedef enum fr_status {
    FR_OK = 0,
    FR_E_INVALID = -1,
    FR_E_HIP = -2,
    FR_E_NOMEM = -3,
    FR_E_UNSUPPORTED = -4
} fr_status;

typedef enum fr_mode {
    FR_WINDING_I16 = 0,
    FR_GRAY_DEBUG = 1,
    FR_MASK_NONZERO = 2,
    FR_COVERAGE_U8 = 3,
    FR_SDF_U8 = 4
} fr_mode;

typedef enum fr_sample_phase { FR_SAMPLE_CORNER = 0, FR_SAMPLE_CENTER = 1 } fr_sample_phase;

#define FR_FILL_CONSISTENT 1u

typedef struct fr_raster_params {
    int32_t mode;
    int32_t samples_per_axis;
    int32_t sample_phase;
    int32_t reserved;
} fr_raster_params;

typedef struct fr_job {
    uint32_t glyph;
    int32_t  min_x, max_y;
    uint32_t w, h;
    uint32_t out_x, out_y;
    float    scale;
} fr_job;

typedef struct fr_ctx fr_ctx;
typedef struct fr_glyphset fr_glyphset;
typedef struct fr_plan fr_plan;

int fr_abi_version(void);
const char *fr_last_error(void);
const char *fr_build_id(void);

int fr_ctx_create(int device, void *hip_stream, fr_ctx **out);
void fr_ctx_destroy(fr_ctx *ctx);
int fr_ctx_sync(fr_ctx *ctx);
int fr_ctx_set_option(fr_ctx *ctx, const char *key, int64_t value);

int fr_glyphset_create(fr_ctx *ctx, const int16_t *points_xy, const uint32_t *contour_start,
                       uint32_t n_contours, const uint32_t *glyph_start, uint32_t n_glyphs,
                       fr_glyphset **out);
void fr_glyphset_destroy(fr_glyphset *gs);
int fr_glyphset_prepare(fr_glyphset *gs);
int fr_glyphset_stats(const fr_glyphset *gs, uint64_t *n_segments, uint64_t *n_records);
int fr_glyphset_set_boxes(fr_glyphset *gs, const int16_t *boxes);

int fr_plan_create(fr_ctx *ctx, const fr_glyphset *gs, const fr_job *jobs, uint32_t n_jobs,
                   const fr_raster_params *params, fr_plan **out);
int fr_plan_create_ex(fr_ctx *ctx, const fr_glyphset *gs, const fr_job *jobs, uint32_t n_jobs,
                      const fr_raster_params *params, uint32_t flags, fr_plan **out);
void fr_plan_destroy(fr_plan *plan);
int fr_plan_render(fr_plan *plan, void *out_dev, size_t out_stride, size_t out_rows);
int fr_plan_render_timed(fr_plan *plan, void *out_dev, size_t out_stride, size_t out_rows, float *ms);
uint64_t fr_plan_pixels(const fr_plan *plan);
int fr_plan_stats(const fr_plan *plan, uint32_t *n_jobs_cov4, uint32_t *n_jobs_general);
int fr_plan_describe(const fr_plan *plan, char *buf, size_t cap);

typedef struct fr_glyph_place {
    uint32_t glyph;
    int32_t  pen_x64;
    int32_t  pen_y;
} fr_glyph_place;

typedef struct fr_text_run {
    uint32_t first, count;
    uint32_t w, h;
    uint32_t out_x, out_y;
    float    scale;
} fr_text_run;

int fr_text_plan_create(fr_ctx *ctx, const fr_glyphset *gs, const fr_glyph_place *places, uint32_t n_places,
                        const fr_text_run *runs, uint32_t n_runs, const fr_raster_params *params, uint32_t flags,
                        fr_plan **out);

#define FR_TEXT_BGRA 4u
#define FR_TEXT_SRGB 8u

#define FR_TEXT_LOAD 32u

int fr_text_plan_create_rgba(fr_ctx *ctx, const fr_glyphset *gs, const fr_glyph_place *places, const uint8_t *place_rgba,
                             uint32_t n_places, const fr_text_run *runs, const uint8_t *run_clear_rgba, uint32_t n_runs,
                             const fr_raster_params *params, uint32_t flags, fr_plan **out);

typedef struct fr_glyph_place_ex {
    uint32_t glyph;
    int32_t  pen_x64;
    int32_t  pen_y64;
    float    scale;
    float    slant;
} fr_glyph_place_ex;

int fr_text_plan_create_ex(fr_ctx *ctx, const fr_glyphset *gs, const fr_glyph_place_ex *places, uint32_t n_places,
                           const fr_text_run *runs, uint32_t n_runs, const fr_raster_params *params, uint32_t flags,
                           fr_plan **out);
int fr_text_plan_create_rgba_ex(fr_ctx *ctx, const fr_glyphset *gs, const fr_glyph_place_ex *places,
                                const uint8_t *place_rgba, uint32_t n_places, const fr_text_run *runs,
                                const uint8_t *run_clear_rgba, uint32_t n_runs, const fr_raster_params *params,
                                uint32_t flags, fr_plan **out);

#define FR_TEXT_CACHE 128u

#define FR_TEXT_OVER 256u

typedef struct fr_glyph_place_affine {
    uint32_t glyph;
    int32_t  pen_x64;
    int32_t  pen_y64;
    float    m[4];
} fr_glyph_place_affine;

int fr_text_plan_create_affine(fr_ctx *ctx, const fr_glyphset *gs, const fr_glyph_place_affine *places, uint32_t n_places,
                               const fr_text_run *runs, uint32_t n_runs, const fr_raster_params *params, uint32_t flags,
                               fr_plan **out);
int fr_text_plan_create_rgba_affine(fr_ctx *ctx, const fr_glyphset *gs, const fr_glyph_place_affine *places,
                                    const uint8_t *place_rgba, uint32_t n_places, const fr_text_run *runs,
                                    const uint8_t *run_clear_rgba, uint32_t n_runs, const fr_raster_params *params,
                                    uint32_t flags, fr_plan **out);

int fr_render_batch(fr_ctx *ctx, const fr_glyphset *gs, const fr_job *jobs, uint32_t n_jobs,
                    const fr_raster_params *params, void *out_host, size_t out_stride, size_t out_rows);
int fr_render_batch_ex(fr_ctx *ctx, const fr_glyphset *gs, const fr_job *jobs, uint32_t n_jobs,
                       const fr_raster_params *params, uint32_t flags, void *out_host, size_t out_stride, size_t out_rows);

int fr_render_glyph_dims(const int16_t box[4], uint16_t units_per_em, uint16_t font_size,
                         int16_t min_corner[2], int16_t max_corner[2],
                         uint16_t *width, uint16_t *height, float *scale);
int fr_render_glyph(fr_ctx *ctx, const int16_t *points_xy, const uint32_t *contour_start,
                    uint32_t n_contours, const int16_t box[4], uint16_t units_per_em,
                    uint16_t font_size, int32_t mode, void *out_host);
int fr_render_glyph_ex(fr_ctx *ctx, const int16_t *points_xy, const uint32_t *contour_start,
                       uint32_t n_contours, const int16_t box[4], uint16_t units_per_em,
                       uint16_t font_size, int32_t mode, uint32_t flags, void *out_host);

int fr_glyph_info_init(fr_ctx *ctx, const int16_t *points_xy, const uint32_t *contour_start,
                       uint32_t n_contours, uint8_t *curve_type, uint8_t *include_p0);
int fr_winding_in_glyph(fr_ctx *ctx, const int16_t *points_xy, const uint32_t *contour_start,
                        uint32_t n_contours, const int16_t *query_xy, uint32_t n_query,
                        int16_t *out_winding);
int fr_winding_lattice(fr_ctx *ctx, const int16_t *points_xy, const uint32_t *contour_start,
                       uint32_t n_contours, const int16_t box[4], int16_t *out_host);

int fr_glyph_debug_render(fr_ctx *ctx, const int16_t *points_xy, const uint32_t *contour_start,
                          uint32_t n_contours, const int16_t box[4], uint8_t winding_scale, uint8_t *rgb_host);

int fr_exact_lattice(fr_ctx *ctx, const int16_t *points_xy, const uint32_t *contour_start,
                     uint32_t n_contours, uint32_t K, int32_t x0, int32_t y0, uint32_t w, uint32_t h,
                     int16_t *out_host );
int fr_exact_coverage(fr_ctx *ctx, const int16_t *points_xy, const uint32_t *contour_start,
                      uint32_t n_contours, uint32_t K, int32_t x0, int32_t y0, uint32_t w_px, uint32_t h_px,
                      uint32_t n, uint8_t *out_host );

int fr_atlas_layout(const int16_t *boxes, uint32_t n_glyphs, uint32_t first_glyph,
                    const uint16_t *units_per_em, uint32_t n_upm, uint16_t font_size,
                    uint32_t cell, uint32_t cols, uint32_t rows_per_page,
                    fr_job *jobs_out, uint32_t *page_of_job, uint32_t *n_pages);

int fr_atlas_layout_glyph_dims(const int16_t *boxes, uint32_t n_glyphs, uint32_t first_glyph,
                               const uint16_t *units_per_em, uint32_t n_upm, uint16_t font_size,
                               uint32_t atlas_w, uint32_t align, fr_job *jobs_out, uint32_t *atlas_h);

int fr_allgather_bands(fr_ctx *ctx, void *nccl_comm, void *atlas_dev, size_t band_bytes);
int fr_gather_bands(fr_ctx *ctx, void *nccl_comm, void *atlas_dev, size_t band_bytes, int root);

typedef struct fr_font fr_font;
#define FR_FONT_ALLOW_HINTED 1u
int fr_font_open(const void *ttf_bytes, size_t len, uint32_t flags, fr_font **out);
void fr_font_close(fr_font *font);
int fr_font_info(const fr_font *font, uint16_t *units_per_em, uint16_t *num_glyphs, int *y0_baseline);
int fr_font_char_to_glyph(const fr_font *font, uint32_t codepoint, uint16_t *glyph_index);
int fr_font_glyph_advance(const fr_font *font, uint16_t glyph_index, int16_t *advance_width);
int fr_font_glyph_measure(fr_font *font, uint16_t glyph_index, uint32_t *n_contours, uint32_t *n_points, int16_t box[4]);
int fr_font_glyph_fill(fr_font *font, uint16_t glyph_index, int16_t *points_xy, uint32_t *contour_start);

int fr_text_layout(const fr_font *font, const uint32_t *codepoints, uint32_t n, uint16_t font_size,
                   uint16_t *glyph_index_out, int32_t *pen_x64_out, int32_t *end_pen_x64);

size_t fr_qoi_bound(uint32_t width, uint32_t height);
int fr_qoi_encode_rgb(const uint8_t *rgb, uint32_t width, uint32_t height, uint8_t *out, size_t cap, size_t *n_out);
int fr_qoi_encode_gray(const uint8_t *gray, uint32_t width, uint32_t height, size_t stride, uint8_t *out, size_t cap, size_t *n_out);
int fr_qoi_encode_rgba(const uint8_t *rgba, uint32_t width, uint32_t height, size_t stride_px, uint8_t *out, size_t cap, size_t *n_out);

int fr_srgb_decode(const uint8_t *in, size_t n, uint16_t *out);
int fr_srgb_encode(const uint16_t *in, size_t n, uint8_t *out);

int fr_rgba_unpremultiply(uint8_t *rgba, size_t n_pixels, int srgb);

int fr_selftest_division(uint32_t d_lo, uint32_t d_hi, uint64_t *mismatches,
                         uint32_t *bad_divisor, uint32_t *bad_x_bits);
int fr_selftest_sqrt(uint64_t *mismatches, uint32_t *bad_x_bits);

#ifdef __cplusplus
}
#endif
#endif
```

Baseline: 2.531 million.

## Precompute per-segment row-cut intervals at prepare time to classify rows cheaply

Adds a prepare-time kernel that computes, for each segment root, a height interval (cut lo/hi) where the row classification changes. The cov4 setup paths load these cuts and use them to drop segments that miss the job's row span early and to classify rows with two comparisons instead of full record classification. This is meant to cut setup cost per glyph cell. It costs an extra float4 per segment of device memory, an extra global load per candidate, and a new selftest to verify the cuts match the reference classification.

```diff
diff --git a/bindings/fr_raster.zig b/bindings/fr_raster.zig
--- a/bindings/fr_raster.zig
+++ b/bindings/fr_raster.zig
@@ -128,6 +128,7 @@
 pub extern "c" fn fr_rgba_unpremultiply(rgba: [*]u8, n_pixels: usize, srgb: c_int) c_int;
 pub extern "c" fn fr_selftest_division(d_lo: u32, d_hi: u32, mismatches: *u64, bad_divisor: ?*u32, bad_x_bits: ?*u32) c_int;
 pub extern "c" fn fr_selftest_sqrt(mismatches: *u64, bad_x_bits: ?*u32) c_int;
+pub extern "c" fn fr_selftest_row_cuts(gs: *fr_glyphset, jobs: [*]const Job, n_jobs: u32, samples_per_axis: c_int, phase: c_int, pairs: *u64, mismatches: *u64, first_bad: ?*[3]u32) c_int;
 
 pub const Error = error{ RasterFailed, OutOfMemory };
 
diff --git a/font-renderer_amd/_lib.py b/font-renderer_amd/_lib.py
--- a/font-renderer_amd/_lib.py
+++ b/font-renderer_amd/_lib.py
@@ -123,6 +123,7 @@
     ("fr_rgba_unpremultiply", C.c_int, [_P, C.c_size_t, C.c_int]),
     ("fr_selftest_sqrt", C.c_int, [C.POINTER(C.c_uint64), C.POINTER(C.c_uint32)]),
     ("fr_selftest_division", C.c_int, [C.c_uint32, C.c_uint32, C.POINTER(C.c_uint64), C.POINTER(C.c_uint32), C.POINTER(C.c_uint32)]),
+    ("fr_selftest_row_cuts", C.c_int, [_P, _P, C.c_uint32, C.c_int, C.c_int, C.POINTER(C.c_uint64), C.POINTER(C.c_uint64), C.POINTER(C.c_uint32)]),
 ]
 
 _lib = None
diff --git a/font-renderer_amd/csrc/fr_api.hip b/font-renderer_amd/csrc/fr_api.hip
--- a/font-renderer_amd/csrc/fr_api.hip
+++ b/font-renderer_amd/csrc/fr_api.hip
@@ -18,6 +18,9 @@
 namespace fr {
 void launch_prepare(const int16_t *, const uint32_t *, const uint32_t *, const uint32_t *, uint32_t, Rec *,
                     uint32_t *, hipStream_t, int fill = 0);
+void launch_cuts(const int16_t *, uint32_t, float4 *, hipStream_t);
+void launch_selftest_row_cuts(const Job *, uint32_t, uint32_t, const uint32_t *, const int16_t *, const float4 *, int, int,
+                              unsigned long long *, hipStream_t);
 hipError_t launch_render(const RenderArgs &, const RasterLaunch &, hipStream_t);
 uint32_t render_wg_waves();
 hipError_t launch_cov4(const RenderArgs &, const RasterLaunch &, hipStream_t);
@@ -75,6 +78,7 @@
     uint32_t lds_pad = 0;
     uint32_t min_wgs = 2048;
     uint32_t cov4 = 1;
+    uint32_t row_cuts = 1;
     uint32_t zero_copy = 0;
     uint32_t sdf_cull = 1;
     uint32_t overlap = 1;
@@ -95,6 +99,7 @@
     int16_t *d_pts = nullptr, *d_seg_pts = nullptr;
     uint32_t *d_seg_p0 = nullptr, *d_seg_prev = nullptr, *d_glyph_seg_start = nullptr, *d_rec_count = nullptr;
     fr::Rec *d_recs = nullptr;
+    float4 *d_seg_cut = nullptr;
     std::vector<uint32_t> h_glyph_seg_start;
     std::vector<uint32_t> h_root_bound;
     std::vector<uint32_t> h_ray_bound;
@@ -157,6 +162,7 @@
     a.pts = plan->gs->d_pts;
     a.seg_p0 = plan->gs->d_seg_p0;
     a.seg_pts = plan->gs->d_seg_pts;
+    a.seg_cut = plan->ctx->row_cuts ? plan->gs->d_seg_cut : nullptr;
     a.fused = plan->ctx->fuse_prepare ? 1u : 0u;
     a.out = out_dev;
     a.out_stride = out_stride;
@@ -312,6 +318,7 @@
     if (!strcmp(key, "fuse_prepare")) { ctx->fuse_prepare = value ? 1u : 0u; return FR_OK; }
     if (!strcmp(key, "lds_pad")) { ctx->lds_pad = (uint32_t)value; return FR_OK; }
     if (!strcmp(key, "cov4")) { ctx->cov4 = value ? 1u : 0u; return FR_OK; }
+    if (!strcmp(key, "row_cuts")) { ctx->row_cuts = value ? 1u : 0u; return FR_OK; }
     if (!strcmp(key, "sdf_cull")) { ctx->sdf_cull = value ? 1u : 0u; return FR_OK; }
     if (!strcmp(key, "overlap")) {
         if (value < 0 || value > 2) return fail(FR_E_INVALID, "overlap must be 0 (never), 1 (plans of >= 32 Mpixel) or 2 (always)");
@@ -333,7 +340,7 @@
     (void)hipSetDevice(gs->ctx->device);
     (void)hipStreamSynchronize(gs->ctx->stream);
     dfree(gs->d_pts); dfree(gs->d_seg_pts); dfree(gs->d_seg_p0); dfree(gs->d_seg_prev); dfree(gs->d_glyph_seg_start);
-    dfree(gs->d_rec_count); dfree(gs->d_recs);
+    dfree(gs->d_rec_count); dfree(gs->d_recs); dfree(gs->d_seg_cut);
     delete gs;
 }
 
@@ -400,6 +407,7 @@
     GS_TRY(hipMalloc(&gs->d_glyph_seg_start, ((size_t)n_glyphs + 1) * 4));
     GS_TRY(hipMalloc(&gs->d_rec_count, ((size_t)n_glyphs + 1) * 4));
     GS_TRY(hipMalloc(&gs->d_recs, 2 * nseg1 * sizeof(fr::Rec)));
+    GS_TRY(hipMalloc(&gs->d_seg_cut, nseg1 * sizeof(float4)));
     hipStream_t st = ctx->stream;
     if (np) GS_TRY(hipMemcpyAsync(gs->d_pts, points_xy, np * 2 * sizeof(int16_t), hipMemcpyHostToDevice, st));
     std::vector<int16_t> seg_pts((size_t)gs->n_seg * 6);
@@ -416,6 +424,8 @@
     GS_TRY(hipMemsetAsync(gs->d_rec_count, 0, ((size_t)n_glyphs + 1) * 4, st));
     fr::launch_prepare(gs->d_pts, gs->d_seg_p0, gs->d_glyph_seg_start, nullptr, n_glyphs, gs->d_recs,
                        gs->d_rec_count, st);
+    GS_TRY(hipGetLastError());
+    fr::launch_cuts(gs->d_seg_pts, gs->n_seg, gs->d_seg_cut, st);
     GS_TRY(hipGetLastError());
     GS_TRY(hipStreamSynchronize(st));
 #undef GS_TRY
@@ -435,6 +445,63 @@
         uint64_t t = 0;
         for (uint32_t g = 0; g < gs->n_glyphs; ++g) t += cnt[g];
         *n_records = t;
+    }
+    return FR_OK;
+}
+
+static int check_job(const fr_glyphset *gs, const fr_job &jb, uint32_t j)
+{
+    if (jb.glyph >= gs->n_glyphs) return fail(FR_E_INVALID, "job %u: glyph %u of %u", j, jb.glyph, gs->n_glyphs);
+    if (!(jb.scale > 0.0f) || !std::isfinite(jb.scale)) return fail(FR_E_INVALID, "job %u: scale must be finite and > 0", j);
+    if (jb.scale < 9.5367431640625e-07f || jb.scale > 1048576.0f)
+        return fail(FR_E_UNSUPPORTED, "job %u: scale outside [2^-20, 2^20]", j);
+    if (jb.w > 65535u || jb.h > 65535u) return fail(FR_E_UNSUPPORTED, "job %u: cell larger than 65535", j);
+    if (jb.min_x < -(1 << 22) || (int64_t)jb.min_x + jb.w > (1 << 22) || jb.max_y > (1 << 22) ||
+        (int64_t)jb.max_y - jb.h < -(1 << 22))
+        return fail(FR_E_UNSUPPORTED, "job %u: pixel coordinates beyond +-2^22", j);
+    return FR_OK;
+}
+
+int fr_selftest_row_cuts(fr_glyphset *gs, const fr_job *jobs, uint32_t n_jobs, int samples_per_axis, int phase,
+                         uint64_t *pairs, uint64_t *mismatches, uint32_t *first_bad)
+{
+    if (!gs || !pairs || !mismatches) return fail(FR_E_INVALID, "fr_selftest_row_cuts: NULL argument");
+    if (n_jobs && !jobs) return fail(FR_E_INVALID, "jobs is NULL");
+    const int n = samples_per_axis;
+    if (n != 1 && n != 2 && n != 4) return fail(FR_E_UNSUPPORTED, "samples_per_axis %d not in {1,2,4}", n);
+    if (phase != FR_SAMPLE_CORNER && phase != FR_SAMPLE_CENTER) return fail(FR_E_INVALID, "unknown sample_phase %d", phase);
+    if (!gs->d_seg_cut) return fail(FR_E_INVALID, "fr_selftest_row_cuts: the glyph set has no row cuts");
+    uint32_t max_rows = 0;
+    for (uint32_t j = 0; j < n_jobs; ++j) {
+        if (const int jrc = check_job(gs, jobs[j], j)) return jrc;
+        max_rows = std::max(max_rows, jobs[j].h * (uint32_t)n);
+    }
+    *pairs = 0; *mismatches = 0;
+    if (first_bad) first_bad[0] = first_bad[1] = first_bad[2] = 0u;
+    if (n_jobs == 0 || max_rows == 0) return FR_OK;
+    HIP_TRY(hipSetDevice(gs->ctx->device));
+    hipStream_t st = gs->ctx->stream;
+    fr::Job *d_jobs = nullptr;
+    unsigned long long *d_res = nullptr;
+    unsigned long long res[3] = {0ull, 0ull, ~0ull};
+    hipError_t e = hipMalloc(&d_jobs, (size_t)n_jobs * sizeof(fr::Job));
+    if (e == hipSuccess) e = hipMalloc(&d_res, sizeof res);
+    if (e == hipSuccess) e = hipMemcpyAsync(d_jobs, jobs, (size_t)n_jobs * sizeof(fr::Job), hipMemcpyHostToDevice, st);
+    if (e == hipSuccess) e = hipMemcpyAsync(d_res, res, sizeof res, hipMemcpyHostToDevice, st);
+    if (e == hipSuccess) {
+        fr::launch_selftest_row_cuts(d_jobs, n_jobs, max_rows, gs->d_glyph_seg_start, gs->d_seg_pts, gs->d_seg_cut, n,
+                                     phase == FR_SAMPLE_CENTER ? 1 : 0, d_res, st);
+        e = hipGetLastError();
+    }
+    if (e == hipSuccess) e = hipMemcpyAsync(res, d_res, sizeof res, hipMemcpyDeviceToHost, st);
+    if (e == hipSuccess) e = hipStreamSynchronize(st);
+    else (void)hipStreamSynchronize(st);
+    dfree(d_jobs); dfree(d_res);
+    if (e != hipSuccess) return fail(e == hipErrorOutOfMemory ? FR_E_NOMEM : FR_E_HIP, "fr_selftest_row_cuts: %s", hipGetErrorString(e));
+    *pairs = res[0];
+    *mismatches = res[1];
+    if (first_bad && res[1]) {
+        first_bad[0] = (uint32_t)(res[2] >> 40); first_bad[1] = (uint32_t)((res[2] >> 20) & 0xfffffu); first_bad[2] = (uint32_t)(res[2] & 0xfffffu);
     }
     return FR_OK;
 }
@@ -525,15 +592,7 @@
     if (rc) return rc;
     if (n_jobs && !jobs) return fail(FR_E_INVALID, "jobs is NULL");
     for (uint32_t j = 0; j < n_jobs; ++j) {
-        const fr_job &jb = jobs[j];
-        if (jb.glyph >= gs->n_glyphs) return fail(FR_E_INVALID, "job %u: glyph %u of %u", j, jb.glyph, gs->n_glyphs);
-        if (!(jb.scale > 0.0f) || !std::isfinite(jb.scale)) return fail(FR_E_INVALID, "job %u: scale must be finite and > 0", j);
-        if (jb.scale < 9.5367431640625e-07f || jb.scale > 1048576.0f)
-            return fail(FR_E_UNSUPPORTED, "job %u: scale outside [2^-20, 2^20]", j);
-        if (jb.w > 65535u || jb.h > 65535u) return fail(FR_E_UNSUPPORTED, "job %u: cell larger than 65535", j);
-        if (jb.min_x < -(1 << 22) || (int64_t)jb.min_x + jb.w > (1 << 22) || jb.max_y > (1 << 22) ||
-            (int64_t)jb.max_y - jb.h < -(1 << 22))
-            return fail(FR_E_UNSUPPORTED, "job %u: pixel coordinates beyond +-2^22", j);
+        if (const int jrc = check_job(gs, jobs[j], j)) return jrc;
     }
     fr_plan *p = new (std::nothrow) fr_plan;
     if (!p) return fail(FR_E_NOMEM, "fr_plan_create: host allocation");
diff --git a/font-renderer_amd/csrc/fr_c4.hpp b/font-renderer_amd/csrc/fr_c4.hpp
--- a/font-renderer_amd/csrc/fr_c4.hpp
+++ b/font-renderer_amd/csrc/fr_c4.hpp
@@ -94,7 +94,15 @@
     }
 }
 
-template <uint32_t RCAP, int N, uint32_t NCOL, int FILL>
+__device__ __forceinline__ Cut c4_load_cut(const RenderArgs &A, uint32_t seg0, uint32_t c)
+{
+    const float2 q = reinterpret_cast<const float2 *>(A.seg_cut)[2u * (size_t)seg0 + c];
+    Cut k;
+    k.lo = q.x; k.hi = q.y;
+    return k;
+}
+
+template <uint32_t RCAP, int N, uint32_t NCOL, int FILL, int CUT>
 __device__ __forceinline__ uint32_t c4_setup_small(const RenderArgs &A, const Job &job, uint32_t seg0, uint32_t nseg, uint32_t x0s,
                                                    int phase, float *s_cxp, Rec40 *s_rec, uint32_t *s_wcnt, uint32_t *s_tmp, const float *cyt = nullptr)
 {
@@ -109,11 +117,15 @@
     Piece pc;
     g.empty = true; g.ra = 1u; g.re = 0u;
     uint32_t cls = 3u;
+    Cut k;
+    k.lo = k.hi = 0.0f;
     if (have) {
-        record_prep<FILL>(A.seg_pts + 6u * (size_t)(seg0 + (lane >> 1)), lane & 1u, geo, r, g, &pc);
+        bool drop = false;
+        if constexpr (CUT != 0) { k = c4_load_cut(A, seg0, lane); drop = cut_misses(k, row_span(geo)); }
+        record_prep<FILL>(A.seg_pts + 6u * (size_t)(seg0 + (lane >> 1)), lane & 1u, geo, r, g, &pc, drop);
         if (!g.empty) {
             const uint32_t row = (wave == 0u) ? g.ra - 1u : (wave == 1u) ? g.ra : (wave == 2u) ? g.re - 1u : g.re;
-            if (row < Hs && (wave != 2u || g.re > g.ra)) cls = (uint32_t)row_class<FILL>(r, pc, geo.cy(row));
+            if (row < Hs && (wave != 2u || g.re > g.ra)) cls = (uint32_t)row_class<FILL, CUT>(r, pc, geo.cy(row), &k);
         }
     }
     s_tmp[tid] = cls;
@@ -131,7 +143,7 @@
             if (!g.empty) {
                 const uint32_t c0 = s_tmp[lane], c1 = s_tmp[64u + lane], c2 = s_tmp[128u + lane], c3 = s_tmp[192u + lane];
                 const bool ok = (c0 >= 2u) && (c1 <= 1u || c1 == 3u) && re >= ra && (c2 >= 1u) && (c3 == 0u || c3 == 3u);
-                if (!ok) record_settle<FILL>(r, geo, ra, re, &pc);
+                if (!ok) record_settle<FILL, CUT>(r, geo, ra, re, &pc, &k);
             }
             live = ra < re;
             mine = c4_make_rec40<FILL>(r, ra, re);
@@ -149,7 +161,7 @@
     return s_wcnt[0];
 }
 
-template <uint32_t RCAP, int N, uint32_t NCOL, int FILL>
+template <uint32_t RCAP, int N, uint32_t NCOL, int FILL, int CUT>
 __device__ __forceinline__ uint32_t c4_setup_mid(const RenderArgs &A, const Job &job, uint32_t seg0, uint32_t nseg, uint32_t x0s,
                                                  int phase, float *s_cxp, Rec40 *s_rec, uint32_t *s_wcnt, uint32_t *s_tmp, const float *cyt = nullptr)
 {
@@ -165,12 +177,16 @@
     Piece pc;
     g.empty = true; g.ra = 1u; g.re = 0u;
     uint32_t cls0 = 3u, cls1 = 3u;
+    Cut k;
+    k.lo = k.hi = 0.0f;
     if (have) {
-        record_prep<FILL>(A.seg_pts + 6u * (size_t)(seg0 + (c >> 1)), c & 1u, geo, r, g, &pc);
+        bool drop = false;
+        if constexpr (CUT != 0) { k = c4_load_cut(A, seg0, c); drop = cut_misses(k, row_span(geo)); }
+        record_prep<FILL>(A.seg_pts + 6u * (size_t)(seg0 + (c >> 1)), c & 1u, geo, r, g, &pc, drop);
         if (!g.empty) {
             const uint32_t end = h ? g.re : g.ra;
-            if (end - 1u < Hs && (h == 0u || g.re > g.ra)) cls0 = (uint32_t)row_class<FILL>(r, pc, geo.cy(end - 1u));
-            if (end < Hs) cls1 = (uint32_t)row_class<FILL>(r, pc, geo.cy(end));
+            if (end - 1u < Hs && (h == 0u || g.re > g.ra)) cls0 = (uint32_t)row_class<FILL, CUT>(r, pc, geo.cy(end - 1u), &k);
+            if (end < Hs) cls1 = (uint32_t)row_class<FILL, CUT>(r, pc, geo.cy(end), &k);
         }
     }
     s_tmp[tid] = cls0 | (cls1 << 8);
@@ -188,7 +204,7 @@
             const uint32_t up = s_tmp[c], dn = s_tmp[128u + c];
             const uint32_t c0 = up & 0xffu, c1 = up >> 8, c2 = dn & 0xffu, c3 = dn >> 8;
             const bool ok = (c0 >= 2u) && (c1 <= 1u || c1 == 3u) && re >= ra && (c2 >= 1u) && (c3 == 0u || c3 == 3u);
-            if (!ok) record_settle<FILL>(r, geo, ra, re, &pc);
+            if (!ok) record_settle<FILL, CUT>(r, geo, ra, re, &pc, &k);
         }
         live = ra < re;
         mine = c4_make_rec40<FILL>(r, ra, re);
@@ -207,14 +223,14 @@
     return min(n_quad + l0 + l1, RCAP);
 }
 
-template <uint32_t NW, uint32_t RCAP, int N, uint32_t NCOL, int FILL = 0>
-__device__ __forceinline__ uint32_t c4_setup(const RenderArgs &A, const Job &job, uint32_t seg0, uint32_t nseg, uint32_t x0s,
-                                             int phase, float *s_cxp, Rec40 *s_rec, uint32_t *s_wcnt, uint32_t *s_tmp, const float *cyt = nullptr)
+template <uint32_t NW, uint32_t RCAP, int N, uint32_t NCOL, int FILL, int CUT>
+__device__ __forceinline__ uint32_t c4_setup_with(const RenderArgs &A, const Job &job, uint32_t seg0, uint32_t nseg, uint32_t x0s,
+                                                  int phase, float *s_cxp, Rec40 *s_rec, uint32_t *s_wcnt, uint32_t *s_tmp, const float *cyt)
 {
     if (NW == 4u && 2u * nseg <= 64u)
-        return c4_setup_small<RCAP, N, NCOL, FILL>(A, job, seg0, nseg, x0s, phase, s_cxp, s_rec, s_wcnt, s_tmp, cyt);
+        return c4_setup_small<RCAP, N, NCOL, FILL, CUT>(A, job, seg0, nseg, x0s, phase, s_cxp, s_rec, s_wcnt, s_tmp, cyt);
     if (NW == 4u && 2u * nseg <= 128u)
-        return c4_setup_mid<RCAP, N, NCOL, FILL>(A, job, seg0, nseg, x0s, phase, s_cxp, s_rec, s_wcnt, s_tmp, cyt);
+        return c4_setup_mid<RCAP, N, NCOL, FILL, CUT>(A, job, seg0, nseg, x0s, phase, s_cxp, s_rec, s_wcnt, s_tmp, cyt);
     const uint32_t tid = threadIdx.x, lane = tid & 63u, wave = tid >> 6;
     const uint32_t Hs = job.h * (uint32_t)N;
     const ScaleDiv sdiv = scale_div(job.scale);
@@ -233,7 +249,13 @@
             Rec r;
             RowGeom geo;
             geo.max_y = job.max_y; geo.set_scale(sdiv); geo.rows = Hs; geo.n = N; geo.phase = phase; geo.cyt = cyt;
-            build_record_rows<FILL>(A.seg_pts + 6u * (size_t)(seg0 + (c >> 1)), c & 1u, geo, r);
+            if constexpr (CUT != 0) {
+                const Cut k = c4_load_cut(A, seg0, c);
+                const RowSpan span = row_span(geo);
+                build_record_rows<FILL, CUT>(A.seg_pts + 6u * (size_t)(seg0 + (c >> 1)), c & 1u, geo, r, &k, &span);
+            } else {
+                build_record_rows<FILL>(A.seg_pts + 6u * (size_t)(seg0 + (c >> 1)), c & 1u, geo, r);
+            }
             const uint32_t ra = __builtin_bit_cast(uint32_t, r.lo), re = __builtin_bit_cast(uint32_t, r.hi);
             live = ra < re;
             mine[it] = c4_make_rec40<FILL>(r, ra, re);
@@ -279,4 +301,19 @@
     return rec_cnt;
 }
 
-}
+template <uint32_t NW, uint32_t RCAP, int N, uint32_t NCOL, int FILL = 0>
+__device__ __forceinline__ uint32_t c4_setup(const RenderArgs &A, const Job &job, uint32_t seg0, uint32_t nseg, uint32_t x0s,
+                                             int phase, float *s_cxp, Rec40 *s_rec, uint32_t *s_wcnt, uint32_t *s_tmp, const float *cyt = nullptr)
+{
+#if !defined(FR_C4_ROW_CUTS) || FR_C4_ROW_CUTS == 1
+    if constexpr (FILL == 0) {
+#ifndef FR_C4_ROW_CUTS
+        if (A.seg_cut)
+#endif
+            return c4_setup_with<NW, RCAP, N, NCOL, 0, 1>(A, job, seg0, nseg, x0s, phase, s_cxp, s_rec, s_wcnt, s_tmp, cyt);
+    }
+#endif
+    return c4_setup_with<NW, RCAP, N, NCOL, FILL, 0>(A, job, seg0, nseg, x0s, phase, s_cxp, s_rec, s_wcnt, s_tmp, cyt);
+}
+
+}
diff --git a/font-renderer_amd/csrc/fr_device.hpp b/font-renderer_amd/csrc/fr_device.hpp
--- a/font-renderer_amd/csrc/fr_device.hpp
+++ b/font-renderer_amd/csrc/fr_device.hpp
@@ -83,6 +83,7 @@
     const int16_t *pts;
     const uint32_t *seg_p0;
     const int16_t *seg_pts;
+    const float4 *seg_cut;
     const uint32_t *job_bits;
     const uint32_t *bits;
     uint32_t fused;
diff --git a/font-renderer_amd/csrc/fr_prepare.hip b/font-renderer_amd/csrc/fr_prepare.hip
--- a/font-renderer_amd/csrc/fr_prepare.hip
+++ b/font-renderer_amd/csrc/fr_prepare.hip
@@ -53,6 +53,28 @@
     prepare_body<1>(pts, seg_p0, glyph_seg_start, glyph_list, n_glyphs, out_recs, glyph_rec_count);
 }
 
+__global__ __launch_bounds__(256) void cut_kernel(const int16_t *__restrict__ seg_pts, uint32_t n_cand, float2 *__restrict__ out)
+{
+    const uint32_t c = blockIdx.x * 256u + threadIdx.x;
+    if (c >= n_cand) return;
+    RowGeom G;
+    G.max_y = 0; G.scale = 1.0f; G.rows = 0u; G.n = 1; G.phase = 0;
+    Rec r;
+    RowGuess g;
+    record_prep<0>(seg_pts + 6u * (size_t)(c >> 1), c & 1u, G, r, g);
+    Cut k;
+    k.lo = __builtin_inff(); k.hi = -__builtin_inff();
+    if (!g.empty) k = find_cut(r);
+    out[c] = make_float2(k.lo, k.hi);
+}
+
+void launch_cuts(const int16_t *seg_pts, uint32_t n_seg, float4 *out, hipStream_t stream)
+{
+    if (n_seg == 0) return;
+    const uint32_t n_cand = 2u * n_seg;
+    hipLaunchKernelGGL(cut_kernel, dim3((uint32_t)(((uint64_t)n_cand + 255u) / 256u)), dim3(256), 0, stream, seg_pts, n_cand, reinterpret_cast<float2 *>(out));
+}
+
 void launch_prepare(const int16_t *pts, const uint32_t *seg_p0, const uint32_t *glyph_seg_start,
                     const uint32_t *glyph_list, uint32_t n_glyphs, Rec *out_recs, uint32_t *glyph_rec_count,
                     hipStream_t stream, int fill)
diff --git a/font-renderer_amd/csrc/fr_records.hpp b/font-renderer_amd/csrc/fr_records.hpp
--- a/font-renderer_amd/csrc/fr_records.hpp
+++ b/font-renderer_amd/csrc/fr_records.hpp
@@ -163,10 +163,43 @@
     const bool below = (pc.vend == 1u) ? !fill_at_or_above_vertex(pc, cy) : (cy < pc.ylo);
     return above ? 2 : (below ? 0 : 1);
 }
-template <int FILL>
-__device__ __forceinline__ int row_class(const Rec &r, const Piece &pc, float cy)
-{
+struct Cut {
+    float lo, hi;
+};
+__device__ __forceinline__ int classify_cut(const Cut &k, float cy)
+{
+    return cy > k.hi ? 2 : (cy < k.lo ? 0 : 1);
+}
+constexpr float CUT_HEIGHT_MIN = 1.1920929e-07f;
+constexpr float CUT_HEIGHT_MAX = 8796093022208.0f;
+__device__ __forceinline__ float cut_height(float cy)
+{
+    return fabsf(cy) < CUT_HEIGHT_MIN ? __builtin_copysignf(0.0f, cy) : cy;
+}
+__device__ inline Cut find_cut(const Rec &r)
+{
+    const uint32_t kmin = f2key(-CUT_HEIGHT_MAX), kmax = f2key(CUT_HEIGHT_MAX);
+    auto first_at_least = [&](int T, uint32_t L) {
+        uint32_t H = kmax + 1u;
+        while (L < H) {
+            const uint32_t mid = L + ((H - L) >> 1);
+            if (classify_row(r, cut_height(key2f(mid))) >= T) H = mid; else L = mid + 1u;
+        }
+        return L;
+    };
+    const uint32_t K1 = first_at_least(1, kmin), K2 = first_at_least(2, K1);
+    Cut k;
+    k.lo = key2f(K1);
+    k.hi = key2f(K2 - 1u);
+    return k;
+}
+
+template <int FILL, int CUT = 0>
+__device__ __forceinline__ int row_class(const Rec &r, const Piece &pc, float cy, const Cut *k = nullptr)
+{
+    static_assert(!(FILL != 0 && CUT != 0), "row cuts hold the reference's acceptance only");
     if constexpr (FILL != 0) return classify_fill(pc, cy);
+    else if constexpr (CUT != 0) return classify_cut(*k, cy);
     else return classify_row(r, cy);
 }
 
@@ -176,7 +209,7 @@
 };
 
 template <int FILL = 0>
-__device__ __forceinline__ void record_prep(const int16_t *p, uint32_t root, const RowGeom &G, Rec &r, RowGuess &g, Piece *pc = nullptr)
+__device__ __forceinline__ void record_prep(const int16_t *p, uint32_t root, const RowGeom &G, Rec &r, RowGuess &g, Piece *pc = nullptr, bool drop = false)
 {
     const float p0x = (float)p[0], p0y = (float)p[1];
     const float p1x = (float)p[2], p1y = (float)p[3];
@@ -233,6 +266,7 @@
             stop_incl = true;
         }
     }
+    empty = empty || drop;
     g.empty = empty;
     g.ra = 1u; g.re = 0u;
     if (!empty) {
@@ -247,11 +281,12 @@
     }
 }
 
-template <int FILL = 0>
-__device__ __forceinline__ void record_settle(const Rec &r, const RowGeom &G, uint32_t &ra, uint32_t &re, const Piece *pc = nullptr)
+template <int FILL = 0, int CUT = 0>
+__device__ __forceinline__ void record_settle(const Rec &r, const RowGeom &G, uint32_t &ra, uint32_t &re, const Piece *pc = nullptr, const Cut *k = nullptr)
 {
     auto classify_row = [&](const Rec &rr, float cy) {
         if constexpr (FILL != 0) return classify_fill(*pc, cy);
+        else if constexpr (CUT != 0) return classify_cut(*k, cy);
         else return fr::classify_row(rr, cy);
     };
 #pragma clang loop unroll(disable) vectorize(disable) interleave(disable)
@@ -265,14 +300,41 @@
     while (re < G.rows && classify_row(r, G.cy(re)) >= 1) ++re;
 }
 
-template <int FILL = 0>
-__device__ __forceinline__ void build_record_rows(const int16_t *p, uint32_t root, const RowGeom &G, Rec &r)
+struct RowSpan {
+    float top, bot;
+};
+__device__ __forceinline__ RowSpan row_span(const RowGeom &G)
+{
+    const uint32_t last = G.rows ? G.rows - 1u : 0u;
+    const float nt = (float)G.max_y - sub_off(0, G.n, G.phase);
+    const float nb = (float)(G.max_y - (int32_t)(last / (uint32_t)G.n)) - sub_off((int)(last % (uint32_t)G.n), G.n, G.phase);
+    RowSpan s;
+    if (G.pow2) {
+        s.top = nt * G.inv;
+        s.bot = nb * G.inv;
+    } else {
+        const float rs = __builtin_amdgcn_rcpf(G.scale);
+        const float t = nt * rs, b = nb * rs;
+        s.top = __builtin_fmaf(fabsf(t), 9.5367431640625e-07f, t);
+        s.bot = __builtin_fmaf(fabsf(b), -9.5367431640625e-07f, b);
+    }
+    return s;
+}
+__device__ __forceinline__ bool cut_misses(const Cut &k, const RowSpan &s)
+{
+    return !(k.lo <= k.hi) || k.hi < s.bot || k.lo > s.top;
+}
+
+template <int FILL = 0, int CUT = 0>
+__device__ __forceinline__ void build_record_rows(const int16_t *p, uint32_t root, const RowGeom &G, Rec &r, const Cut *k = nullptr, const RowSpan *span = nullptr)
 {
     RowGuess g;
     Piece pc;
-    record_prep<FILL>(p, root, G, r, g, &pc);
+    bool drop = false;
+    if constexpr (CUT != 0) drop = cut_misses(*k, *span);
+    record_prep<FILL>(p, root, G, r, g, &pc, drop);
     uint32_t ra = g.ra, re = g.re;
-    if (!g.empty) record_settle<FILL>(r, G, ra, re, &pc);
+    if (!g.empty) record_settle<FILL, CUT>(r, G, ra, re, &pc, k);
     r.lo = __builtin_bit_cast(float, ra);
     r.hi = __builtin_bit_cast(float, re);
 }
diff --git a/font-renderer_amd/csrc/fr_selftest.hip b/font-renderer_amd/csrc/fr_selftest.hip
--- a/font-renderer_amd/csrc/fr_selftest.hip
+++ b/font-renderer_amd/csrc/fr_selftest.hip
@@ -1,5 +1,5 @@
 #include "../../include/fr_raster.h"
-#include "fr_device.hpp"
+#include "fr_records.hpp"
 
 namespace fr {
 
@@ -65,6 +65,55 @@
         atomicAdd(mismatches, (unsigned long long)bad);
         first_bad[0] = bad_x;
     }
+}
+
+__global__ __launch_bounds__(256) void selftest_row_cuts_kernel(const Job *__restrict__ jobs, const uint32_t *__restrict__ glyph_seg_start,
+                                                                const int16_t *__restrict__ seg_pts, const float4 *__restrict__ seg_cut,
+                                                                int n, int phase, unsigned long long *res)
+{
+    const uint32_t j = blockIdx.x, row0 = blockIdx.y * 64u;
+    const Job job = jobs[j];
+    const uint32_t rows = job.h * (uint32_t)n;
+    if (row0 >= rows) return;
+    const uint32_t row1 = min(row0 + 64u, rows);
+    const uint32_t seg0 = glyph_seg_start[job.glyph], n_cand = 2u * (glyph_seg_start[job.glyph + 1u] - seg0);
+    RowGeom geo;
+    geo.max_y = job.max_y; geo.set_scale(scale_div(job.scale)); geo.rows = rows; geo.n = n; geo.phase = phase;
+    const RowSpan span = row_span(geo);
+    unsigned long long pairs = 0ull, bad = 0ull, first = ~0ull;
+    for (uint32_t c = threadIdx.x; c < n_cand; c += 256u) {
+        Rec r;
+        RowGuess g;
+        record_prep<0>(seg_pts + 6u * (size_t)(seg0 + (c >> 1)), c & 1u, geo, r, g);
+        if (g.empty) continue;
+        const float2 q = reinterpret_cast<const float2 *>(seg_cut)[2u * (size_t)seg0 + c];
+        Cut k;
+        k.lo = q.x; k.hi = q.y;
+        const unsigned long long where = ((unsigned long long)j << 40) | ((unsigned long long)min(c, 0xfffffu) << 20);
+        for (uint32_t row = row0; row < row1; ++row) {
+            const float cy = geo.cy(row);
+            ++pairs;
+            if (classify_cut(k, cy) != classify_row(r, cy)) { ++bad; first = min(first, where | row); }
+        }
+        if (row0 == 0u) {
+            uint32_t ra0 = g.ra, re0 = g.re, ra1 = g.ra, re1 = g.re;
+            record_settle<0, 0>(r, geo, ra0, re0);
+            record_settle<0, 1>(r, geo, ra1, re1, nullptr, &k);
+            bool differ = ra0 != ra1 || re0 != re1;
+            if (cut_misses(k, span)) differ = differ || ra0 < re0;
+            if (differ) { ++bad; first = min(first, where | 0xfffffull); }
+        }
+    }
+    if (pairs) atomicAdd(&res[0], pairs);
+    if (bad) { atomicAdd(&res[1], bad); atomicMin(&res[2], first); }
+}
+
+void launch_selftest_row_cuts(const Job *jobs, uint32_t n_jobs, uint32_t max_rows, const uint32_t *glyph_seg_start, const int16_t *seg_pts,
+                              const float4 *seg_cut, int n, int phase, unsigned long long *res, hipStream_t stream)
+{
+    if (n_jobs == 0 || max_rows == 0) return;
+    hipLaunchKernelGGL(selftest_row_cuts_kernel, dim3(n_jobs, (max_rows + 63u) / 64u), dim3(256), 0, stream, jobs, glyph_seg_start,
+                       seg_pts, seg_cut, n, phase, res);
 }
 
 }
diff --git a/font-renderer_amd/render_glyph.py b/font-renderer_amd/render_glyph.py
--- a/font-renderer_amd/render_glyph.py
+++ b/font-renderer_amd/render_glyph.py
@@ -76,6 +76,15 @@
         a, b = C.c_uint64(), C.c_uint64()
         L.check(self.ctx._lib.fr_glyphset_stats(self._h, C.byref(a), C.byref(b)))
         return {"segments": a.value, "records": b.value}
+
+    def selftest_row_cuts(self, jobs: np.ndarray, samples_per_axis: int = 1, sample_phase: int = L.FR_SAMPLE_CORNER):
+        assert jobs.dtype.itemsize == 32
+        jobs = np.ascontiguousarray(jobs)
+        pairs, bad = C.c_uint64(), C.c_uint64()
+        first = (C.c_uint32 * 3)()
+        L.check(self.ctx._lib.fr_selftest_row_cuts(self._h, L.ptr(jobs), len(jobs), samples_per_axis, sample_phase,
+                                                   C.byref(pairs), C.byref(bad), first))
+        return pairs.value, bad.value, tuple(first)
 
     def close(self) -> None:
         if getattr(self, "_h", None):
diff --git a/include/fr_raster.h b/include/fr_raster.h
--- a/include/fr_raster.h
+++ b/include/fr_raster.h
@@ -209,6 +209,8 @@
 int fr_selftest_division(uint32_t d_lo, uint32_t d_hi, uint64_t *mismatches,
                          uint32_t *bad_divisor, uint32_t *bad_x_bits);
 int fr_selftest_sqrt(uint64_t *mismatches, uint32_t *bad_x_bits);
+int fr_selftest_row_cuts(fr_glyphset *gs, const fr_job *jobs, uint32_t n_jobs, int samples_per_axis, int phase,
+                         uint64_t *pairs, uint64_t *mismatches, uint32_t *first_bad);
 
 #ifdef __cplusplus
 }
```

After: 2.569 million, median of 6. 1.5% higher.
